# mahmoudnafifi/HistoGAN

Measured on AMD Instinct MI355X. Metric: train images/sec (G+D step, 256², h=64) at 1/2/4/8 MI355X; hist-kernel HBM GB/s, higher is better.
Workload: dtype f32; 1 GPU; HistoGAN G+D train step 256x256 capacity=16 batch=32/GPU h=64 insz=150 inverse-quadratic (GP every 4th, PL every 32nd step); batch_per_gpu=32, global_batch=32, image_size=256, network_capacity=16, h=64, parallelism=dp1, params_G=82968288, params_D=90896289

## Files before the change

### histogan_amd/_lib.py

```python
import ctypes
import os

import torch

_PKG = os.path.dirname(os.path.abspath(__file__))
_TAG = os.environ.get('HG_LIB_TAG', '')
LIB_PATH = os.path.join(_PKG, 'libhistogan_hip' + ('_' + _TAG if _TAG else '') + '.so')

HG_METHOD = {'thresholding': 0, 'RBF': 1, 'inverse-quadratic': 2}
HG_RESIZE_NONE, HG_RESIZE_BILINEAR, HG_RESIZE_SAMPLING = 0, 1, 2
HG_PROJ = {'rgbuv': 0, 'rgchroma': 1, 'direct': 2}


class HgHistParams(ctypes.Structure):
    _fields_ = [
        ('struct_size', ctypes.c_uint32),
        ('B', ctypes.c_int32), ('C', ctypes.c_int32), ('H', ctypes.c_int32), ('W', ctypes.c_int32),
        ('stride_b', ctypes.c_int64), ('stride_c', ctypes.c_int64),
        ('stride_h', ctypes.c_int64), ('stride_w', ctypes.c_int64),
        ('Hs', ctypes.c_int32), ('Ws', ctypes.c_int32),
        ('resize_mode', ctypes.c_int32),
        ('row_idx', ctypes.c_void_p), ('col_idx', ctypes.c_void_p),
        ('h', ctypes.c_int32),
        ('lo', ctypes.c_double), ('hi', ctypes.c_double),
        ('method', ctypes.c_int32),
        ('sigma', ctypes.c_double),
        ('intensity_scale', ctypes.c_int32),
        ('green_only', ctypes.c_int32),
        ('projection', ctypes.c_int32),
        ('pre_relu', ctypes.c_int32),
        ('proj_cache', ctypes.c_void_p),
        ('weight', ctypes.c_void_p),
        ('weight_stride_b', ctypes.c_int64), ('weight_stride_h', ctypes.c_int64), ('weight_stride_w', ctypes.c_int64),
    ]


class GlinLayer(ctypes.Structure):
    _fields_ = [('x', ctypes.c_void_p), ('w', ctypes.c_void_p), ('b', ctypes.c_void_p), ('y', ctypes.c_void_p),
                ('gw', ctypes.c_void_p), ('gb', ctypes.c_void_p), ('N', ctypes.c_int32), ('group', ctypes.c_int32)]


def _load():
    if not os.path.exists(LIB_PATH):
        raise ImportError(
            f'{LIB_PATH} not found: the gfx950 HIP library has not been built. '
            f'Run `python -m histogan_amd.build` (needs hipcc). There is no CPU/PyTorch fallback.')
    lib = ctypes.CDLL(LIB_PATH, mode=ctypes.RTLD_GLOBAL)
    vp, sz, i32, i64, f32 = ctypes.c_void_p, ctypes.c_size_t, ctypes.c_int32, ctypes.c_int64, ctypes.c_float
    PP = ctypes.POINTER(HgHistParams)
    lib.hg_version.restype = ctypes.c_int
    lib.hg_version.argtypes = []
    lib.hg_error_string.restype = ctypes.c_char_p
    lib.hg_error_string.argtypes = [ctypes.c_int]
    lib.hg_rgbuv_hist_workspace_bytes.restype = ctypes.c_int
    lib.hg_rgbuv_hist_workspace_bytes.argtypes = [PP, ctypes.POINTER(sz), ctypes.POINTER(sz)]
    lib.hg_rgbuv_hist_uses_proj_cache.restype = ctypes.c_int
    lib.hg_rgbuv_hist_uses_proj_cache.argtypes = [PP]
    lib.hg_rgbuv_hist_fwd.restype = ctypes.c_int
    lib.hg_rgbuv_hist_fwd.argtypes = [PP, vp, vp, vp, vp, sz, vp]
    lib.hg_rgbuv_hist_bwd.restype = ctypes.c_int
    lib.hg_rgbuv_hist_bwd.argtypes = [PP, vp, vp, vp, vp, vp, vp, sz, vp]
    lib.hg_hellinger_workspace_bytes.restype = sz
    lib.hg_hellinger_workspace_bytes.argtypes = [i64]
    lib.hg_hellinger_fwd_bwd.restype = ctypes.c_int
    lib.hg_hellinger_fwd_bwd.argtypes = [vp, vp, i64, i32, f32, vp, vp, vp, sz, vp]
    lib.hg_selftest_fastlog.restype = ctypes.c_int
    lib.hg_selftest_fastlog.argtypes = [vp, vp]
    lib.hg_modulate_fwd.restype = ctypes.c_int
    lib.hg_modulate_fwd.argtypes = [vp, vp, vp, i32, i32, i32, i32, i32, vp]
    lib.hg_modulate_bwd.restype = ctypes.c_int
    lib.hg_modulate_bwd.argtypes = [vp, vp, vp, vp, vp, i32, i32, i32, i32, i32, vp, sz, vp]
    lib.hg_nets_workspace_bytes.restype = sz
    lib.hg_nets_workspace_bytes.argtypes = [i32, i32, i32, i32]
    lib.hg_torgb_fwd.restype = ctypes.c_int
    lib.hg_torgb_fwd.argtypes = [vp, vp, vp, vp, vp, i32, i32, i32, i32, vp]
    lib.hg_torgb_bwd_workspace_bytes.restype = sz
    lib.hg_torgb_bwd_workspace_bytes.argtypes = [i32, i32, i32, i32]
    lib.hg_torgb_bwd.restype = ctypes.c_int
    lib.hg_torgb_bwd.argtypes = [vp, vp, vp, vp, vp, vp, vp, i32, i32, i32, i32, vp, sz, vp]
    lib.hg_gstage_bwd_workspace_bytes.restype = sz
    lib.hg_gstage_bwd_workspace_bytes.argtypes = [i32, i32, i32, i32]
    lib.hg_gstage_bwd.restype = ctypes.c_int
    lib.hg_gstage_bwd.argtypes = [vp, vp, vp, i32, vp, vp, vp, i32, vp, vp, vp, vp, i32, vp, vp, vp, vp, vp, vp, vp, i32, i32, i32,
                                  vp, sz, vp]
    lib.hg_channel_sum.restype = ctypes.c_int
    lib.hg_channel_sum.argtypes = [vp, vp, i32, i32, i32, vp, sz, vp]
    lib.hg_demod_noise_lrelu_fwd.restype = ctypes.c_int
    lib.hg_demod_noise_lrelu_fwd.argtypes = [vp, vp, vp, vp, vp, vp, i32, i32, i32, i32, vp]
    lib.hg_demod_noise_lrelu_bwd.restype = ctypes.c_int
    lib.hg_demod_noise_lrelu_bwd.argtypes = [vp, vp, vp, vp, vp, vp, vp, vp, vp, vp, vp, i32, i32, i32, i32, vp, sz, vp]
    lib.hg_lrelu_bwd_channel_sum.restype = ctypes.c_int
    lib.hg_lrelu_bwd_channel_sum.argtypes = [vp, vp, f32, vp, vp, i32, i32, i32, vp, sz, vp]
    lib.hg_demod_style_grad_workspace_bytes.restype = ctypes.c_size_t
    lib.hg_demod_style_grad_workspace_bytes.argtypes = [i32, i32, i32]
    lib.hg_demod_style_grad.restype = ctypes.c_int
    lib.hg_demod_style_grad.argtypes = [vp, vp, vp, vp, vp, i32, i32, i32, vp, sz, vp]
    lib.hg_demod_weight_term.restype = ctypes.c_int
    lib.hg_demod_weight_term.argtypes = [vp, vp, vp, vp, vp, i32, i32, i32, i32, i32, vp]
    lib.hg_diffgrad_step.restype = ctypes.c_int
    lib.hg_diffgrad_step.argtypes = [vp, vp, vp, vp, vp, i64, f32, f32, f32, f32, i32, vp]
    lib.hg_diffgrad_step_size.restype = f32
    lib.hg_diffgrad_step_size.argtypes = [f32, f32, f32, i32]
    lib.hg_diffgrad_step_dev.restype = ctypes.c_int
    lib.hg_diffgrad_step_dev.argtypes = [vp, vp, vp, vp, vp, i64, vp, f32, f32, f32, vp]
    lib.hg_ema_update.restype = ctypes.c_int
    lib.hg_ema_update.argtypes = [vp, vp, i64, f32, vp]
    lib.hg_conv_packed_elems.restype = sz
    lib.hg_conv_packed_elems.argtypes = [i32, i32, i32, i32]
    lib.hg_conv_pack_weights.restype = ctypes.c_int
    lib.hg_conv_pack_weights.argtypes = [vp, vp, i32, i32, i32, i32, vp]
    lib.hg_conv_pack_weights_both.restype = ctypes.c_int
    lib.hg_conv_pack_weights_both.argtypes = [vp, vp, vp, i32, i32, i32, vp]
    lib.hg_conv2d_fwd.restype = ctypes.c_int
    lib.hg_conv2d_fwd.argtypes = [vp, vp, vp, vp, vp, vp, i32, i32, i32, i32, i32, i32, i32, vp, sz, vp]
    lib.hg_conv2d_fwd_add.restype = ctypes.c_int
    lib.hg_conv2d_fwd_add.argtypes = [vp, vp, vp, vp, vp, i32, i32, i32, i32, i32, i32, i32, vp, sz, vp]
    lib.hg_modconv2d_fwd.restype = ctypes.c_int
    lib.hg_modconv2d_fwd.argtypes = [vp, vp, vp, vp, vp, vp, vp, vp, i32, f32, i32, i32, i32, i32, i32, i32, vp, sz, vp]
    lib.hg_conv2d_workspace_bytes.restype = sz
    lib.hg_conv2d_workspace_bytes.argtypes = [i32, i32, i32, i32, i32, i32, i32, i32]
    lib.hg_conv_pack_blocks.restype = ctypes.c_int32
    lib.hg_conv_pack_blocks.argtypes = [i32, i32]
    lib.hg_conv_pack_weights_multi.restype = ctypes.c_int
    lib.hg_conv_pack_weights_multi.argtypes = [vp, i32, i32, vp]
    lib.hg_conv2d_plan.restype = ctypes.c_int
    lib.hg_conv2d_plan.argtypes = [i32, i32, i32, i32, i32, i32, i32, i32, ctypes.POINTER(ctypes.c_int32)]
    lib.hg_conv2d_dgrad.restype = ctypes.c_int
    lib.hg_conv2d_dgrad.argtypes = [vp, vp, vp, vp, vp, i32, i32, i32, i32, i32, i32, i32, vp, sz, vp]
    lib.hg_conv2d_wgrad_workspace_bytes.restype = sz
    lib.hg_conv2d_wgrad_workspace_bytes.argtypes = [i32, i32, i32, i32, i32, i32, i32]
    lib.hg_conv2d_wgrad.restype = ctypes.c_int
    lib.hg_conv2d_wgrad.argtypes = [vp, vp, vp, vp, vp, i32, i32, i32, i32, i32, i32, i32, vp, sz, vp]
    lib.hg_instnorm_workspace_bytes.restype = sz
    lib.hg_instnorm_workspace_bytes.argtypes = [i64]
    lib.hg_instnorm_lrelu_fwd.restype = ctypes.c_int
    lib.hg_instnorm_lrelu_fwd.argtypes = [vp, vp, vp, i64, i32, f32, f32, vp, sz, vp]
    lib.hg_instnorm_lrelu_bwd.restype = ctypes.c_int
    lib.hg_instnorm_lrelu_bwd.argtypes = [vp, vp, vp, vp, i64, i32, f32, vp, sz, vp]
    lib.hg_stencil3.restype = ctypes.c_int
    lib.hg_stencil3.argtypes = [vp, vp, ctypes.POINTER(f32), i32, i32, i32, i32, i32, vp]
    lib.hg_depthwise_valid.restype = ctypes.c_int
    lib.hg_depthwise_valid.argtypes = [vp, vp, vp, i64, i32, i32, i32, i32, vp]
    GL = ctypes.POINTER(GlinLayer)
    lib.hg_grouped_linear_fwd.restype = ctypes.c_int
    lib.hg_grouped_linear_fwd.argtypes = [GL, i32, i32, i32, vp]
    lib.hg_grouped_linear_bwd_input_workspace_bytes.restype = sz
    lib.hg_grouped_linear_bwd_input_workspace_bytes.argtypes = [GL, i32, i32, i32]
    lib.hg_grouped_linear_bwd_input.restype = ctypes.c_int
    lib.hg_grouped_linear_bwd_input.argtypes = [GL, i32, ctypes.POINTER(vp), i32, i32, i32, vp, sz, vp]
    lib.hg_grouped_linear_bwd_params.restype = ctypes.c_int
    lib.hg_grouped_linear_bwd_params.argtypes = [GL, i32, i32, i32, vp]
    lib.hg_wino_supported.restype = ctypes.c_int
    lib.hg_wino_supported.argtypes = [i32, i32, i32, i32, i32]
    lib.hg_wino_packed_elems.restype = sz
    lib.hg_wino_packed_elems.argtypes = [i32, i32, i32]
    lib.hg_wino_pack_weights.restype = ctypes.c_int
    lib.hg_wino_pack_weights.argtypes = [vp, vp, i32, i32, i32, vp]
    lib.hg_wino_pack_blocks.restype = ctypes.c_int32
    lib.hg_wino_pack_blocks.argtypes = [i32, i32, i32, i32]
    lib.hg_wino_pack_weights_multi.restype = ctypes.c_int
    lib.hg_wino_pack_weights_multi.argtypes = [vp, i32, i32, vp]
    lib.hg_wino_workspace_bytes.restype = sz
    lib.hg_wino_workspace_bytes.argtypes = [i32, i32, i32, i32, i32]
    lib.hg_wino_conv2d.restype = ctypes.c_int
    lib.hg_wino_conv2d.argtypes = [vp, vp, vp, vp, vp, vp, vp, vp, i32, f32, vp, i32, i32, i32, i32, i32, vp, sz, vp]
    lib.hg_wino_wgrad_supported.restype = ctypes.c_int
    lib.hg_wino_wgrad_supported.argtypes = [i32, i32, i32, i32, i32]
    lib.hg_wino_wgrad_workspace_bytes.restype = sz
    lib.hg_wino_wgrad_workspace_bytes.argtypes = [i32, i32, i32, i32, i32]
    lib.hg_wino_wgrad.restype = ctypes.c_int
    lib.hg_wino_wgrad.argtypes = [vp, vp, vp, i32, i32, i32, i32, i32, vp, sz, vp]
    lib.hg_augment_spatial.restype = ctypes.c_int
    lib.hg_augment_spatial.argtypes = [vp, vp, vp, i32, i32, i32, i32, i32, vp]
    lib.hg_augment_workspace_bytes.restype = sz
    lib.hg_augment_workspace_bytes.argtypes = [i32]
    lib.hg_sample_mean.restype = ctypes.c_int
    lib.hg_sample_mean.argtypes = [vp, vp, i32, i64, vp, sz, vp]
    lib.hg_augment_color.restype = ctypes.c_int
    lib.hg_augment_color.argtypes = [vp, vp, vp, vp, i32, i32, i32, i32, vp]
    lib.hg_resize_axis.restype = ctypes.c_int
    lib.hg_resize_axis.argtypes = [vp, i32, i64, i64, i64, i32, vp, i32, i64, i64, i64, i32, i32, i32, i32, vp, vp, i32,
                                   i32, vp]
    lib.hg_pyr_down.restype = ctypes.c_int
    lib.hg_pyr_down.argtypes = [vp, vp, i32, i32, i32, vp]
    lib.hg_pyr_up_add.restype = ctypes.c_int
    lib.hg_pyr_up_add.argtypes = [vp, vp, vp, f32, vp, vp, f32, vp, i32, i32, i32, vp]
    lib.hg_color_moments_workspace_bytes.restype = sz
    lib.hg_color_moments_workspace_bytes.argtypes = [i64]
    lib.hg_color_moments.restype = ctypes.c_int
    lib.hg_color_moments.argtypes = [vp, i64, i64, i64, vp, vp, sz, vp]
    lib.hg_color_affine.restype = ctypes.c_int
    lib.hg_color_affine.argtypes = [vp, i64, i64, i64, ctypes.POINTER(f32), vp, i32, vp]
    lib.hg_u8_hwc_to_f32.restype = ctypes.c_int
    lib.hg_u8_hwc_to_f32.argtypes = [vp, vp, i32, i64, vp]
    lib.hg_f32_to_u8_hwc.restype = ctypes.c_int
    lib.hg_f32_to_u8_hwc.argtypes = [vp, vp, i32, i64, vp]
    return lib


lib = _load()

EXPORTS = ('hg_version', 'hg_error_string', 'hg_rgbuv_hist_workspace_bytes', 'hg_rgbuv_hist_uses_proj_cache', 'hg_rgbuv_hist_fwd',
           'hg_rgbuv_hist_bwd', 'hg_hellinger_workspace_bytes', 'hg_hellinger_fwd_bwd', 'hg_selftest_fastlog',
           'hg_modulate_fwd', 'hg_modulate_bwd', 'hg_demod_noise_lrelu_fwd', 'hg_demod_noise_lrelu_bwd',
           'hg_diffgrad_step', 'hg_diffgrad_step_size', 'hg_diffgrad_step_dev', 'hg_ema_update', 'hg_nets_workspace_bytes', 'hg_channel_sum', 'hg_lrelu_bwd_channel_sum', 'hg_demod_weight_term', 'hg_demod_style_grad', 'hg_demod_style_grad_workspace_bytes',
           'hg_conv_packed_elems', 'hg_conv_pack_weights', 'hg_conv_pack_weights_both', 'hg_conv_pack_blocks', 'hg_conv_pack_weights_multi', 'hg_conv2d_fwd', 'hg_conv2d_fwd_add', 'hg_modconv2d_fwd', 'hg_conv2d_workspace_bytes', 'hg_conv2d_plan', 'hg_conv2d_dgrad',
           'hg_conv2d_wgrad_workspace_bytes',
           'hg_conv2d_wgrad',
           'hg_instnorm_workspace_bytes', 'hg_instnorm_lrelu_fwd', 'hg_instnorm_lrelu_bwd', 'hg_stencil3',
           'hg_depthwise_valid', 'hg_augment_spatial', 'hg_augment_workspace_bytes', 'hg_sample_mean',
           'hg_augment_color', 'hg_grouped_linear_fwd', 'hg_grouped_linear_bwd_input_workspace_bytes',
           'hg_grouped_linear_bwd_input', 'hg_grouped_linear_bwd_params',
           'hg_wino_supported', 'hg_wino_packed_elems', 'hg_wino_pack_weights', 'hg_wino_pack_blocks', 'hg_wino_pack_weights_multi', 'hg_wino_workspace_bytes', 'hg_wino_conv2d',
           'hg_wino_wgrad_supported', 'hg_wino_wgrad_workspace_bytes', 'hg_wino_wgrad',
           'hg_torgb_fwd', 'hg_torgb_bwd_workspace_bytes', 'hg_torgb_bwd', 'hg_gstage_bwd_workspace_bytes', 'hg_gstage_bwd',
           'hg_resize_axis', 'hg_pyr_down', 'hg_pyr_up_add', 'hg_color_moments_workspace_bytes', 'hg_color_moments',
           'hg_color_affine', 'hg_u8_hwc_to_f32', 'hg_f32_to_u8_hwc')


class HgError(RuntimeError):
    pass


def check(rc, what):
    if rc != 0:
        msg = lib.hg_error_string(rc).decode()
        raise HgError(f'{what}: {msg} (code {rc})')


class NullCtx:
    def __enter__(self):
        return self

    def __exit__(self, *a):
        return False


_NULL = NullCtx()


def on_device(device):
    idx = device.index
    if idx is None or idx == torch.cuda.current_device():
        return _NULL
    return torch.cuda.device(device)


def raw_stream(device):
    idx = device.index if device.index is not None else torch.cuda.current_device()
    return ctypes.c_void_p(torch._C._cuda_getCurrentRawStream(idx))


def stream_of(t):
    return raw_stream(t.device)


def f32c(t):
    t = t.detach()
    t = t if t.dtype == torch.float32 else t.float()
    return t if t.is_contiguous() else t.contiguous()


def ptr(t):
    return None if t is None else t.data_ptr()


def need_gpu(t, what, found='tensor on {}'):
    if not torch.is_tensor(t) or not t.is_cuda:
        raise RuntimeError(f'{what}: {found.format(getattr(t, "device", None))}; the MI355X-native path has no CPU implementation')


def workspace(nbytes, device):
    return torch.empty(max(nbytes, 4), dtype=torch.uint8, device=device)
```

### histogan_amd/conv.py

```python
import contextlib
import ctypes
import os
import weakref

import torch

from ._lib import check, f32c, lib, on_device, ptr, raw_stream, stream_of, workspace
from .launch import channel_sum

PACK_FWD, PACK_DGRAD = 0, 1
_skip_wgrad = False

WINO = os.environ.get('HG_WINO', '1') != '0'
_wino_ok = {}
_wino_used = set()


def wino_supported(B, K, N, H, W):
    key = (B, K, N, H, W)
    r = _wino_ok.get(key)
    if r is None:
        r = _wino_ok[key] = bool(WINO and lib.hg_wino_supported(B, K, N, H, W))
    return r

# ... 305 lines not shown
    if st is None:
        st = _pack_streams[device.index] = torch.cuda.Stream(device=device)
    st.wait_event(torch.cuda.current_stream(device).record_event())
    with torch.cuda.stream(st):
        ok = _pack_owner(owner, device, record_on=st)
    return ok


def drain_pack_streams():
    for idx, st in _pack_streams.items():
        torch.cuda.current_stream(torch.device('cuda', idx)).wait_stream(st)
    _pack_events.clear()


def _await_pack(owner, device, key=None):
    if torch.cuda.is_current_stream_capturing():
        return
    ents = _pack_events.get(owner)
    if ents:
        cur = torch.cuda.current_stream(device)
        for ev, seen, keys in ents:
            if (key is None or key in keys) and cur.cuda_stream not in seen:
                cur.wait_event(ev)
                seen.add(cur.cuda_stream)


def _pack_both(w):
    Co, Ci, k, _ = w.shape
    with on_device(w.device):
        wf = torch.empty(lib.hg_conv_packed_elems(Co, Ci, k, PACK_FWD), dtype=torch.float32, device=w.device)
        wd = torch.empty(lib.hg_conv_packed_elems(Co, Ci, k, PACK_DGRAD), dtype=torch.float32, device=w.device)
        check(lib.hg_conv_pack_weights_both(w.data_ptr(), wf.data_ptr(), wd.data_ptr(), Co, Ci, k, stream_of(w)),
              'hg_conv_pack_weights_both')
    if k == 3:
        wf.wino_src = wd.wino_src = w
    return {PACK_FWD: wf, PACK_DGRAD: wd}


def _pack_weights(w, mode):
    Co, Ci, k, _ = w.shape
    n = lib.hg_conv_packed_elems(Co, Ci, k, mode)
    if n == 0:
        raise ValueError(f'conv weights {tuple(w.shape)}: only square 1x1 / 3x3 kernels are implemented')
    with on_device(w.device):
        wt = torch.empty(n, dtype=torch.float32, device=w.device)
        check(lib.hg_conv_pack_weights(w.data_ptr(), wt.data_ptr(), Co, Ci, k, mode, stream_of(w)), 'hg_conv_pack_weights')
    if k == 3:
        wt.wino_src = w
    return wt


def conv_fwd_packed(x, wt, N, ksize, stride=1, iscale=None, oscale=None, bias=None):
    B, K, H, W = x.shape
    if ksize == 3 and stride == 1:
        u = _wino_u(wt, PACK_FWD, B, K, N, H, W)
        if u is not None:
            return wino_conv(x, u, N, iscale, oscale, bias)
    with on_device(x.device):
        out = torch.empty((B, N, _out_size(H, stride), _out_size(W, stride)), dtype=torch.float32, device=x.device)
        nb = lib.hg_conv2d_workspace_bytes(B, K, N, H, W, ksize, stride, 0)
        ws = torch.empty(nb, dtype=torch.uint8, device=x.device) if nb else None
        check(lib.hg_conv2d_fwd(x.data_ptr(), _direct_operand(wt).data_ptr(), out.data_ptr(), ptr(iscale), ptr(oscale), ptr(bias),
                                B, K, N, H, W, ksize, stride, ptr(ws), nb, stream_of(x)), 'hg_conv2d_fwd')
    return out


def conv_fwd_add_packed(x, wt, N, ksize, addend, bias=None, stride=1):
    B, K, H, W = x.shape
    if ksize == 3 and stride == 1 and tuple(addend.shape) == (B, N, H, W):
        u = _wino_u(wt, PACK_FWD, B, K, N, H, W)
        if u is not None:
            return wino_conv(x, u, N, bias=bias, addend=addend)
    with on_device(x.device):
        out = torch.empty((B, N, _out_size(H, stride), _out_size(W, stride)), dtype=torch.float32, device=x.device)
        if addend.shape != out.shape:
            raise ValueError(f'conv2d_add: addend {tuple(addend.shape)} does not match the output {tuple(out.shape)}')
        nb = lib.hg_conv2d_workspace_bytes(B, K, N, H, W, ksize, stride, 0)
        ws = torch.empty(nb, dtype=torch.uint8, device=x.device) if nb else None
        check(lib.hg_conv2d_fwd_add(x.data_ptr(), _direct_operand(wt).data_ptr(), out.data_ptr(), addend.data_ptr(), ptr(bias),
                                    B, K, N, H, W, ksize, stride, ptr(ws), nb, stream_of(x)), 'hg_conv2d_fwd_add')
    return out


def lrelu_bwd_channel_sum(g, out, slope, want_sum=True):
    g, out = f32c(g), f32c(out)
    B, C, H, W = g.shape
    with on_device(g.device):
        gm = torch.empty_like(g)
        cs = torch.empty(C, dtype=torch.float32, device=g.device) if want_sum else None
        nb = lib.hg_nets_workspace_bytes(B, C, H, W)
        ws = workspace(nb, g.device)
        check(lib.hg_lrelu_bwd_channel_sum(g.data_ptr(), out.data_ptr(), float(slope), gm.data_ptr(), ptr(cs), B, C, H * W,
                                           ws.data_ptr(), ws.numel(), stream_of(g)), 'hg_lrelu_bwd_channel_sum')
    return gm, cs


def conv_dgrad_packed(g, wt, N, H, W, ksize, stride=1, iscale=None, oscale=None):
    B, K = g.shape[:2]
    if ksize == 3 and stride == 1:
        u = _wino_u(wt, PACK_DGRAD, B, K, N, H, W)
        if u is not None:
            return wino_conv(g, u, N, iscale, oscale)
    with on_device(g.device):
        gin = torch.empty((B, N, H, W), dtype=torch.float32, device=g.device)
        nb = lib.hg_conv2d_workspace_bytes(B, K, N, H, W, ksize, stride, 1)
        ws = torch.empty(nb, dtype=torch.uint8, device=g.device) if nb else None
        check(lib.hg_conv2d_dgrad(g.data_ptr(), _direct_operand(wt).data_ptr(), gin.data_ptr(), ptr(iscale), ptr(oscale),
                                  B, K, N, H, W, ksize, stride, ptr(ws), nb, stream_of(g)), 'hg_conv2d_dgrad')
    return gin


def conv_wgrad(x, gout, ksize, stride=1, iscale=None, gscale=None, out=None):
    B, K, H, W = x.shape
    N = gout.shape[1]
    if ksize == 3 and stride == 1 and iscale is None and gscale is None and wino_wgrad_supported(B, K, N, H, W):
        with on_device(x.device):
            nbytes = lib.hg_wino_wgrad_workspace_bytes(B, K, N, H, W)
            ws = torch.empty(nbytes, dtype=torch.uint8, device=x.device)
            gw = out if out is not None else torch.empty((N, K, 3, 3), dtype=torch.float32, device=x.device)
            check(lib.hg_wino_wgrad(x.data_ptr(), gout.data_ptr(), gw.data_ptr(), B, K, N, H, W, ws.data_ptr(), nbytes, stream_of(x)),
                  'hg_wino_wgrad')
        return gw
    with on_device(x.device):
        nbytes = lib.hg_conv2d_wgrad_workspace_bytes(B, K, N, H, W, ksize, stride)
        ws = workspace(nbytes, x.device)
        gw = out if out is not None else torch.empty((N, K, ksize, ksize), dtype=torch.float32, device=x.device)
        check(lib.hg_conv2d_wgrad(x.data_ptr(), gout.data_ptr(), gw.data_ptr(), ptr(iscale), ptr(gscale),
                                  B, K, N, H, W, ksize, stride, ws.data_ptr(), ws.numel(), stream_of(x)), 'hg_conv2d_wgrad')
    return gw



_slots = {}
_side_streams = {}


def register_grad_slots(flat):
    ref = weakref.ref(flat)
    off = 0
    for p in flat.params:
        n = p.numel()
        if p.dim() == 4 and flat.grad is not None:
            _slots[(p.data_ptr(), tuple(p.shape))] = (off, n, ref)
        off += n


def grad_slot(w):
    if torch.is_grad_enabled():
        return None
    ent = _slots.get((w.data_ptr(), tuple(w.shape)))
    if ent is None:
        return None
    off, n, ref = ent
    flat = ref()
    if flat is None or not getattr(flat, 'direct_ok', False):
        return None
    return flat.grad[off:off + n].view(w.shape), flat


def side_stream(device):
    st = _side_streams.get(device.index)
    if st is None:
        st = _side_streams[device.index] = torch.cuda.Stream(device=device)
    return st


def _assert_single_writer(device):
    cur = torch.cuda.current_stream(device)
    assert torch.cuda.is_current_stream_capturing() or cur.cuda_stream == side_stream(device).cuda_stream, \
        'direct gradient write outside the weight-gradient stream'


def _direct_wgrad(w, x, g, stride):
    if torch.is_grad_enabled():
        return False
    key = (w.data_ptr(), tuple(w.shape))
    ent = _slots.get(key)
    if ent is None:
        return False
    off, n, ref = ent
    flat = ref()
    if flat is None:
        del _slots[key]
        return False
    if not getattr(flat, 'direct_ok', False):
        return False
    slot = flat.grad[off:off + n].view(w.shape)
    xc, gc = f32c(x), f32c(g)
    if _batch_pieces(xc, w, stride) != 1:
        return False
    skey = slot.data_ptr()
    if torch.cuda.is_current_stream_capturing():
# ... 116 lines not shown
        ctx.save_for_backward(g, x)
        ctx.stride = stride
        return conv_wgrad(f32c(x), f32c(g), ksize, stride)

    @staticmethod
    def backward(ctx, ggw):
        g, x = ctx.saved_tensors
        gg = gx = None
        if ctx.needs_input_grad[0]:
            gg = _Conv.apply(x, ggw, None, ctx.stride)
        if ctx.needs_input_grad[1]:
            gx = _ConvDgrad.apply(g, ggw, x.shape[2], x.shape[3], ctx.stride)
        return gg, gx, None, None


class _ConvLrelu(torch.autograd.Function):

    @staticmethod
    def forward(ctx, x, w, bias, stride, slope):
        _check_args(x, w, stride)
        if x.shape[1] != w.shape[1]:
            raise ValueError(f'conv2d: x {tuple(x.shape)} does not match w {tuple(w.shape)}')
        xc, wc = f32c(x), f32c(w)
        B, K, H, W = xc.shape
        N, k = w.shape[0], w.shape[2]
        wt = pack_weights(wc, PACK_FWD)
        bc = None if bias is None else f32c(bias)
        if stride != 1:
            raise ValueError('conv2d_lrelu: stride 1 only')
        out = modconv_fwd_packed(xc, wt, N, k, bias=bc, slope=slope)
        ctx.save_for_backward(x, w, out)
        ctx.stride, ctx.has_bias, ctx.slope = stride, bias is not None, float(slope)
        return out

    @staticmethod
    def backward(ctx, g):
        x, w, out = ctx.saved_tensors
        gx = gw = gb = None
        want_gb = ctx.has_bias and ctx.needs_input_grad[2] and not _skip_wgrad
        if torch.is_grad_enabled():
            gm = torch.ops.aten.leaky_relu_backward(g, out, ctx.slope, True)
            if want_gb:
                gb = gm.sum(dim=(0, 2, 3))
        else:
            gm, gb = lrelu_bwd_channel_sum(g, out, ctx.slope, want_gb)
        if ctx.needs_input_grad[0]:
            gx = _ConvDgrad.apply(gm, w, x.shape[2], x.shape[3], ctx.stride)
        if not _skip_wgrad:
            if ctx.needs_input_grad[1] and not _direct_wgrad(w, x, gm, ctx.stride):
                gw = _ConvWgrad.apply(gm, x, w.shape[2], ctx.stride)
        return gx, gw, gb, None, None


class _ConvAdd(torch.autograd.Function):

    @staticmethod
    def forward(ctx, x, w, bias, addend, stride):
        _check_args(x, w, stride)
        if x.shape[1] != w.shape[1]:
            raise ValueError(f'conv2d: x {tuple(x.shape)} does not match w {tuple(w.shape)}')
        ctx.save_for_backward(x, w)
        ctx.stride, ctx.has_bias = stride, bias is not None
        xc, wc = f32c(x), f32c(w)
        bc = None if bias is None else f32c(bias)
        return conv_fwd_add_packed(xc, pack_weights(wc, PACK_FWD), w.shape[0], w.shape[2], f32c(addend), bc, stride)

    @staticmethod
    def backward(ctx, g):
        x, w = ctx.saved_tensors
        gx = gw = gb = None
        if ctx.needs_input_grad[0]:
            gx = _ConvDgrad.apply(g, w, x.shape[2], x.shape[3], ctx.stride)
        if not _skip_wgrad:
            if ctx.needs_input_grad[1] and not _direct_wgrad(w, x, g, ctx.stride):
                gw = _ConvWgrad.apply(g, x, w.shape[2], ctx.stride)
            if ctx.has_bias and ctx.needs_input_grad[2]:
                if torch.is_grad_enabled():
                    gb = g.sum(dim=(0, 2, 3))
                else:
                    gb = channel_sum(g)
        return gx, gw, gb, (g if ctx.needs_input_grad[3] else None), None


_I32 = 2 ** 31 - 1


def _batch_pieces(x, w, stride):
    B, K, H, W = x.shape
    per = max(K * H * W, w.shape[0] * _out_size(H, stride) * _out_size(W, stride))
    if B * per <= _I32:
        return 1
    if per > _I32:
        raise ValueError(f'conv2d: one sample of shape {tuple(x.shape[1:])} -> {w.shape[0]} channels exceeds 2^31 elements')
    return -(-B // (_I32 // per))


def _sliced(fn, x, w, stride):
    n = _batch_pieces(x, w, stride)
    if n == 1:
        return fn(x)
    return torch.cat([fn(xs) for xs in x.chunk(n, dim=0)], dim=0)


def conv2d_lrelu(x, w, bias=None, slope=0.2):
    return _sliced(lambda t: _ConvLrelu.apply(t, w, bias, 1, slope), x, w, 1)


def conv2d(x, w, bias=None, stride=1):
    return _sliced(lambda t: _Conv.apply(t, w, bias, stride), x, w, stride)


def conv2d_add(x, w, bias, addend, stride=1):
    if _batch_pieces(x, w, stride) != 1:
        return conv2d(x, w, bias, stride) + addend
    return _ConvAdd.apply(x, w, bias, addend, stride)


def conv2d_same(x, w, bias=None):
    return _sliced(lambda t: _Conv.apply(t, w, bias, 1), x, w, 1)
```

### histogan_amd/csrc/hg_conv.hip

```cpp
#include <atomic>
#include <cstdio>
#include <cstdlib>
#include "hg_common.h"
#include "../../include/hg_hist.h"
#include "../../include/hg_conv.h"

constexpr int kConvMinWaves = 2;
constexpr int kConvKC = 4;

namespace {

struct Geom {
  int lTW, lTH, lNI;
  int TWp, IMS, HALO, CHS;
  float inv_TWp, inv_IMS, inv_HALO;
  int tiles_x, tiles_y, groups;
  int lo_y, lo_x;
};

struct ConvArgs {
  const float *in, *wt;
  float *out;
  const float *iscale, *oscale, *bias;
  const float *addend;
  int B, K, N, Kp, Np;
  int Hi, Wi;
  int Ho, Wo;
  int Hc, Wc;
  int os, oy, ox;
  int toff[9];
  int ntx, wrow0, wrow_dy, wrow_dx;
  int ksplit;
  float *slab;
  const float *noise_w, *noise_img;
  int noise_S;
  float slope;
  Geom g;
};

__device__ __forceinline__ int fdiv(int e, float inv) {
  return (int)(((float)e + 0.5f) * inv);
}

constexpr unsigned kOOB = 0xFFFFFFFFu;
__device__ __forceinline__ __amdgpu_buffer_rsrc_t make_rsrc(const float *base, unsigned bytes = kOOB) {
  return __builtin_amdgcn_make_buffer_rsrc(const_cast<float *>(base), 0, (int)bytes, 0x00020000);
}
__device__ __forceinline__ const float *uniform_ptr(const float *p) {
  const unsigned long long v = (unsigned long long)p;
  const unsigned lo = __builtin_amdgcn_readfirstlane((unsigned)v), hi = __builtin_amdgcn_readfirstlane((unsigned)(v >> 32));
  return (const float *)(((unsigned long long)hi << 32) | lo);
}
constexpr unsigned kFar = 0x80000000u;
__device__ __forceinline__ float buf_load(__amdgpu_buffer_rsrc_t r, unsigned voff, int soff) {
  return __builtin_bit_cast(float, __builtin_amdgcn_raw_buffer_load_b32(r, (int)voff, soff, 0));
}
__device__ __forceinline__ f32x4 buf_load4(__amdgpu_buffer_rsrc_t r, unsigned voff, int soff) {
  return __builtin_bit_cast(f32x4, __builtin_amdgcn_raw_buffer_load_b128(r, (int)voff, soff, 0));
}

template <int MT>
struct MfmaTile {
  typedef f32x16 acc_t;
  static constexpr int NR = 16, KS = 2;
  static __device__ __forceinline__ acc_t mma(float a, float b, acc_t c) { return __builtin_amdgcn_mfma_f32_32x32x2f32(a, b, c, 0, 0, 0); }
  static __device__ __forceinline__ int row(int r, int lk) { return (r & 3) + 8 * (r >> 2) + 4 * lk; }
};
template <>
struct MfmaTile<16> {
  typedef f32x4 acc_t;
  static constexpr int NR = 4, KS = 4;
  static __device__ __forceinline__ acc_t mma(float a, float b, acc_t c) { return __builtin_amdgcn_mfma_f32_16x16x4f32(a, b, c, 0, 0, 0); }
  static __device__ __forceinline__ int row(int r, int lk) { return 4 * lk + r; }
};

template <int WC, int WP, int TC, int TP, int TAPS, int KC, int IS, bool SM, int MT, bool FE>
__device__ __forceinline__ void conv_body(const ConvArgs &a, const int bidx, const int bidy, const int bidz) {
  typedef MfmaTile<MT> M;
  constexpr int KS = M::KS;
  static_assert(KC % KS == 0, "chunk must hold whole MFMA k-steps");
  constexpr int NT = WC * WP * 64;
  constexpr int NB = WC * TC * MT;
  constexpr int MB = WP * TP * MT;
  constexpr int WPT = KC * NB / 4;
  constexpr int WTOT = TAPS * WPT;
  constexpr int NW = (WTOT + NT - 1) / NT;
  constexpr int R16 = IS == 2 ? (SM ? 100 : 83) : (TAPS == 1 ? 16 : (SM ? 64 : (MB == 256 ? 22 : (MB == 128 ? 26 : 36))));
  constexpr int HMAX = KC * MB * R16 / 16;
  constexpr int NH = (HMAX + NT - 1) / NT;

  extern __shared__ float smem[];
  float *Ws = smem;
  float *Xs = smem + TAPS * KC * NB;

  const Geom &g = a.g;
  const int tid = threadIdx.x, lane = tid & 63, wave = tid >> 6;
  const int lm = lane % MT, lk = lane / MT;
  const int wc = wave % WC, wp = wave / WC;
  const int Hi = a.Hi, Wi = a.Wi, K = a.K, N = a.N;

  int pt = bidx;
  const int tx = pt % g.tiles_x;
  pt /= g.tiles_x;
  const int ty = pt % g.tiles_y;
  const int grp = pt / g.tiles_y;
  const int x0 = tx << g.lTW, y0 = ty << g.lTH, b0 = grp << g.lNI;
  const int n0 = bidy * NB;
  const int TWm = (1 << g.lTW) - 1, THm = (1 << g.lTH) - 1;

  unsigned voff[NH];
  int xso[NH];
  const int htot = KC * g.HALO;
#pragma unroll
  for (int i = 0; i < NH; ++i) {
    const int e = tid + i * NT;
    voff[i] = kOOB;
    xso[i] = KC * g.CHS + lane;
    if (e < htot) {
      const int kc = fdiv(e, g.inv_HALO);
      const int r = e - kc * g.HALO;
      const int img = fdiv(r, g.inv_IMS);
      const int rr = r - img * g.IMS;
      const int hy = fdiv(rr, g.inv_TWp);
      const int hx = rr - hy * g.TWp;
      const int gy = y0 * IS + g.lo_y + hy, gx = x0 * IS + g.lo_x + hx, b = b0 + img;
      xso[i] = kc * g.CHS + r;
      if (b < a.B && (unsigned)gy < (unsigned)Hi && (unsigned)gx < (unsigned)Wi)
        voff[i] = (unsigned)(((img * K + kc) * Hi + gy) * Wi + gx) * 4u;
    }
  }
  unsigned wv[NW];
#pragma unroll
  for (int i = 0; i < NW; ++i) {
    const int id = tid + i * NT;
    const int t = id / WPT, e4 = id % WPT;
    const int kc = e4 / (NB / 4), c4 = e4 % (NB / 4);
    const int wrow = t < TAPS ? a.wrow0 + (t / a.ntx) * a.wrow_dy + (t % a.ntx) * a.wrow_dx : 0;
    wv[i] = (NW * NT == WTOT || id < WTOT) ? (unsigned)((wrow + kc) * a.Np + n0 + c4 * 4) * 4u : kOOB;
  }
  const int wdump = (TAPS * KC * NB + KC * g.CHS + 64) / 4 + 1 + lane;

  int pixoff[TP];
#pragma unroll
  for (int tp = 0; tp < TP; ++tp) {
    const int p = (wp * TP + tp) * MT + lm;
    const int px = p & TWm, py = (p >> g.lTW) & THm, pi = p >> (g.lTW + g.lTH);
    pixoff[tp] = pi * g.IMS + py * IS * g.TWp + px * IS + lk * g.CHS;
  }
  const int aoff = lk * NB + wc * TC * MT + lm;

  typename M::acc_t acc[TC][TP];
#pragma unroll
  for (int i = 0; i < TC; ++i)
#pragma unroll
    for (int j = 0; j < TP; ++j)
#pragma unroll
      for (int r = 0; r < M::NR; ++r) acc[i][j][r] = 0.f;

  float xr[NH];
// ... 15 lines not shown
  const int nchunks_all = (K + KC - 1) / KC;
  const int cps = (nchunks_all + a.ksplit - 1) / a.ksplit;
  const int c_begin = bidz * cps;
  const int nchunks = c_begin + cps < nchunks_all ? c_begin + cps : nchunks_all;
  const int HWi = Hi * Wi;
  const float *inblk = a.in + (size_t)b0 * K * HWi;
  const __amdgpu_buffer_rsrc_t rw = make_rsrc(a.wt), rs = make_rsrc(uniform_ptr(FE && a.iscale ? a.iscale : a.wt));

  auto prefetch = [&](int c) __attribute__((always_inline)) {
    const __amdgpu_buffer_rsrc_t rx = make_rsrc(inblk + (size_t)c * KC * HWi);
    if (K - c * KC < KC) {
      const int krem = K - c * KC;
#pragma unroll
      for (int i = 0; i < NH; ++i)
        if (fdiv(tid + i * NT, g.inv_HALO) >= krem) {
          voff[i] = kOOB;
          if constexpr (FE) soff[i] = kOOB;
        }
    }
#pragma unroll
    for (int i = 0; i < NH; ++i) xr[i] = buf_load(rx, voff[i], 0);
    if constexpr (FE) {
      if (a.iscale != nullptr) {
#pragma unroll
        for (int i = 0; i < NH; ++i) xs[i] = buf_load(rs, soff[i], c * KC * 4);
      }
    }
#pragma unroll
    for (int i = 0; i < NW; ++i) wr[i] = buf_load4(rw, wv[i], c * KC * a.Np * 4);
  };

  for (int c = c_begin - 1; c < nchunks; ++c) {
    if (c >= c_begin) {
      __syncthreads();
#pragma unroll
      for (int i = 0; i < NH; ++i) Xs[xso[i]] = (FE && a.iscale != nullptr) ? xr[i] * xs[FE ? i : 0] : xr[i];
#pragma unroll
      for (int i = 0; i < NW; ++i) {
        const int id = tid + i * NT;
        if (NW * NT == WTOT || i + 1 < NW) reinterpret_cast<f32x4 *>(Ws)[id] = wr[i];
        else reinterpret_cast<f32x4 *>(Ws)[id < WTOT ? id : wdump] = wr[i];
      }
      __syncthreads();
    }
    if (c + 1 < nchunks) prefetch(c + 1);
    if (c < c_begin) continue;

    constexpr int NS = TAPS * (KC / KS);
    float av[2][TC], bv[2][TP];
    auto ldop = [&](int s_, int slot) __attribute__((always_inline)) {
      const int t = s_ / (KC / KS), kk = s_ % (KC / KS);
#pragma unroll
      for (int i = 0; i < TC; ++i) av[slot][i] = Ws[(t * KC + kk * KS) * NB + aoff + i * MT];
      if constexpr (TAPS == 9) {
        const int roff = a.toff[(t / 3) * 3];
#pragma unroll
        for (int j = 0; j < TP; ++j) bv[slot][j] = (Xs + pixoff[j] + roff + kk * KS * g.CHS)[t % 3];
      } else {
        const int toff = a.toff[t];
#pragma unroll
        for (int j = 0; j < TP; ++j) bv[slot][j] = Xs[pixoff[j] + toff + kk * KS * g.CHS];
      }
    };
    ldop(0, 0);
    constexpr int DSN = (MT == 32 ? (TC + 1) / 2 : TC) + TP;
    __builtin_amdgcn_sched_group_barrier(0x100, DSN, 0);
#pragma unroll
    for (int s_ = 0; s_ < NS; ++s_) {
      if (s_ + 1 < NS) ldop(s_ + 1, (s_ + 1) & 1);
#pragma unroll
      for (int i = 0; i < TC; ++i)
#pragma unroll
        for (int j = 0; j < TP; ++j) acc[i][j] = M::mma(av[s_ & 1][i], bv[s_ & 1][j], acc[i][j]);
      if (s_ + 1 < NS) {
        __builtin_amdgcn_sched_group_barrier(0x002, 1, 0);
        __builtin_amdgcn_sched_group_barrier(0x100, DSN, 0);
      }
      __builtin_amdgcn_sched_group_barrier(0x008, TC * TP, 0);
    }
  }

  const int HWo = a.Ho * a.Wo;
  auto epilogue = [&](const bool fin) __attribute__((always_inline)) {
  if constexpr (!FE) {
#pragma unroll
    for (int j = 0; j < TP; ++j) {
      const int p = (wp * TP + j) * MT + lm;
      const int px = p & TWm, py = (p >> g.lTW) & THm, pi = p >> (g.lTW + g.lTH);
      const int cx = x0 + px, cy = y0 + py, b = b0 + pi;
      if (b >= a.B || cy >= a.Hc || cx >= a.Wc) continue;
      const size_t pofs = ((size_t)b * N) * HWo + (cy * a.os + a.oy) * a.Wo + cx * a.os + a.ox;
      float *ob = (fin ? a.out : a.slab + (size_t)bidz * a.B * N * HWo) + pofs;
#pragma unroll
      for (int i = 0; i < TC; ++i) {
#pragma unroll
        for (int r = 0; r < M::NR; ++r) {
          const int ch = n0 + (wc * TC + i) * MT + M::row(r, lk);
          if (ch < N) {
            float v = acc[i][j][r];
            if (fin && a.bias) v += a.bias[ch];
            if (fin && a.addend) v += a.addend[pofs + (size_t)ch * HWo];
            ob[(size_t)ch * HWo] = v;
          }
        }
      }
    }
  } else {
    const float *__restrict__ pbias_ = a.bias, *__restrict__ pnw_ = a.noise_w, *__restrict__ posc_ = a.oscale;
#pragma unroll
    for (int i = 0; i < TC; ++i) {
      float pbias[M::NR], pnw[M::NR];
#pragma unroll
      for (int r = 0; r < M::NR; ++r) {
        const int ch = n0 + (wc * TC + i) * MT + M::row(r, lk);
        const int cc = ch < N ? ch : N - 1;
        pbias[r] = (fin && pbias_) ? pbias_[cc] : 0.f;
        pnw[r] = (fin && a.noise_img) ? pnw_[cc] : 0.f;
      }
#pragma unroll
      for (int j = 0; j < TP; ++j) {
        const int p = (wp * TP + j) * MT + lm;
        const int px = p & TWm, py = (p >> g.lTW) & THm, pi = p >> (g.lTW + g.lTH);
        const int cx = x0 + px, cy = y0 + py, b = b0 + pi;
        if (b >= a.B || cy >= a.Hc || cx >= a.Wc) continue;
        const size_t pofs = ((size_t)b * N) * HWo + (cy * a.os + a.oy) * a.Wo + cx * a.os + a.ox;
        float *ob = (fin ? a.out : a.slab + (size_t)bidz * a.B * N * HWo) + pofs;
        const float nz = (a.noise_img != nullptr && fin)
                             ? a.noise_img[((size_t)b * a.noise_S + cy * a.os + a.oy) * a.noise_S + cx * a.os + a.ox] : 0.f;
        float posc[M::NR];
#pragma unroll
        for (int r = 0; r < M::NR; ++r) {
          const int ch = n0 + (wc * TC + i) * MT + M::row(r, lk);
          posc[r] = (fin && posc_) ? posc_[b * N + (ch < N ? ch : N - 1)] : 1.f;
        }
#pragma unroll
        for (int r = 0; r < M::NR; ++r) {
          const int ch = n0 + (wc * TC + i) * MT + M::row(r, lk);
          if (ch < N) {
            float v = fmaf(acc[i][j][r], posc[r], fmaf(pnw[r], nz, pbias[r]));
            if (fin && a.slope > 0.f) v = v > 0.f ? v : a.slope * v;
            ob[(size_t)ch * HWo] = v;
          }
        }
      }
    }
  }
  };
  epilogue(a.ksplit == 1);
}

template <int WC, int WP, int TC, int TP, int TAPS, int KC, int IS, bool SM, int MT, bool FE>
__global__ __launch_bounds__(WC *WP * 64, kConvMinWaves) void k_conv(const ConvArgs a) {
  conv_body<WC, WP, TC, TP, TAPS, KC, IS, SM, MT, FE>(a, blockIdx.x, blockIdx.y, blockIdx.z);
}

struct ConvArgs4 {
  ConvArgs c[4];
  int tiles[4];
  int xcd_map;
};
template <int WC, int WP, int TC, int TP, int KC, bool SM, int MT, bool FE>
__global__ __launch_bounds__(WC *WP * 64, kConvMinWaves) void k_conv_parity4(const ConvArgs4 a) {
  const int cls = a.xcd_map ? (blockIdx.x >> 3) & 3 : blockIdx.x & 3;
  const int t = a.xcd_map ? (blockIdx.x >> 5) * 8 + (blockIdx.x & 7) : blockIdx.x >> 2;
  if (t >= a.tiles[cls]) return;
  if (cls == 0) conv_body<WC, WP, TC, TP, 1, KC, 1, SM, MT, FE>(a.c[0], t, blockIdx.y, blockIdx.z);
  else if (cls == 1) conv_body<WC, WP, TC, TP, 2, KC, 1, SM, MT, FE>(a.c[1], t, blockIdx.y, blockIdx.z);
  else if (cls == 2) conv_body<WC, WP, TC, TP, 2, KC, 1, SM, MT, FE>(a.c[2], t, blockIdx.y, blockIdx.z);
  else conv_body<WC, WP, TC, TP, 4, KC, 1, SM, MT, FE>(a.c[3], t, blockIdx.y, blockIdx.z);
}

__global__ __launch_bounds__(256) void k_splitk_reduce(const float *__restrict__ slab, float *__restrict__ out,
                                                       const float *__restrict__ oscale, const float *__restrict__ bias,
                                                       const float *__restrict__ noise_w, const float *__restrict__ noise_img,
                                                       const float *__restrict__ addend, int noise_S, float slope,
                                                       long long total, int HWo, int Wo, int N, int ksplit) {
  for (long long i = (long long)blockIdx.x * 256 + threadIdx.x; i < total; i += (long long)gridDim.x * 256) {
    float v = 0.f;
    for (int z = 0; z < ksplit; ++z) v += slab[(size_t)z * total + i];
    const long long bn = i / HWo;
    const int n = (int)(bn % N);
    float add = bias ? bias[n] : 0.f;
    if (noise_img) {
      const int p = (int)(i - bn * HWo), y = p / Wo, x = p - y * Wo;
      add = fmaf(noise_w[n], noise_img[((size_t)(bn / N) * noise_S + y) * noise_S + x], add);
    }
    v = oscale ? fmaf(v, oscale[bn], add) : v + add;
    if (addend) v += addend[i];
    if (slope > 0.f) v = v > 0.f ? v : slope * v;
    out[i] = v;
  }
}

struct WgradArgs {
  const float *in, *gout;
  float *slab;
  const float *iscale, *gscale;
  int B, K, N, Hi, Wi, Ho, Wo, Kp32, Np32;
  int tiles_x, tiles_y, nchunks, splits, ktiles;
  float *gw;
};

constexpr int WG_TP = 32 * 9 + 4;

template <int PC, int LTW, int PAD, int IS>
struct CGeom {
  static constexpr int TW = 1 << LTW;
  static constexpr int TH = (PC / TW) < TW ? (PC / TW) : TW;
  static constexpr int NI = PC / (TW * TH);
  static constexpr int TWp = (TW - 1) * IS + 1 + 2 * PAD, THp = (TH - 1) * IS + 1 + 2 * PAD;
  static constexpr int IMS = TWp * THp, HALO = NI * IMS, CHS = HALO | 1;
};

template <int WN, int WK, int WS, int TAPS, int PC, int LTW, int IS, int MT, int TS = 1, bool SC = false>
__global__ __launch_bounds__(WN *WK *WS *TS * 64) void k_wgrad(const WgradArgs a) {
  typedef MfmaTile<MT> M;
  static_assert(TS == 1 || (TS == 3 && TAPS == 9), "tap split: rows of the 3x3 kernel");
  constexpr int TPW = TAPS / TS;
  constexpr int KS = M::KS;
  constexpr int NT = WN * WK * WS * TS * 64;
  constexpr int NBW = WN * MT;
  constexpr int KBW = WK * MT;
  constexpr int PAD = TAPS == 9 ? 1 : 0;
  using G = CGeom<PC, LTW, PAD, IS>;
  constexpr int GP = PC + 1;

  extern __shared__ float smem[];
  float *Gs = smem;
  float *Xs = smem + NBW * GP;

  const int tid = threadIdx.x, lane = tid & 63, wave = tid >> 6;
  const int lm = lane % MT, lk = lane / MT;
  static_assert((1 << LTW) >= KS, "the pixels of one MFMA k-step must lie in one tile row");
  const int wn = wave % WN, wk = (wave / WN) % WK, ws = (wave / (WN * WK)) % WS, wt = wave / (WN * WK * WS);
  const int t0 = wt * TPW;
  const int Hi = a.Hi, Wi = a.Wi, Ho = a.Ho, Wo = a.Wo, K = a.K, N = a.N;
  const int HWi = Hi * Wi, HWo = Ho * Wo;
  const int k0 = (blockIdx.x % a.ktiles) * KBW, n0 = (blockIdx.x / a.ktiles) * NBW;

  typename M::acc_t acc[TPW];
#pragma unroll
  for (int t = 0; t < TPW; ++t)
#pragma unroll
    for (int r = 0; r < M::NR; ++r) acc[t][r] = 0.f;

  const float *Ga = Gs + (wn * MT + lm) * GP + lk;
  const float *Xa = Xs + (wk * MT + lm) * G::CHS + lk * IS;

  constexpr int GCPI = NT / PC, NGI = (NBW + GCPI - 1) / GCPI;
  constexpr int HCPI = NT / G::HALO, NHI = (KBW + HCPI - 1) / HCPI;
  static_assert(HCPI >= 1, "halo tile wider than the block");
  const int gcs = tid / PC, gp = tid % PC;
  const int gpx = gp % G::TW, gpy = (gp / G::TW) % G::TH, gpi = gp / (G::TW * G::TH);
  const int hcs = tid / G::HALO, hrr = tid % G::HALO;
  const int himg = hrr / G::IMS, hy = (hrr % G::IMS) / G::TWp, hx = hrr % G::TWp;
  const bool hlane = hcs < HCPI;

  unsigned gstat = 0;
  unsigned long long hstat = 0;
  static_assert(NGI <= 32 && NHI <= 64, "validity masks");
#pragma unroll
  for (int i = 0; i < NGI; ++i)
    if (n0 + gcs + i * GCPI < N && (NGI * GCPI == NBW || gcs + i * GCPI < NBW)) gstat |= 1u << i;
#pragma unroll
  for (int i = 0; i < NHI; ++i)
    if (hlane && k0 + hcs + i * HCPI < K && (NHI * HCPI == KBW || hcs + i * HCPI < KBW)) hstat |= 1ull << i;

  float gr[NGI], hr[NHI];
  unsigned gmask = 0;
  unsigned long long hmask = 0;
  int pb0 = 0;
  auto prefetch = [&](int chunk) __attribute__((always_inline)) {
    int pt = chunk;
    const int tx = pt % a.tiles_x;
// ... 487 lines not shown
  const long long nblk = (long long)((Wc + tw - 1) / tw) * ((Hc + th - 1) / th) * ((B + ni - 1) / ni) * ((N + 63) / 64);
  const int kc = IS == 2 ? 8 : 2 * kConvKC, nchunks = (K + kc - 1) / kc;
  const int tgt64 = (big_split && IS == 1) ? 1024 : 512;
  if (have_ws && os == 1 && nblk < 384 && nchunks >= 8) {
    int ks = (int)((tgt64 + nblk - 1) / nblk);
    if (ks > nchunks / 4) ks = nchunks / 4;
    if (ks > 32) ks = 32;
    if (ks > 1) p.ksplit = ks;
  }
  return p;
}

inline int launch_splitk_reduce(const ConvArgs &a, int ksplit, hipStream_t st);

inline unsigned long long next_conv_tag() {
  static std::atomic<unsigned long long> ctr{0x9E3779B97F4A7C15ull ^ ((unsigned long long)(uintptr_t)&ctr << 17)};
  return ctr.fetch_add(2, std::memory_order_relaxed) | 1ull;
}

inline long long plan_blocks(const ConvPlan &p, int B, int N, int Hc, int Wc) {
  const long long px = (long long)B * Hc * Wc;
  const int nbt = p.tile == TILE_16x256 ? 16 : p.tile == TILE_32x256 ? 32 : (p.tile == TILE_64x256 || p.tile == TILE_64x64) ? 64 : 128;
  const int mbt = (p.tile == TILE_128x128 || p.tile == TILE_128x128_SM) ? 128 : p.tile == TILE_64x64 ? 64 : 256;
  return ((N + nbt - 1) / nbt) * ((px + mbt - 1) / mbt);
}
inline bool short_k_chunks(const ConvPlan &p, int B, int N, int Hc, int Wc) {
  if (p.tile == TILE_32x256) return true;
  if (p.tile == TILE_64x256 || (p.tile == TILE_128x128 && p.ksplit == 1)) {
    const long long nwg = plan_blocks(p, B, N, Hc, Wc), cus = num_cus();
    return nwg % (4 * cus) == 0 && nwg % (3 * cus) != 0 && nwg <= 32 * cus;
  }
  return false;
}

template <int WC, int WP, int TC, int TP, int TAPS, int KC, int IS, bool SM, int MT>
size_t prep_conv(ConvArgs &a, const Taps &tp, int ksplit) {
  constexpr int NB = WC * TC * MT, MB = WP * TP * MT;
  int lo_y = 0, hi_y = 0, lo_x = 0, hi_x = 0;
  for (int t = 0; t < TAPS; ++t) {
    lo_y = tp.dy[t] < lo_y ? tp.dy[t] : lo_y; hi_y = tp.dy[t] > hi_y ? tp.dy[t] : hi_y;
    lo_x = tp.dx[t] < lo_x ? tp.dx[t] : lo_x; hi_x = tp.dx[t] > hi_x ? tp.dx[t] : hi_x;
  }
  a.g = make_geom(MB, a.B, a.Hc, a.Wc, IS, lo_y, hi_y, lo_x, hi_x, false, SM ? 2 : 4);
  for (int t = 0; t < TAPS; ++t) a.toff[t] = (tp.dy[t] - lo_y) * a.g.TWp + (tp.dx[t] - lo_x);
  a.ntx = tp.ntx;
  a.wrow0 = tp.w[0] * a.Kp;
  a.wrow_dx = tp.ntx > 1 ? (tp.w[1] - tp.w[0]) * a.Kp : 0;
  a.wrow_dy = TAPS > tp.ntx ? (tp.w[tp.ntx] - tp.w[0]) * a.Kp : 0;
  a.ksplit = ksplit;
  if ((long long)(1 << a.g.lNI) * a.K * a.Hi * a.Wi >= (1LL << 30)) return 0;
  return ((size_t)TAPS * KC * NB + (size_t)KC * a.g.CHS + 64 + 8 + 256) * sizeof(float);
}

inline int fit_blocks_per_cu(const void *kern, int threads, long long nwg, size_t &lds, int state[2], const char *what) {
  if (!state[0]) {
    int n = 0;
    if (hipOccupancyMaxActiveBlocksPerMultiprocessor(&n, kern, threads, lds) != hipSuccess || n < 1) n = 1;
    state[0] = n;
  }
  const int by_lds = (int)(kLdsPerCu / lds), cm = by_lds < state[0] ? (by_lds > 1 ? by_lds : 1) : state[0];
  const int c = pick_blocks_per_cu(nwg, cm);
  if (c < cm) {
    const size_t need = (size_t)kLdsPerCu / (c + 1) + 512;
    if (lds < need) lds = need;
  }
  static const bool dbg = getenv("HG_CONV_DEBUG") != nullptr;
  if (dbg) fprintf(stderr, "%s: %lld blocks, max %d (registers %d) -> %d per CU, lds %zu\n", what, nwg, cm, state[0], c, lds);
  if (lds > 48 * 1024 && !state[1]) {
    hipError_t e = hipFuncSetAttribute(kern, hipFuncAttributeMaxDynamicSharedMemorySize, (int)kLdsPerCu);
    if (e != hipSuccess) return (int)e;
    state[1] = 1;
  }
  return 0;
}

template <int WC, int WP, int TC, int TP, int TAPS, int KC, int IS, bool SM = false, int MT = 32>
int launch_conv(ConvArgs a, const Taps &tp, int ksplit, bool reduce, hipStream_t st, size_t ws_bytes = 0) {
  constexpr int NB = WC * TC * MT, NT = WC * WP * 64;
  size_t lds = prep_conv<WC, WP, TC, TP, TAPS, KC, IS, SM, MT>(a, tp, ksplit);
  if (!lds) return HG_EUNSUPPORTED;
  bool inkernel_combine = false;
  (void)ws_bytes;
  const bool fe = a.iscale || a.oscale || a.noise_img || a.slope > 0.f;
  auto kern = fe ? k_conv<WC, WP, TC, TP, TAPS, KC, IS, SM, MT, true> : k_conv<WC, WP, TC, TP, TAPS, KC, IS, SM, MT, false>;
  static int state[2][2] = {{0, 0}, {0, 0}};
  const long long nwg = (long long)a.g.tiles_x * a.g.tiles_y * a.g.groups * ((a.N + NB - 1) / NB) * ksplit;
  char what[96];
  snprintf(what, sizeof what, "k_conv<%d,%d,%d,%d,taps %d,kc %d,is %d,mt %d,fe %d>", WC, WP, TC, TP, TAPS, KC, IS, MT, (int)fe);
  if (int rc = fit_blocks_per_cu((const void *)kern, NT, nwg, lds, state[fe], what)) return rc;
  unsigned gx = (unsigned)(a.g.tiles_x * a.g.tiles_y * a.g.groups);
  if (inkernel_combine) {
    const unsigned ny = (unsigned)((a.N + NB - 1) / NB);
    unsigned m = 8;
    for (unsigned d = 2; d <= 8; d *= 2) if (ny % d == 0) m = 8 / d;
    gx = (gx + m - 1) / m * m;
  }
  dim3 grid(gx, (unsigned)((a.N + NB - 1) / NB), (unsigned)ksplit);
  hipLaunchKernelGGL(kern, grid, dim3(NT), lds, st, a);
  HG_LAUNCH_CHECK();
  if (ksplit > 1 && reduce && !inkernel_combine) return launch_splitk_reduce(a, ksplit, st);
  return HG_OK;
}

template <int WC, int WP, int TC, int TP, int KC, bool SM = false, int MT = 32, bool WITH_FE = true>
int launch_conv_parity4(const ConvArgs (&base)[4], const Taps (&tp)[4], int ksplit, hipStream_t st) {
  constexpr int NB = WC * TC * MT, NT = WC * WP * 64;
  ConvArgs4 a4;
  size_t lds = 0;
  long long tiles_sum = 0;
  int tiles_max = 0;
  for (int c = 0; c < 4; ++c) {
    a4.c[c] = base[c];
    a4.tiles[c] = 0;
    if (base[c].Hc <= 0 || base[c].Wc <= 0) continue;
    size_t l = c == 0 ? prep_conv<WC, WP, TC, TP, 1, KC, 1, SM, MT>(a4.c[c], tp[c], ksplit)
               : c == 3 ? prep_conv<WC, WP, TC, TP, 4, KC, 1, SM, MT>(a4.c[c], tp[c], ksplit)
                        : prep_conv<WC, WP, TC, TP, 2, KC, 1, SM, MT>(a4.c[c], tp[c], ksplit);
    if (!l) return HG_EUNSUPPORTED;
    lds = l > lds ? l : lds;
    a4.tiles[c] = a4.c[c].g.tiles_x * a4.c[c].g.tiles_y * a4.c[c].g.groups;
    tiles_sum += a4.tiles[c];
    tiles_max = a4.tiles[c] > tiles_max ? a4.tiles[c] : tiles_max;
  }
  if (!tiles_max) return HG_OK;
  const ConvArgs &a = base[0];
  const bool fe = a.iscale || a.oscale || a.noise_img || a.slope > 0.f;
  if (fe && !WITH_FE) return HG_EUNSUPPORTED;
  auto kern = k_conv_parity4<WC, WP, TC, TP, KC, SM, MT, false>;
  if constexpr (WITH_FE) { if (fe) kern = k_conv_parity4<WC, WP, TC, TP, KC, SM, MT, true>; }
  static int state[2][2] = {{0, 0}, {0, 0}};
  const int ny = (a.N + NB - 1) / NB;
  if (int rc = fit_blocks_per_cu((const void *)kern, NT, tiles_sum * ny * ksplit, lds, state[fe], "k_conv_parity4")) return rc;
  const bool xcd_map = tiles_max >= 64;
  a4.xcd_map = xcd_map;
  const unsigned gx = xcd_map ? (unsigned)((tiles_max + 7) / 8 * 32) : (unsigned)(4 * tiles_max);
  hipLaunchKernelGGL(kern, dim3(gx, (unsigned)ny, (unsigned)ksplit), dim3(NT), lds, st, a4);
  HG_LAUNCH_CHECK();
  return HG_OK;
}

inline size_t conv_slab_bytes(const ConvPlan &p, int B, int N, int Ho, int Wo) {
  return p.ksplit > 1 ? (size_t)p.ksplit * B * N * Ho * Wo * sizeof(float) : 0;
}
inline size_t conv_ws_bytes(const ConvPlan &p, int B, int N, int Ho, int Wo) { return conv_slab_bytes(p, B, N, Ho, Wo); }


inline int launch_splitk_reduce(const ConvArgs &a, int ksplit, hipStream_t st) {
  const long long total = (long long)a.B * a.N * a.Ho * a.Wo;
  long long nb = (total + 255) / 256;
  if (nb > 4096) nb = 4096;
  hipLaunchKernelGGL(k_splitk_reduce, dim3((unsigned)nb), dim3(256), 0, st, a.slab, a.out, a.oscale, a.bias, a.noise_w,
                     a.noise_img, a.addend, a.noise_S, a.slope, total, a.Ho * a.Wo, a.Wo, a.N, ksplit);
  HG_LAUNCH_CHECK();
  return HG_OK;
}

template <int TAPS, int IS>
int dispatch_conv(ConvArgs a, const Taps &tp, void *ws, size_t ws_bytes, hipStream_t st, int force_ksplit = 0) {
  constexpr int KC = IS == 2 ? 4 : kConvKC;
  a.slab = (float *)ws;
  if (force_ksplit > 0) return launch_conv<2, 2, 1, 1, TAPS, 2 * KC, IS, true>(a, tp, force_ksplit, false, st);
  ConvPlan p = plan_conv(a.B, a.K, a.N, a.Hc, a.Wc, IS, a.os, ws != nullptr, true, TAPS);
  if (conv_slab_bytes(p, a.B, a.N, a.Ho, a.Wo) > ws_bytes) p.ksplit = 1;
  if constexpr (TAPS == 9 && IS == 1 && KC == 4) {
    const bool fe = a.iscale || a.oscale || a.noise_img || a.slope > 0.f;
    if (short_k_chunks(p, a.B, a.N, a.Hc, a.Wc) && (!fe || p.tile == TILE_32x256)) {
      if (p.tile == TILE_32x256) return launch_conv<1, 4, 1, 2, TAPS, 2, IS>(a, tp, 1, true, st);
      if (p.tile == TILE_64x256) return launch_conv<1, 4, 2, 2, TAPS, 2, IS>(a, tp, 1, true, st);
      return launch_conv<2, 2, 2, 2, TAPS, 2, IS>(a, tp, 1, true, st);
    }
  }
  switch (p.tile) {
    case TILE_16x256:
      return launch_conv<1, 4, 1, 4, TAPS, 4, IS, false, 16>(a, tp, 1, true, st);
    case TILE_32x256: return launch_conv<1, 4, 1, 2, TAPS, KC, IS>(a, tp, 1, true, st);
    case TILE_64x256: return launch_conv<1, 4, 2, 2, TAPS, KC, IS>(a, tp, 1, true, st);
    case TILE_128x128: return launch_conv<2, 2, 2, 2, TAPS, KC, IS>(a, tp, p.ksplit, true, st, ws_bytes);
    case TILE_128x128_SM:
      if constexpr (IS == 1) return launch_conv<2, 2, 2, 2, TAPS, KC, IS, true>(a, tp, p.ksplit, true, st, ws_bytes);
      else return HG_EUNSUPPORTED;
    default: return launch_conv<2, 2, 1, 1, TAPS, 2 * KC, IS, true>(a, tp, p.ksplit, true, st, ws_bytes);
  }
}

struct WgradPlan {
  int PC, lTW, tiles_x, tiles_y, groups;
  int MT;
  int WN, WK, WS;
  int nchunks, splits, ktiles, ntiles, Kp32, Np32;
  size_t slab_bytes;
};

inline int out_size(int in, int stride) { return (in - 1) / stride + 1; }

constexpr int wgrad_chunk_pixels(int stride, int MT, int lTW, int WS, int taps) {
  return stride == 2 ? 32 : ((MT == 16 && lTW >= 3) || (MT == 32 && WS > 1 && taps == 9 && lTW >= 4)) ? 128 : 64;
}

WgradPlan make_wgrad_plan(int B, int K, int N, int Hi, int Wi, int ksize, int stride) {
  WgradPlan p;
  const int Ho = out_size(Hi, stride), Wo = out_size(Wi, stride);
  p.MT = (N <= 16 && K <= 16) ? 16 : 32;
  int lTW = ceil_log2(Wo < 2 ? 2 : Wo);
  if (p.MT == 16 && lTW < 2) lTW = 2;
  if (lTW > 5) lTW = 5;
  p.lTW = lTW;
  if (p.MT == 16) {
    p.WN = p.WK = 1;
  } else if (stride == 2) {
    p.WN = p.WK = (N > 32 && K > 32) ? 2 : 1;
  } else {
    p.WN = N > 32 ? 2 : 1;
    p.WK = K > 32 ? 2 : 1;
  }
  p.WS = 4 / (p.WN * p.WK);
  p.PC = wgrad_chunk_pixels(stride, p.MT, lTW, p.WS, ksize * ksize);
  const int TW = 1 << lTW, TH = (p.PC / TW) < TW ? (p.PC / TW) : TW, NI = p.PC / (TW * TH);
  p.tiles_x = (Wo + TW - 1) / TW;
  p.tiles_y = (Ho + TH - 1) / TH;
  p.groups = (B + NI - 1) / NI;
  p.nchunks = p.tiles_x * p.tiles_y * p.groups;
  p.ktiles = (K + p.WK * p.MT - 1) / (p.WK * p.MT);
  p.ntiles = (N + p.WN * p.MT - 1) / (p.WN * p.MT);
  const int tiles = p.ktiles * p.ntiles;
  const int target = (ksize == 3 && p.MT == 32) ? 256 : 512;
  int s = (target + tiles - 1) / tiles;
  if (s > p.nchunks) s = p.nchunks;
  if (s < 1) s = 1;
  p.splits = s;
  p.Kp32 = p.ktiles * p.WK * p.MT;
  p.Np32 = p.ntiles * p.WN * p.MT;
  p.slab_bytes = (size_t)s * ksize * ksize * p.Kp32 * p.Np32 * sizeof(float);
  return p;
}

template <int WN, int WK, int WS, int TAPS, int LTW, int IS, int MT = 32, int TS = 1>
// ... 136 lines not shown
int hg_conv2d_plan(int32_t B, int32_t K, int32_t N, int32_t Hi, int32_t Wi, int32_t ksize, int32_t stride, int32_t dgrad,
                   int32_t out[5]) {
  if (!out || !conv_args_ok(B, K, N, Hi, Wi, ksize, stride)) return HG_EINVAL;
  if (dgrad && stride != 1) return HG_EUNSUPPORTED;
  const int Hc = dgrad ? Hi : out_size(Hi, stride), Wc = dgrad ? Wi : out_size(Wi, stride);
  const ConvPlan p = plan_conv(B, K, N, Hc, Wc, dgrad ? 1 : stride, 1, true, true, ksize * ksize);
  const bool k2 = ksize == 3 && stride == 1 && short_k_chunks(p, B, N, Hc, Wc);
  const int base_kc = (dgrad ? 1 : stride) == 2 ? 4 : kConvKC;
  out[0] = (int32_t)p.tile;
  out[1] = p.ksplit;
  out[2] = p.tile == TILE_16x256 ? 4 : (p.tile == TILE_64x64 ? 2 * base_kc : (k2 ? 2 : base_kc));
  const long long nb = plan_blocks(p, B, N, Hc, Wc) * p.ksplit;
  out[3] = nb > 0x7fffffffLL ? 0x7fffffff : (int32_t)nb;
  out[4] = num_cus();
  return HG_OK;
}

int hg_conv_pack_weights_both(const float *w, float *wt_fwd, float *wt_dgrad, int32_t Co, int32_t Ci, int32_t ksize,
                              void *stream) {
  if (!w || !wt_fwd || !wt_dgrad || Co <= 0 || Ci <= 0 || (ksize != 1 && ksize != 3)) return HG_EINVAL;
  const int Kpf = round_up(Ci, 16), Npf = round_up(Co, 128), Kpd = round_up(Co, 16), Npd = round_up(Ci, 128);
  const dim3 grid((unsigned)(round_up(Ci, 128) / 32), (unsigned)(round_up(Co, 128) / 32));
  hipStream_t st = (hipStream_t)stream;
  if (ksize == 3)
    hipLaunchKernelGGL(k_pack_both<9>, grid, dim3(256), 0, st, w, wt_fwd, wt_dgrad, Co, Ci, Kpf, Npf, Kpd, Npd);
  else
    hipLaunchKernelGGL(k_pack_both<1>, grid, dim3(256), 0, st, w, wt_fwd, wt_dgrad, Co, Ci, Kpf, Npf, Kpd, Npd);
  HG_LAUNCH_CHECK();
  return HG_OK;
}

static int conv2d_fwd_impl(const float *in, const float *wt, float *out, const float *iscale, const float *oscale,
                           const float *bias, const float *noise_w, const float *noise_img, int32_t noise_S,
                           float lrelu_slope, int32_t B, int32_t K, int32_t N, int32_t Hi, int32_t Wi, int32_t ksize,
                           int32_t stride, void *workspace, size_t workspace_bytes, void *stream,
                           const float *addend = nullptr) {
  if (!in || !wt || !out || !conv_args_ok(B, K, N, Hi, Wi, ksize, stride)) return HG_EINVAL;
  if (addend && (iscale || oscale || noise_img || lrelu_slope > 0.f)) return HG_EINVAL;
  if ((noise_img != nullptr) != (noise_w != nullptr) || lrelu_slope < 0.f) return HG_EINVAL;
  if (noise_img && (noise_S < out_size(Hi, stride) || noise_S < out_size(Wi, stride))) return HG_EINVAL;
  if (!fits_i32(B, K, N, Hi, Wi)) return HG_EUNSUPPORTED;
  ConvArgs a;
  a.in = in; a.wt = wt; a.out = out; a.iscale = iscale; a.oscale = oscale; a.bias = bias; a.addend = addend;
  a.noise_w = noise_w; a.noise_img = noise_img; a.noise_S = noise_S; a.slope = lrelu_slope;
  a.B = B; a.K = K; a.N = N; a.Hi = Hi; a.Wi = Wi;
  a.Ho = a.Hc = out_size(Hi, stride); a.Wo = a.Wc = out_size(Wi, stride);
  a.os = 1; a.oy = a.ox = 0;
  a.Kp = round_up(K, 16); a.Np = round_up(N, 128);
  Taps tp;
  hipStream_t st = (hipStream_t)stream;
  if (ksize == 1) {
    tp.n = 1; tp.ntx = 1; tp.dy[0] = tp.dx[0] = 0; tp.w[0] = 0;
    return dispatch_conv<1, 1>(a, tp, workspace, workspace_bytes, st);
  }
  tp.n = 9; tp.ntx = 3;
  for (int t = 0; t < 9; ++t) { tp.dy[t] = t / 3 - 1; tp.dx[t] = t % 3 - 1; tp.w[t] = t; }
  return stride == 1 ? dispatch_conv<9, 1>(a, tp, workspace, workspace_bytes, st)
                     : dispatch_conv<9, 2>(a, tp, workspace, workspace_bytes, st);
}

int hg_conv2d_fwd(const float *in, const float *wt, float *out, const float *iscale, const float *oscale,
                  const float *bias, int32_t B, int32_t K, int32_t N, int32_t Hi, int32_t Wi, int32_t ksize,
                  int32_t stride, void *workspace, size_t workspace_bytes, void *stream) {
  return conv2d_fwd_impl(in, wt, out, iscale, oscale, bias, nullptr, nullptr, 0, 0.f, B, K, N, Hi, Wi, ksize, stride,
                         workspace, workspace_bytes, stream);
}

int hg_conv2d_fwd_add(const float *in, const float *wt, float *out, const float *addend, const float *bias, int32_t B,
                      int32_t K, int32_t N, int32_t Hi, int32_t Wi, int32_t ksize, int32_t stride, void *workspace,
                      size_t workspace_bytes, void *stream) {
  if (!addend) return HG_EINVAL;
  return conv2d_fwd_impl(in, wt, out, nullptr, nullptr, bias, nullptr, nullptr, 0, 0.f, B, K, N, Hi, Wi, ksize, stride,
                         workspace, workspace_bytes, stream, addend);
}

int hg_modconv2d_fwd(const float *in, const float *wt, float *out, const float *iscale, const float *oscale,
                     const float *bias, const float *noise_w, const float *noise_img, int32_t noise_S,
                     float lrelu_slope, int32_t B, int32_t K, int32_t N, int32_t H, int32_t W, int32_t ksize,
                     void *workspace, size_t workspace_bytes, void *stream) {
  return conv2d_fwd_impl(in, wt, out, iscale, oscale, bias, noise_w, noise_img, noise_S, lrelu_slope, B, K, N, H, W, ksize,
                         1, workspace, workspace_bytes, stream);
}

int hg_conv2d_dgrad(const float *gout, const float *wt, float *gin, const float *iscale, const float *oscale,
                    int32_t B, int32_t K, int32_t N, int32_t Hi, int32_t Wi, int32_t ksize, int32_t stride,
                    void *workspace, size_t workspace_bytes, void *stream) {
  if (!gout || !wt || !gin || !conv_args_ok(B, K, N, Hi, Wi, ksize, stride)) return HG_EINVAL;
  if (!fits_i32(B, K, N, Hi, Wi)) return HG_EUNSUPPORTED;
  hipStream_t st = (hipStream_t)stream;
  ConvArgs a;
  a.in = gout; a.wt = wt; a.out = gin; a.iscale = iscale; a.oscale = oscale; a.bias = nullptr; a.addend = nullptr;
  a.noise_w = a.noise_img = nullptr; a.noise_S = 0; a.slope = 0.f;
  a.B = B; a.K = K; a.N = N;
  a.Hi = out_size(Hi, stride); a.Wi = out_size(Wi, stride);
  a.Ho = Hi; a.Wo = Wi;
  a.Kp = round_up(K, 16); a.Np = round_up(N, 128);
  Taps tp;
  if (stride == 1) {
    a.Hc = Hi; a.Wc = Wi; a.os = 1; a.oy = a.ox = 0;
    if (ksize == 1) {
      tp.n = 1; tp.ntx = 1; tp.dy[0] = tp.dx[0] = 0; tp.w[0] = 0;
      return dispatch_conv<1, 1>(a, tp, workspace, workspace_bytes, st);
    }
    tp.n = 9; tp.ntx = 3;
    for (int t = 0; t < 9; ++t) { tp.dy[t] = t / 3 - 1; tp.dx[t] = t % 3 - 1; tp.w[t] = t; }
    return dispatch_conv<9, 1>(a, tp, workspace, workspace_bytes, st);
  }
  a.os = 2;
  int ksplit = 0;
  bool plan64 = false;
  {
    ConvPlan p = plan_conv(B, K, N, (Hi + 1) / 2, (Wi + 1) / 2, 1, 1, workspace != nullptr, false);
    plan64 = p.tile == TILE_64x64 && Hi > 1 && Wi > 1;
    if (Hi > 1 && Wi > 1 && p.tile == TILE_64x64 && p.ksplit > 1 &&
        (size_t)p.ksplit * B * N * Hi * Wi * sizeof(float) <= workspace_bytes)
      ksplit = p.ksplit;
  }
  ConvArgs ca[4];
  Taps tps[4];
  for (int pY = 0; pY < 2; ++pY)
    for (int pX = 0; pX < 2; ++pX) {
      ConvArgs &c = ca[pY * 2 + pX];
      Taps &t = tps[pY * 2 + pX];
      c = a;
      c.Hc = (Hi - pY + 1) / 2; c.Wc = (Wi - pX + 1) / 2;
      c.oy = pY; c.ox = pX;
      t.n = 0; t.ntx = pX ? 2 : 1;
      for (int dy = 0; dy < 3; ++dy)
        for (int dx = 0; dx < 3; ++dx)
          if (((pY + 1 - dy) & 1) == 0 && ((pX + 1 - dx) & 1) == 0) {
            t.dy[t.n] = (pY + 1 - dy) / 2; t.dx[t.n] = (pX + 1 - dx) / 2; t.w[t.n] = 8 - (3 * dy + dx);
            ++t.n;
          }
    }
  if (!plan64 && Hi > 1 && Wi > 1) {
    const ConvPlan p = plan_conv(B, K, N, Hi / 2, Wi / 2, 1, 2, false, false, 4);
    int rc = HG_EUNSUPPORTED;
    switch (p.tile) {
      case TILE_16x256: rc = launch_conv_parity4<1, 4, 1, 4, 4, false, 16, false>(ca, tps, 1, st); break;
      case TILE_32x256: rc = launch_conv_parity4<1, 4, 1, 2, kConvKC, false, 32, false>(ca, tps, 1, st); break;
      case TILE_64x256: rc = launch_conv_parity4<1, 4, 2, 2, kConvKC, false, 32, false>(ca, tps, 1, st); break;
      case TILE_128x128: rc = launch_conv_parity4<2, 2, 2, 2, kConvKC, false, 32, false>(ca, tps, 1, st); break;
      default: break;
    }
    if (rc != HG_EUNSUPPORTED) return rc;
  }
  if (plan64) {
    if (ksplit > 1) ksplit = ksplit / 2 > 1 ? ksplit / 2 : 1;
    for (int c = 0; c < 4; ++c) ca[c].slab = (float *)workspace;
    const int rc = launch_conv_parity4<2, 2, 1, 1, 2 * kConvKC, true>(ca, tps, ksplit > 1 ? ksplit : 1, st);
    if (rc) return rc;
  } else {
    for (int c = 0; c < 4; ++c) {
      if (ca[c].Hc <= 0 || ca[c].Wc <= 0) continue;
      int rc;
      if (tps[c].n == 1) rc = dispatch_conv<1, 1>(ca[c], tps[c], workspace, workspace_bytes, st, ksplit);
      else if (tps[c].n == 2) rc = dispatch_conv<2, 1>(ca[c], tps[c], workspace, workspace_bytes, st, ksplit);
      else rc = dispatch_conv<4, 1>(ca[c], tps[c], workspace, workspace_bytes, st, ksplit);
      if (rc) return rc;
    }
  }
  if (ksplit > 1) {
    a.slab = (float *)workspace;
    return launch_splitk_reduce(a, ksplit, st);
  }
  return HG_OK;
}

size_t hg_conv2d_wgrad_workspace_bytes(int32_t B, int32_t K, int32_t N, int32_t Hi, int32_t Wi, int32_t ksize,
                                       int32_t stride) {
  if (!conv_args_ok(B, K, N, Hi, Wi, ksize, stride)) return 0;
  return make_wgrad_plan(B, K, N, Hi, Wi, ksize, stride).slab_bytes;
}

int hg_conv2d_wgrad(const float *in, const float *gout, float *gw, const float *iscale, const float *gscale, int32_t B,
// ... 17 lines not shown
```

### histogan_amd/csrc/hg_nets.hip

```cpp
#include "hg_common.h"
#include "../../include/hg_hist.h"
#include "../../include/hg_nets.h"

namespace {

template <int NT>
__device__ __forceinline__ float block_sum(float v, float *sm) {
  v = hg_wave_sum(v);
  if constexpr (NT == 64) return v;
  const int w = threadIdx.x >> 6;
  if ((threadIdx.x & 63) == 0) sm[w] = v;
  __syncthreads();
  float r = 0.f;
#pragma unroll
  for (int i = 0; i < NT / 64; ++i) r += sm[i];
  __syncthreads();
  return r;
}

__device__ __forceinline__ void up2_taps(int Y, int H, int &i0, int &i1, float &l) {
  const float src = fmaxf(0.5f * ((float)Y + 0.5f) - 0.5f, 0.f);
  i0 = min((int)src, H - 1);
  l = src - (float)i0;
  i1 = i0 + (i0 < H - 1 ? 1 : 0);
// ... 244 lines not shown
  a_b = block_sum<256>(a_b, sm);
  if (threadIdx.x == 0) {
    const size_t planes = gridDim.y, idx = (size_t)bo * gridDim.x + blockIdx.x;
    part[idx] = a_d;
    part[planes * gridDim.x + idx] = a_w;
    part[2 * planes * gridDim.x + idx] = a_b;
  }
}

__global__ __launch_bounds__(256) void k_dnl_bwd_finish(const float *__restrict__ part, float *__restrict__ gd,
                                                        float *__restrict__ gw, float *__restrict__ gb,
                                                        const float *__restrict__ ddiv, int planes, int chunks) {
  const int p = blockIdx.x * 256 + threadIdx.x;
  if (p >= planes) return;
  float v0 = 0.f, v1 = 0.f, v2 = 0.f;
  for (int c = 0; c < chunks; ++c) {
    v0 += part[(size_t)p * chunks + c];
    v1 += part[(size_t)planes * chunks + (size_t)p * chunks + c];
    v2 += part[2 * (size_t)planes * chunks + (size_t)p * chunks + c];
  }
  if (gd) gd[p] = ddiv ? v0 / ddiv[p] : v0;
  gw[p] = v1;
  gb[p] = v2;
}

__global__ __launch_bounds__(256) void k_channel_sum(const float *__restrict__ g, float *__restrict__ part, int B, int C,
                                                     int HW) {
  __shared__ float sm[4];
  const int c = blockIdx.y;
  float acc = 0.f;
  const long long per = (long long)B * HW;
  if ((HW & 3) == 0) {
    const int hw4 = HW / 4;
    for (long long e = (long long)blockIdx.x * 256 + threadIdx.x; e < per / 4; e += (long long)gridDim.x * 256) {
      const long long b = e / hw4, p4 = e - b * hw4;
      const float4 v = reinterpret_cast<const float4 *>(g + ((size_t)b * C + c) * HW)[p4];
      acc += (v.x + v.y) + (v.z + v.w);
    }
  } else {
    for (long long e = (long long)blockIdx.x * 256 + threadIdx.x; e < per; e += (long long)gridDim.x * 256) {
      const long long b = e / HW, p = e - b * HW;
      acc += g[((size_t)b * C + c) * HW + p];
    }
  }
  acc = block_sum<256>(acc, sm);
  if (threadIdx.x == 0) part[(size_t)c * gridDim.x + blockIdx.x] = acc;
}

__global__ __launch_bounds__(256) void k_lrelu_bwd_csum(const float *__restrict__ g, const float *__restrict__ out,
                                                        float *__restrict__ gm, float *__restrict__ part, float slope,
                                                        int B, int C, int HW) {
  __shared__ float sm[4];
  const int c = blockIdx.y;
  float acc = 0.f;
  const long long per = (long long)B * HW;
  if ((HW & 3) == 0) {
    const int hw4 = HW / 4;
    for (long long e = (long long)blockIdx.x * 256 + threadIdx.x; e < per / 4; e += (long long)gridDim.x * 256) {
      const long long b = e / hw4, p4 = e - b * hw4;
      const size_t off = ((size_t)b * C + c) * HW;
      const float4 v = reinterpret_cast<const float4 *>(g + off)[p4];
      const float4 o = reinterpret_cast<const float4 *>(out + off)[p4];
      float4 r;
      r.x = o.x > 0.f ? v.x : v.x * slope; r.y = o.y > 0.f ? v.y : v.y * slope;
      r.z = o.z > 0.f ? v.z : v.z * slope; r.w = o.w > 0.f ? v.w : v.w * slope;
      reinterpret_cast<float4 *>(gm + off)[p4] = r;
      acc += (r.x + r.y) + (r.z + r.w);
    }
  } else {
    for (long long e = (long long)blockIdx.x * 256 + threadIdx.x; e < per; e += (long long)gridDim.x * 256) {
      const long long b = e / HW, p = e - b * HW;
      const size_t off = ((size_t)b * C + c) * HW + p;
      const float v = g[off], r = out[off] > 0.f ? v : v * slope;
      gm[off] = r;
      acc += r;
    }
  }
  if (part) {
    acc = block_sum<256>(acc, sm);
    if (threadIdx.x == 0) part[(size_t)c * gridDim.x + blockIdx.x] = acc;
  }
}

__global__ __launch_bounds__(256) void k_diffgrad(float *__restrict__ p, const float *__restrict__ g,
                                                  float *__restrict__ m, float *__restrict__ v,
                                                  float *__restrict__ pg, long long n, float step_size, float b1,
                                                  float b2, float eps) {
  for (long long i = (long long)blockIdx.x * 256 + threadIdx.x; i < n; i += (long long)gridDim.x * 256) {
    const float gi = g[i];
    const float mi = b1 * m[i] + (1.f - b1) * gi;
    const float vi = b2 * v[i] + (1.f - b2) * gi * gi;
    const float dfc = 1.f / (1.f + expf(-fabsf(pg[i] - gi)));
    m[i] = mi; v[i] = vi; pg[i] = gi;
    p[i] -= step_size * (mi * dfc) / (sqrtf(vi) + eps);
  }
}

__global__ __launch_bounds__(256) void k_diffgrad_dev(float *__restrict__ p, const float *__restrict__ g,
                                                      float *__restrict__ m, float *__restrict__ v,
                                                      float *__restrict__ pg, long long n,
                                                      const float *__restrict__ step_size_dev, float b1, float b2,
                                                      float eps) {
  const float step_size = *step_size_dev;
  for (long long i = (long long)blockIdx.x * 256 + threadIdx.x; i < n; i += (long long)gridDim.x * 256) {
    const float gi = g[i];
    const float mi = b1 * m[i] + (1.f - b1) * gi;
    const float vi = b2 * v[i] + (1.f - b2) * gi * gi;
    const float dfc = 1.f / (1.f + expf(-fabsf(pg[i] - gi)));
    m[i] = mi; v[i] = vi; pg[i] = gi;
    p[i] -= step_size * (mi * dfc) / (sqrtf(vi) + eps);
  }
}

__global__ __launch_bounds__(256) void k_ema(float *__restrict__ ma, const float *__restrict__ p, long long n,
                                             float beta) {
  for (long long i = (long long)blockIdx.x * 256 + threadIdx.x; i < n; i += (long long)gridDim.x * 256)
    ma[i] = ma[i] * beta + (1.f - beta) * p[i];
}

inline unsigned grid_for(long long n_threads) {
  long long b = (n_threads + 255) / 256;
  if (b < 1) b = 1;
  if (b > 256 * 16) b = 256 * 16;
  return (unsigned)b;
}

__global__ __launch_bounds__(256) void k_demod_weight_term(const float *__restrict__ w, const float *__restrict__ gd,
                                                           const float *__restrict__ d, const float *__restrict__ s1,
                                                           float *__restrict__ gw, int B, int N, int K, int T,
                                                           int accumulate) {
  extern __shared__ float dsm[];
  float *Mrow = dsm, *gqc = dsm + K;
  const int o = blockIdx.x;
  for (int b = threadIdx.x; b < B; b += 256) {
    const float dd = d[(size_t)b * N + o];
    gqc[b] = gd[(size_t)b * N + o] * (-0.5f) * dd * dd * dd;
  }
  __syncthreads();
  for (int i = threadIdx.x; i < K; i += 256) {
    float m = 0.f;
    for (int b = 0; b < B; ++b) {
      const float sv = s1[(size_t)b * K + i];
      m = fmaf(gqc[b], sv * sv, m);
    }
    Mrow[i] = 2.f * m;
  }
  __syncthreads();
  const size_t base = (size_t)o * K * T;
  const int n = K * T;
  if ((n & 3) == 0) {
    const f32x4 *w4 = reinterpret_cast<const f32x4 *>(w + base);
    f32x4 *g4 = reinterpret_cast<f32x4 *>(gw + base);
    for (int e = threadIdx.x; e < n / 4; e += 256) {
      f32x4 v = w4[e];
#pragma unroll
      for (int c = 0; c < 4; ++c) v[c] *= Mrow[(4 * e + c) / T];
      if (accumulate) v += g4[e];
      g4[e] = v;
    }
  } else {
    for (int e = threadIdx.x; e < n; e += 256) {
      const float v = w[base + e] * Mrow[e / T];
      gw[base + e] = accumulate ? gw[base + e] + v : v;
    }
  }
}
// ... 136 lines not shown
  if (!conv && (!wn || !bn)) return HG_EINVAL;
  hipStream_t st = (hipStream_t)stream;
  const int planes = B * O;
  const int chunks = plane_chunks(planes, (long long)H * H / 4);
  if (!workspace || workspace_bytes < (size_t)3 * planes * chunks * sizeof(float)) return HG_EWORKSPACE;
  float *part = (float *)workspace;
  hipLaunchKernelGGL(k_dnl_bwd, dim3(chunks, planes), dim3(256), 0, st, gout, out, conv, d, nzt, wn, bn, gconv, part, O, H,
                     S);
  HG_LAUNCH_CHECK();
  hipLaunchKernelGGL(k_dnl_bwd_finish, dim3((planes + 255) / 256), dim3(256), 0, st, part, gd, gwn_part, gbn_part,
                     (!conv && d) ? d : nullptr, planes, chunks);
  HG_LAUNCH_CHECK();
  return HG_OK;
}

int hg_channel_sum(const float *g, float *out, int32_t B, int32_t C, int32_t HW, void *workspace, size_t workspace_bytes,
                   void *stream) {
  if (!g || !out || B <= 0 || C <= 0 || HW <= 0) return HG_EINVAL;
  hipStream_t st = (hipStream_t)stream;
  const int chunks = plane_chunks(C, (long long)B * HW / 4);
  if (!workspace || workspace_bytes < (size_t)C * chunks * sizeof(float)) return HG_EWORKSPACE;
  hipLaunchKernelGGL(k_channel_sum, dim3(chunks, C), dim3(256), 0, st, g, (float *)workspace, B, C, HW);
  HG_LAUNCH_CHECK();
  hipLaunchKernelGGL(k_plane_sum_finish, dim3((C + 255) / 256), dim3(256), 0, st, (const float *)workspace, out, C, chunks);
  HG_LAUNCH_CHECK();
  return HG_OK;
}

static int demod_style_splits(int N) {
  int ns = (N + 63) / 64;
  return ns > 64 ? 64 : (ns < 1 ? 1 : ns);
}

size_t hg_demod_style_grad_workspace_bytes(int32_t B, int32_t N, int32_t K) {
  if (B <= 0 || N <= 0 || K <= 0) return 0;
  return (size_t)demod_style_splits(N) * B * K * sizeof(float);
}

int hg_demod_style_grad(const float *gd, const float *d, const float *s1, const float *wsq, float *gy, int32_t B, int32_t N,
                        int32_t K, void *workspace, size_t workspace_bytes, void *stream) {
  if (!gd || !d || !s1 || !wsq || !gy || B <= 0 || N <= 0 || K <= 0) return HG_EINVAL;
  if (!workspace || workspace_bytes < hg_demod_style_grad_workspace_bytes(B, N, K)) return HG_EWORKSPACE;
  const int ns = demod_style_splits(N), rows_per = (N + ns - 1) / ns;
  const size_t lds = ((size_t)rows_per * DSG_LD + 4 * DSG_BT * 64) * sizeof(float);
  if (lds > 64 * 1024) return HG_EUNSUPPORTED;
  hipStream_t st = (hipStream_t)stream;
  hipLaunchKernelGGL(k_demod_style_grad, dim3((unsigned)((K + 63) / 64), (unsigned)ns), dim3(256), lds, st, gd, d, wsq,
                     (float *)workspace, B, N, K, rows_per);
  HG_LAUNCH_CHECK();
  const int BK = B * K;
  hipLaunchKernelGGL(k_demod_style_grad_finish, dim3((unsigned)((BK + 255) / 256)), dim3(256), 0, st,
                     (const float *)workspace, s1, gy, BK, ns);
  HG_LAUNCH_CHECK();
  return HG_OK;
}

int hg_demod_weight_term(const float *w, const float *gd, const float *d, const float *s1, float *gw, int32_t B,
                         int32_t N, int32_t K, int32_t taps, int32_t accumulate, void *stream) {
  if (!w || !gd || !d || !s1 || !gw || B <= 0 || N <= 0 || K <= 0 || taps <= 0) return HG_EINVAL;
  const size_t lds = (size_t)(K + B) * sizeof(float);
  if (lds > 64 * 1024) return HG_EUNSUPPORTED;
  hipLaunchKernelGGL(k_demod_weight_term, dim3((unsigned)N), dim3(256), lds, (hipStream_t)stream, w, gd, d, s1, gw, B, N,
                     K, taps, accumulate);
  HG_LAUNCH_CHECK();
  return HG_OK;
}

int hg_lrelu_bwd_channel_sum(const float *g, const float *out, float slope, float *gm, float *csum, int32_t B, int32_t C,
                             int32_t HW, void *workspace, size_t workspace_bytes, void *stream) {
  if (!g || !out || !gm || B <= 0 || C <= 0 || HW <= 0 || !(slope >= 0.f)) return HG_EINVAL;
  hipStream_t st = (hipStream_t)stream;
  const int chunks = plane_chunks(C, (long long)B * HW / 4);
  if (csum && (!workspace || workspace_bytes < (size_t)C * chunks * sizeof(float))) return HG_EWORKSPACE;
  hipLaunchKernelGGL(k_lrelu_bwd_csum, dim3(chunks, C), dim3(256), 0, st, g, out, gm, csum ? (float *)workspace : nullptr,
                     slope, B, C, HW);
  HG_LAUNCH_CHECK();
  if (csum) {
    hipLaunchKernelGGL(k_plane_sum_finish, dim3((C + 255) / 256), dim3(256), 0, st, (const float *)workspace, csum, C, chunks);
    HG_LAUNCH_CHECK();
  }
  return HG_OK;
}

int hg_diffgrad_step(float *p, const float *g, float *exp_avg, float *exp_avg_sq, float *prev_grad, int64_t n,
                     float lr, float beta1, float beta2, float eps, int32_t step, void *stream) {
  if (!p || !g || !exp_avg || !exp_avg_sq || !prev_grad || n <= 0 || step < 1) return HG_EINVAL;
  const double bc1 = 1.0 - pow((double)beta1, (double)step), bc2 = 1.0 - pow((double)beta2, (double)step);
  const float step_size = (float)((double)lr * sqrt(bc2) / bc1);
  hipLaunchKernelGGL(k_diffgrad, dim3(grid_for(n)), dim3(256), 0, (hipStream_t)stream, p, g, exp_avg, exp_avg_sq,
                     prev_grad, (long long)n, step_size, beta1, beta2, eps);
  HG_LAUNCH_CHECK();
  return HG_OK;
}

float hg_diffgrad_step_size(float lr, float beta1, float beta2, int32_t step) {
  const double bc1 = 1.0 - pow((double)beta1, (double)step), bc2 = 1.0 - pow((double)beta2, (double)step);
  return (float)((double)lr * sqrt(bc2) / bc1);
}

int hg_diffgrad_step_dev(float *p, const float *g, float *exp_avg, float *exp_avg_sq, float *prev_grad, int64_t n,
                         const float *step_size_dev, float beta1, float beta2, float eps, void *stream) {
  if (!p || !g || !exp_avg || !exp_avg_sq || !prev_grad || !step_size_dev || n <= 0) return HG_EINVAL;
  hipLaunchKernelGGL(k_diffgrad_dev, dim3(grid_for(n)), dim3(256), 0, (hipStream_t)stream, p, g, exp_avg, exp_avg_sq,
                     prev_grad, (long long)n, step_size_dev, beta1, beta2, eps);
  HG_LAUNCH_CHECK();
  return HG_OK;
}

int hg_ema_update(float *ma, const float *p, int64_t n, float beta, void *stream) {
  if (!ma || !p || n <= 0) return HG_EINVAL;
  hipLaunchKernelGGL(k_ema, dim3(grid_for(n)), dim3(256), 0, (hipStream_t)stream, ma, p, (long long)n, beta);
  HG_LAUNCH_CHECK();
  return HG_OK;
}

}
```

### histogan_amd/csrc/hg_wino.hip

```cpp
#include <cstdio>
#include <cstdlib>
#include <type_traits>
#include "hg_common.h"
#include "../../include/hg_hist.h"
#include "../../include/hg_conv.h"
#include "../../include/hg_wino.h"

namespace {

constexpr unsigned kOOB = 0xFFFFFFFFu;
__device__ __forceinline__ __amdgpu_buffer_rsrc_t make_rsrc(const float *base, unsigned bytes = kOOB) {
  return __builtin_amdgcn_make_buffer_rsrc(const_cast<float *>(base), 0, (int)bytes, 0x00020000);
}
__device__ __forceinline__ float buf_load(__amdgpu_buffer_rsrc_t r, unsigned voff, int soff) {
  return __builtin_bit_cast(float, __builtin_amdgcn_raw_buffer_load_b32(r, (int)voff, soff, 0));
}
__device__ __forceinline__ f32x2 buf_load2(__amdgpu_buffer_rsrc_t r, unsigned voff, int soff) {
  return __builtin_bit_cast(f32x2, __builtin_amdgcn_raw_buffer_load_b64(r, (int)voff, soff, 0));
}
__device__ __forceinline__ f32x4 buf_load4(__amdgpu_buffer_rsrc_t r, unsigned voff, int soff) {
  return __builtin_bit_cast(f32x4, __builtin_amdgcn_raw_buffer_load_b128(r, (int)voff, soff, 0));
}

struct WinoArgs {
  const float *in, *u;
  float *out;
  const float *iscale, *oscale, *bias, *addend, *noise_w, *noise_img;
  int noise_S;
  float slope;
  int B, K, N, H, W;
  int nblk, nch;
  int lTW, lTH, lNI;
  int tiles_w, tiles_h;
  int bt_x, bt_y;
  int ksplit;
  float *slab;
  int blocks, total_tiles;
  int xcd;
};

__device__ __forceinline__ int mrow(int r, int lk) { return (r & 3) + 8 * (r >> 2) + 4 * lk; }

template <int TC, int TP, int KC, bool FE>
__global__ __launch_bounds__(512) void k_wino(const WinoArgs a) {
  constexpr int NT = 512, NB = 32 * TC, TB = 32 * TP;
  static_assert(KC * TB == NT, "one (channel, tile) patch per thread and chunk");
  constexpr int NV = (KC / 2) * TC;
  static_assert(NV == 2 || NV % 4 == 0, "operand loads are 8 or 16 bytes");
  constexpr int VSZ = 16 * KC * TB;
  extern __shared__ float smem[];
  typedef std::integral_constant<int, 0> S0;
  typedef std::integral_constant<int, 1> S1;

  const int tid = threadIdx.x, lane = tid & 63, wave = tid >> 6;
  const int lm = lane & 31, lk = lane >> 5;
  const int H = a.H, W = a.W, K = a.K, N = a.N, HW = H * W;
  const int TWm = (1 << a.lTW) - 1, THm = (1 << a.lTH) - 1;
  const int t = tid % TB, kc = tid / TB;
  const size_t in_elems = (size_t)a.B * K * HW;
  const __amdgpu_buffer_rsrc_t ru = make_rsrc(a.u);
  const __amdgpu_buffer_rsrc_t rs = make_rsrc(FE && a.iscale ? a.iscale : a.u);
  const bool has_is = FE && a.iscale != nullptr;
  const int cps = (a.nch + a.ksplit - 1) / a.ksplit;

  int nb = 0, bx = 0, by = 0, b0 = 0, zs = 0, c_begin = 0, c_end = 0;
  const float *inblk = a.in;
  unsigned vo[4], so = kOOB, uo[2];
  bool c0bad = false, c3bad = false, sh1 = false;
  auto tile_setup = [&](int L) __attribute__((always_inline)) {
    int pt = L % a.blocks;
    zs = L / a.blocks;
    if (a.xcd) {
      const int q = pt & 7, r = pt >> 3;
      nb = r % a.nblk;
      pt = (r / a.nblk) * 8 + q;
    } else {
      nb = pt % a.nblk;
      pt /= a.nblk;
    }
    bx = pt % a.bt_x;
    pt /= a.bt_x;
    by = pt % a.bt_y;
    b0 = (pt / a.bt_y) << a.lNI;
    c_begin = zs * cps;
    c_end = c_begin + cps < a.nch ? c_begin + cps : a.nch;
    inblk = a.in + (size_t)b0 * K * HW;
    const int ttx = t & TWm, tty = (t >> a.lTW) & THm, timg = t >> (a.lTW + a.lTH);
    const int gtx = (bx << a.lTW) + ttx, gty = (by << a.lTH) + tty, b = b0 + timg;
    const bool ok = gtx < a.tiles_w && gty < a.tiles_h && b < a.B;
    const int x = 2 * gtx - 1, y0 = 2 * gty - 1;
    c0bad = x < 0;
    c3bad = x + 3 >= W;
    sh1 = ok && timg == 0 && kc == 0 && gty == 0 && gtx == 0;
#pragma unroll
    for (int r = 0; r < 4; ++r) {
      const int y = y0 + r;
      const bool rok = ok && (unsigned)y < (unsigned)H;
      const unsigned e = (unsigned)(((timg * K + kc) * H + y) * W + x);
      vo[r] = rok ? (r == 1 && sh1 ? 0u : e * 4u) : kOOB;
    }
    so = (FE && ok) ? (unsigned)(b * K + kc) * 4u : kOOB;
#pragma unroll
    for (int x2 = 0; x2 < 2; ++x2)
      uo[x2] = (unsigned)((((2 * wave + x2) * a.nblk + nb) * a.nch) * (NV * 64) + lane * (NV >= 4 ? 4 : 2)) * 4u;
  };

  f32x16 acc[2][TC][TP];
  float pd[2][16];
  float ps[2] = {1.f, 1.f};
  float ua[2][2][NV];

  auto load_patch = [&](int c, auto SET) __attribute__((always_inline)) {
    constexpr int S = decltype(SET)::value;
    const size_t rem = in_elems - ((size_t)b0 * K * HW + (size_t)c * KC * HW);
    const __amdgpu_buffer_rsrc_t rx = make_rsrc(inblk + (size_t)c * KC * HW, rem < (1ull << 30) ? (unsigned)rem * 4u : kOOB);
#pragma unroll
    for (int r = 0; r < 4; ++r) {
      const f32x4 m = buf_load4(rx, vo[r], 0);
#pragma unroll
      for (int e = 0; e < 4; ++e) pd[S][4 * r + e] = m[e];
    }
    if constexpr (FE) {
      if (has_is) ps[S] = buf_load(rs, so, c * KC * 4);
    }
  };
  auto load_u = [&](int c, auto SET) __attribute__((always_inline)) {
    constexpr int S = decltype(SET)::value;
// ... 57 lines not shown
      for (int j = 0; j < TP; ++j) bv[slot][j] = Vc[((2 * wave + x2) * KC + 2 * ks) * TB + 32 * j];
    };
    constexpr int DSN = (TP + 1) / 2;
    ldb(0, 0);
    __builtin_amdgcn_sched_group_barrier(0x100, DSN, 0);
#pragma unroll
    for (int st = 0; st < STEPS; ++st) {
      const int x2 = st / (KC / 2), ks = st % (KC / 2);
      if (st + 1 < STEPS) ldb(st + 1, (st + 1) & 1);
#pragma unroll
      for (int i = 0; i < TC; ++i)
#pragma unroll
        for (int j = 0; j < TP; ++j)
          acc[x2][i][j] = __builtin_amdgcn_mfma_f32_32x32x2f32(ua[S][x2][ks * TC + i], bv[st & 1][j], acc[x2][i][j], 0, 0, 0);
      if (st + 1 < STEPS) __builtin_amdgcn_sched_group_barrier(0x100, DSN, 0);
      __builtin_amdgcn_sched_group_barrier(0x008, TC * TP, 0);
    }
  };
  auto clampc = [&](int c) __attribute__((always_inline)) { return c < c_end ? c : c_end - 1; };
#define HG_WINO_BARRIER()               \
  __builtin_amdgcn_sched_barrier(0);    \
  __syncthreads();                      \
  __builtin_amdgcn_sched_barrier(0)

  int L = blockIdx.x;
  if (L < a.total_tiles) {
    tile_setup(L);
    if (c_begin < c_end) {
      load_patch(c_begin, S0{});
      load_u(c_begin, S0{});
    }
  }
  for (; L < a.total_tiles; L += gridDim.x) {
#pragma unroll
    for (int x2 = 0; x2 < 2; ++x2)
#pragma unroll
      for (int i = 0; i < TC; ++i)
#pragma unroll
        for (int j = 0; j < TP; ++j)
#pragma unroll
          for (int r = 0; r < 16; ++r) acc[x2][i][j][r] = 0.f;

    const int nc = c_end - c_begin;
    if (nc > 0) {
      load_patch(clampc(c_begin + 1), S1{});
      load_u(clampc(c_begin + 1), S1{});
      transform_store(0, S0{});
      HG_WINO_BARRIER();
      for (int c = c_begin; c + 1 < c_end; c += 2) {
        load_patch(clampc(c + 2), S0{});
        __builtin_amdgcn_sched_barrier(0);
        mfma_chunk(0, S0{});
        transform_store(1, S1{});
        load_u(clampc(c + 2), S0{});
        HG_WINO_BARRIER();
        load_patch(clampc(c + 3), S1{});
        __builtin_amdgcn_sched_barrier(0);
        mfma_chunk(1, S1{});
        transform_store(0, S0{});
        load_u(clampc(c + 3), S1{});
        HG_WINO_BARRIER();
      }
      if (nc & 1) mfma_chunk(0, S0{});
    }
    __builtin_amdgcn_sched_barrier(0);

    const int e_n0 = nb * NB, e_bx = bx, e_by = by, e_b0 = b0, e_zs = zs;
    if (L + (int)gridDim.x < a.total_tiles) {
      tile_setup(L + (int)gridDim.x);
      if (c_begin < c_end) {
        load_patch(c_begin, S0{});
        load_u(c_begin, S0{});
      }
    }
    __builtin_amdgcn_sched_barrier(0);

  const bool fin = a.ksplit == 1;
  float *ob = fin ? a.out : a.slab + (size_t)e_zs * a.B * N * HW;
  const int erow = tid >> 5, ecol = tid & 31;
  int etb[TP], ety[TP], etx[TP];
  bool eok[TP];
  float ebias[TC][2], enw[TC][2], eosc[TC][2][TP];
  f32x2 enz[TP][2];
#pragma unroll
  for (int j = 0; j < TP; ++j) {
    const int tl = 32 * j + ecol;
    const int ttx = tl & TWm, tty = (tl >> a.lTW) & THm, timg = tl >> (a.lTW + a.lTH);
    etx[j] = (e_bx << a.lTW) + ttx; ety[j] = (e_by << a.lTH) + tty; etb[j] = e_b0 + timg;
    eok[j] = etx[j] < a.tiles_w && ety[j] < a.tiles_h && etb[j] < a.B;
#pragma unroll
    for (int p2 = 0; p2 < 2; ++p2) {
      enz[j][p2] = f32x2{0.f, 0.f};
      if (fin && a.noise_img && eok[j])
        enz[j][p2] = *reinterpret_cast<const f32x2 *>(a.noise_img + ((size_t)etb[j] * a.noise_S + 2 * ety[j] + p2) * a.noise_S + 2 * etx[j]);
    }
  }
#pragma unroll
  for (int i = 0; i < TC; ++i)
#pragma unroll
    for (int h = 0; h < 2; ++h) {
      const int n = e_n0 + 32 * i + erow + 16 * h, nc_ = n < N ? n : N - 1;
      ebias[i][h] = (fin && a.bias) ? a.bias[nc_] : 0.f;
      enw[i][h] = (fin && a.noise_img) ? a.noise_w[nc_] : 0.f;
#pragma unroll
      for (int j = 0; j < TP; ++j) eosc[i][h][j] = (fin && a.oscale && eok[j]) ? a.oscale[etb[j] * N + nc_] : 1.f;
    }
#pragma unroll
  for (int i = 0; i < TC; ++i) {
#pragma unroll
    for (int j = 0; j < TP; ++j) {
      f32x2 ead[2][2];
#pragma unroll
      for (int h = 0; h < 2; ++h)
#pragma unroll
        for (int p2 = 0; p2 < 2; ++p2) {
          ead[h][p2] = f32x2{0.f, 0.f};
          const int n = e_n0 + 32 * i + erow + 16 * h;
          if (fin && a.addend && eok[j] && n < N)
            ead[h][p2] = *reinterpret_cast<const f32x2 *>(a.addend + (((size_t)etb[j] * N + n) * H + 2 * ety[j] + p2) * W + 2 * etx[j]);
        }
      __syncthreads();
#pragma unroll
      for (int x2 = 0; x2 < 2; ++x2)
#pragma unroll
        for (int r = 0; r < 16; ++r) smem[((2 * wave + x2) * 32 + mrow(r, lk)) * 32 + lm] = acc[x2][i][j][r];
      __syncthreads();
#pragma unroll
      for (int h = 0; h < 2; ++h) {
        const int row = erow + 16 * h;
        const int n = e_n0 + 32 * i + row;
        float m[16];
#pragma unroll
        for (int e = 0; e < 16; ++e) m[e] = smem[(e * 32 + row) * 32 + ecol];
        if (!eok[j] || n >= N) continue;
        float s0[4], s1[4];
#pragma unroll
        for (int c = 0; c < 4; ++c) {
          s0[c] = m[c] + m[4 + c] + m[8 + c];
          s1[c] = m[4 + c] - m[8 + c] - m[12 + c];
        }
        float y[2][2];
        y[0][0] = s0[0] + s0[1] + s0[2];
        y[0][1] = s0[1] - s0[2] - s0[3];
        y[1][0] = s1[0] + s1[1] + s1[2];
        y[1][1] = s1[1] - s1[2] - s1[3];
        const size_t o = (((size_t)etb[j] * N + n) * H + 2 * ety[j]) * W + 2 * etx[j];
        if (fin) {
#pragma unroll
          for (int p2 = 0; p2 < 2; ++p2)
#pragma unroll
            for (int q = 0; q < 2; ++q) {
              float v = fmaf(y[p2][q], eosc[i][h][j], fmaf(enw[i][h], enz[j][p2][q], ebias[i][h])) + ead[h][p2][q];
              if (a.slope > 0.f) v = v > 0.f ? v : a.slope * v;
              y[p2][q] = v;
            }
        }
        *reinterpret_cast<f32x2 *>(ob + o) = f32x2{y[0][0], y[0][1]};
        *reinterpret_cast<f32x2 *>(ob + o + W) = f32x2{y[1][0], y[1][1]};
      }
    }
  }
    __syncthreads();
  }
#undef HG_WINO_BARRIER
}

__global__ __launch_bounds__(256) void k_wino_reduce(const float *__restrict__ slab, float *__restrict__ out,
                                                     const float *__restrict__ oscale, const float *__restrict__ bias,
                                                     const float *__restrict__ noise_w, const float *__restrict__ noise_img,
                                                     const float *__restrict__ addend, int noise_S, float slope,
                                                     long long total4, int HW, int W, int N, int ksplit) {
  const size_t total = (size_t)total4 * 4;
  for (long long i4 = (long long)blockIdx.x * 256 + threadIdx.x; i4 < total4; i4 += (long long)gridDim.x * 256) {
    f32x4 v = {0.f, 0.f, 0.f, 0.f};
    for (int z = 0; z < ksplit; ++z) v += *reinterpret_cast<const f32x4 *>(slab + (size_t)z * total + (size_t)i4 * 4);
    const long long i = i4 * 4;
    const long long bn = i / HW;
    const int n = (int)(bn % N);
    const float bs = bias ? bias[n] : 0.f, osc = oscale ? oscale[bn] : 1.f, nw = noise_img ? noise_w[n] : 0.f;
    f32x4 nz = {0.f, 0.f, 0.f, 0.f};
    if (noise_img) {
      const int p = (int)(i - bn * HW), y = p / W, x = p - y * W;
#pragma unroll
      for (int e = 0; e < 4; ++e) {
        const int xe = x + e, ye = y + xe / W;
        nz[e] = noise_img[((size_t)(bn / N) * noise_S + ye) * noise_S + xe % W];
      }
    }
    f32x4 ad = {0.f, 0.f, 0.f, 0.f};
    if (addend) ad = *reinterpret_cast<const f32x4 *>(addend + i);
#pragma unroll
    for (int e = 0; e < 4; ++e) {
      float r = fmaf(v[e], osc, fmaf(nw, nz[e], bs)) + ad[e];
      if (slope > 0.f) r = r > 0.f ? r : slope * r;
      v[e] = r;
    }
    *reinterpret_cast<f32x4 *>(out + i) = v;
  }
}

template <int TC, int KC>
__device__ __forceinline__ void wino_pack_slot(const float *__restrict__ w, float *__restrict__ u, int Co, int Ci, int nblk,
                                               int nch, int mode, int ch, int nb, int tid ,
                                               float *__restrict__ wsq = nullptr) {
  constexpr int NV = (KC / 2) * TC, NB = 32 * TC;
  int e, lane;
  if constexpr (NV >= 4) {
    e = (tid >> 8) * 4 + (tid & 3);
    lane = (tid >> 2) & 63;
  } else {
    e = tid & 1;
    lane = tid >> 1;
  }
  const int ks = e / TC, i = e % TC, lm = lane & 31, lk = lane >> 5;
  const int k = ch * KC + 2 * ks + lk, n = nb * NB + 32 * i + lm;
  const int K = mode == HG_CONV_PACK_FWD ? Ci : Co, N = mode == HG_CONV_PACK_FWD ? Co : Ci;
  float g[9];
#pragma unroll
  for (int q = 0; q < 9; ++q) g[q] = 0.f;
  if (k < K && n < N) {
    const float *p = w + (mode == HG_CONV_PACK_FWD ? ((size_t)n * Ci + k) : ((size_t)k * Ci + n)) * 9;
#pragma unroll
    for (int q = 0; q < 9; ++q) g[q] = p[q];
    if (wsq != nullptr && mode == HG_CONV_PACK_FWD) {
      float q2 = 0.f;
#pragma unroll
      for (int q = 0; q < 9; ++q) q2 = fmaf(g[q], g[q], q2);
      wsq[(size_t)n * Ci + k] = q2;
    }
  }
  float gg[4][3];
#pragma unroll
  for (int c = 0; c < 3; ++c) {
    gg[0][c] = g[c];
    gg[1][c] = 0.5f * (g[c] + g[3 + c] + g[6 + c]);
    gg[2][c] = 0.5f * (g[c] - g[3 + c] + g[6 + c]);
    gg[3][c] = g[6 + c];
  }
  float uu[4][4];
#pragma unroll
  for (int r = 0; r < 4; ++r) {
    uu[r][0] = gg[r][0];
    uu[r][1] = 0.5f * (gg[r][0] + gg[r][1] + gg[r][2]);
    uu[r][2] = 0.5f * (gg[r][0] - gg[r][1] + gg[r][2]);
    uu[r][3] = gg[r][2];
  }
  const size_t xstride = (size_t)nblk * nch * (NV * 64);
  float *dst = u + ((size_t)nb * nch + ch) * (NV * 64) + tid;
#pragma unroll
  for (int r = 0; r < 4; ++r)
#pragma unroll
    for (int c = 0; c < 4; ++c) {
      const int rr = mode == HG_CONV_PACK_FWD ? r : (r == 0 ? 3 : (r == 3 ? 0 : r));
      const int cc = mode == HG_CONV_PACK_FWD ? c : (c == 0 ? 3 : (c == 3 ? 0 : c));
      dst[(size_t)(4 * r + c) * xstride] = uu[rr][cc];
    }
}

struct PackGeom {
  int variant, nblk, nch, blocks;
};
__host__ __device__ inline PackGeom pack_geom(int Co, int Ci, int mode, int force_variant) {
  const int K = mode == HG_CONV_PACK_FWD ? Ci : Co, N = mode == HG_CONV_PACK_FWD ? Co : Ci;
  PackGeom g;
  g.variant = force_variant >= 0 ? force_variant : (N <= 32 ? 1 : 0);
  const int NB = g.variant ? 32 : 64, KC = g.variant ? 4 : 8;
  g.nblk = (N + NB - 1) / NB;
  g.nch = K / KC;
  g.blocks = (K % KC) ? 0 : (g.variant ? ((g.nch + 3) / 4) * g.nblk : g.nch * g.nblk);
  return g;
}
__device__ __forceinline__ void wino_pack_block(const float *w, float *u, int Co, int Ci, int mode, const PackGeom &g, int local,
                                                float *wsq = nullptr) {
  if (g.variant == 0) {
    wino_pack_slot<2, 8>(w, u, Co, Ci, g.nblk, g.nch, mode, local % g.nch, local / g.nch, threadIdx.x, wsq);
  } else {
    const int cg = (g.nch + 3) / 4;
// ... 286 lines not shown
inline int force_variant() {
  static const int force = getenv("HG_WINO_VARIANT") ? atoi(getenv("HG_WINO_VARIANT")) : -1;
  return force;
}
inline int variant_of(int N) { return force_variant() >= 0 ? force_variant() : (N <= 32 ? 1 : 0); }
struct WinoPlan {
  int variant, NB, TB, KC, nblk, nch;
  int lTW, lTH, lNI, tiles_w, tiles_h, bt_x, bt_y, groups;
  int ksplit;
  long long blocks;
};
inline bool make_plan(int B, int K, int N, int H, int W, WinoPlan &p) {
  if (B <= 0 || K <= 0 || N <= 0 || H < 2 || W < 2 || (H & 1) || (W & 1)) return false;
  p.variant = variant_of(N);
  p.NB = p.variant ? 32 : 64;
  p.TB = p.variant ? 128 : 64;
  p.KC = p.variant ? 4 : 8;
  if (K % p.KC) return false;
  p.nblk = (N + p.NB - 1) / p.NB;
  p.nch = K / p.KC;
  p.tiles_w = W / 2;
  p.tiles_h = H / 2;
  const int lTB = ceil_log2(p.TB);
  p.lTW = ceil_log2(p.tiles_w);
  if (p.lTW > 4) p.lTW = 4;
  p.lTH = ceil_log2(p.tiles_h);
  if (p.lTH > lTB - p.lTW) p.lTH = lTB - p.lTW;
  p.lNI = lTB - p.lTW - p.lTH;
  p.bt_x = (p.tiles_w + (1 << p.lTW) - 1) >> p.lTW;
  p.bt_y = (p.tiles_h + (1 << p.lTH) - 1) >> p.lTH;
  p.groups = (B + (1 << p.lNI) - 1) >> p.lNI;
  p.blocks = (long long)p.nblk * p.bt_x * p.bt_y * p.groups;
  if ((long long)(1 << p.lNI) * K * H * W >= (1LL << 30)) return false;
  if (16LL * p.nblk * p.nch * ((p.KC / 2) * (p.NB / 32) * 64) >= (1LL << 30)) return false;
  if ((long long)B * N * H * W >= (1LL << 31) || (long long)B * K * H * W >= (1LL << 31)) return false;
  static const int force_ks = getenv("HG_WINO_KSPLIT") ? atoi(getenv("HG_WINO_KSPLIT")) : 0;
  const int cus = num_cus();
  int best = 1;
  double best_t = 1e300;
  for (int ks = 1; ks <= 16; ++ks) {
    if (ks > 1 && p.nch / ks < 8) break;
    const long long rounds = (p.blocks * ks + cus - 1) / cus;
    double t = (double)rounds * ((p.nch + ks - 1) / ks + 6);
    if (ks > 1) t += 4.0 + 0.02 * ks * rounds;
    if (t < best_t * 0.97) { best_t = t; best = ks; }
  }
  p.ksplit = force_ks > 0 ? (force_ks < p.nch ? force_ks : p.nch) : best;
  return true;
}

struct WgPlan {
  int lPW, lPH, lPI, lcg, lrg, nchunks, ktiles, ntiles, splits;
  size_t slab_bytes;
};
inline bool is_pow2(int v) { return v > 0 && (v & (v - 1)) == 0; }
inline bool make_wg_plan(int B, int K, int N, int H, int W, WgPlan &p) {
  if (B <= 0 || K <= 0 || N <= 0 || H < 2 || W < 2 || (H & 1) || (W & 1)) return false;
  const int tw = W / 2, th = H / 2;
  if (!is_pow2(tw) || !is_pow2(th)) return false;
  const int ltw = ceil_log2(tw), lth = ceil_log2(th);
  p.lPW = ltw < 3 ? ltw : 3;
  p.lPH = lth < 3 - p.lPW ? lth : 3 - p.lPW;
  p.lPI = 3 - p.lPW - p.lPH;
  p.lcg = ltw - p.lPW;
  p.lrg = lth - p.lPH;
  const int igroups = (B + (1 << p.lPI) - 1) >> p.lPI;
  const long long nch = (long long)igroups << (p.lcg + p.lrg);
  if (nch > (1 << 30)) return false;
  p.nchunks = (int)nch;
  p.ktiles = (K + 63) / 64;
  p.ntiles = (N + 63) / 64;
  if ((long long)((1 << p.lPI) * (K > N ? K : N) + 1) * H * W >= (1LL << 30)) return false;
  const int tiles = p.ktiles * p.ntiles, cus = num_cus();
  static const int force = getenv("HG_WINO_WG_SPLITS") ? atoi(getenv("HG_WINO_WG_SPLITS")) : 0;
  int s = tiles >= cus ? 1 : (cus + tiles - 1) / tiles;
  if (force > 0) s = force;
  if (s > p.nchunks) s = p.nchunks;
  if (s < 1) s = 1;
  p.splits = s;
  p.slab_bytes = (size_t)s * 16 * (p.ntiles * 64) * (p.ktiles * 64) * sizeof(float);
  return true;
}

template <int TC, int TP, int KC>
int launch_wino(const WinoArgs &a, const WinoPlan &p, bool fe, hipStream_t st) {
  auto kern = fe ? k_wino<TC, TP, KC, true> : k_wino<TC, TP, KC, false>;
  constexpr size_t lds = 2 * 16 * KC * 32 * TP * sizeof(float);
  static bool attr[kMaxDev][2] = {};
  const int dev = cur_dev();
  if (!attr[dev][fe]) {
    hipError_t e = hipFuncSetAttribute((const void *)kern, hipFuncAttributeMaxDynamicSharedMemorySize, (int)lds);
    if (e != hipSuccess) return (int)e;
    attr[dev][fe] = true;
  }
  const long long total = p.blocks * a.ksplit;
  static const int persist = getenv("HG_WINO_PERSIST") ? atoi(getenv("HG_WINO_PERSIST")) : 1;
  const long long grid = persist && total > num_cus() ? num_cus() : total;
  hipLaunchKernelGGL(kern, dim3((unsigned)grid), dim3(512), lds, st, a);
  HG_LAUNCH_CHECK();
  return HG_OK;
}

}

extern "C" {

int hg_wino_supported(int32_t B, int32_t K, int32_t N, int32_t H, int32_t W) {
  WinoPlan p;
  if (!make_plan(B, K, N, H, W, p)) return 0;
  constexpr int kMinK = 32;
  if (K < kMinK) return 0;
  return p.blocks * p.ksplit >= num_cus() / 2;
}

size_t hg_wino_packed_elems(int32_t Co, int32_t Ci, int32_t mode) {
  if (Co <= 0 || Ci <= 0 || (mode != HG_CONV_PACK_FWD && mode != HG_CONV_PACK_DGRAD)) return 0;
  const PackGeom g = pack_geom(Co, Ci, mode, force_variant());
  if (!g.blocks) return 0;
  return (size_t)16 * g.nblk * g.nch * (g.variant ? 128 : 512);
}

int hg_wino_pack_weights(const float *w, float *u, int32_t Co, int32_t Ci, int32_t mode, void *stream) {
  if (!w || !u || !hg_wino_packed_elems(Co, Ci, mode)) return HG_EINVAL;
  const PackGeom g = pack_geom(Co, Ci, mode, force_variant());
  hipLaunchKernelGGL(k_wino_pack, dim3((unsigned)g.blocks), dim3(512), 0, (hipStream_t)stream, w, u, Co, Ci, mode, force_variant());
  HG_LAUNCH_CHECK();
  return HG_OK;
}

int32_t hg_wino_pack_blocks(int32_t Co, int32_t Ci, int32_t want_fwd, int32_t want_dgrad) {
  if (Co <= 0 || Ci <= 0) return 0;
  return (want_fwd ? pack_geom(Co, Ci, HG_CONV_PACK_FWD, force_variant()).blocks : 0) +
         (want_dgrad ? pack_geom(Co, Ci, HG_CONV_PACK_DGRAD, force_variant()).blocks : 0);
}

int hg_wino_pack_weights_multi(const hg_wino_pack_item *items_dev, int32_t n_items, int32_t total_blocks, void *stream) {
  if (!items_dev || n_items <= 0 || total_blocks <= 0) return HG_EINVAL;
  hipLaunchKernelGGL(k_wino_pack_multi, dim3((unsigned)total_blocks), dim3(512), 0, (hipStream_t)stream, items_dev, n_items,
                     force_variant());
  HG_LAUNCH_CHECK();
  return HG_OK;
}

size_t hg_wino_workspace_bytes(int32_t B, int32_t K, int32_t N, int32_t H, int32_t W) {
  WinoPlan p;
  if (!make_plan(B, K, N, H, W, p) || p.ksplit == 1) return 0;
  return (size_t)p.ksplit * B * N * H * W * sizeof(float);
}

int hg_wino_conv2d(const float *in, const float *u, float *out, const float *iscale, const float *oscale,
                   const float *bias, const float *noise_w, const float *noise_img, int32_t noise_S, float lrelu_slope,
                   const float *addend, int32_t B, int32_t K, int32_t N, int32_t H, int32_t W, void *workspace,
                   size_t workspace_bytes, void *stream) {
  if (!in || !u || !out) return HG_EINVAL;
  if ((noise_img != nullptr) != (noise_w != nullptr) || lrelu_slope < 0.f) return HG_EINVAL;
  if (noise_img && (noise_S < H || noise_S < W || (noise_S & 1))) return HG_EINVAL;
  if (addend && (iscale || oscale || noise_img || lrelu_slope > 0.f)) return HG_EINVAL;
  WinoPlan p;
  if (!make_plan(B, K, N, H, W, p)) return HG_EUNSUPPORTED;
  if (p.ksplit > 1 && (!workspace || workspace_bytes < (size_t)p.ksplit * B * N * H * W * sizeof(float))) p.ksplit = 1;
  WinoArgs a;
  a.in = in; a.u = u; a.out = out; a.iscale = iscale; a.oscale = oscale; a.bias = bias; a.addend = addend;
  a.noise_w = noise_w; a.noise_img = noise_img; a.noise_S = noise_S; a.slope = lrelu_slope;
  a.B = B; a.K = K; a.N = N; a.H = H; a.W = W;
  a.nblk = p.nblk; a.nch = p.nch; a.lTW = p.lTW; a.lTH = p.lTH; a.lNI = p.lNI;
  a.tiles_w = p.tiles_w; a.tiles_h = p.tiles_h; a.bt_x = p.bt_x; a.bt_y = p.bt_y;
  a.ksplit = p.ksplit; a.slab = (float *)workspace;
  a.blocks = (int)p.blocks; a.total_tiles = (int)(p.blocks * p.ksplit);
  a.xcd = p.nblk > 1 && p.nblk < 8 && (p.blocks / p.nblk) % 8 == 0;
  hipStream_t st = (hipStream_t)stream;
  const bool fe = iscale != nullptr;
  int rc = p.variant == 0 ? launch_wino<2, 2, 8>(a, p, fe, st) : launch_wino<1, 4, 4>(a, p, fe, st);
  if (rc) return rc;
  if (p.ksplit > 1) {
    const long long total = (long long)B * N * H * W;
    long long nb = (total / 4 + 255) / 256;
    if (nb > 4096) nb = 4096;
    hipLaunchKernelGGL(k_wino_reduce, dim3((unsigned)nb), dim3(256), 0, st, a.slab, out, oscale, bias, noise_w, noise_img,
                       addend, noise_S, lrelu_slope, total / 4, H * W, W, N, p.ksplit);
    HG_LAUNCH_CHECK();
  }
  return HG_OK;
}

size_t hg_wino_wgrad_workspace_bytes(int32_t B, int32_t K, int32_t N, int32_t H, int32_t W) {
  WgPlan p;
  if (!make_wg_plan(B, K, N, H, W, p)) return 0;
  return p.slab_bytes;
}

int hg_wino_wgrad_supported(int32_t B, int32_t K, int32_t N, int32_t H, int32_t W) {
  WgPlan p;
  if (!make_wg_plan(B, K, N, H, W, p)) return 0;
  constexpr int kMinChannels = 64, kMinSide = 4;
  if (K < kMinChannels || N < kMinChannels || H < kMinSide || W < kMinSide) return 0;
  return p.nchunks / p.splits >= 4;
}

int hg_wino_wgrad(const float *in, const float *gout, float *gw, int32_t B, int32_t K, int32_t N, int32_t H, int32_t W,
                  void *workspace, size_t workspace_bytes, void *stream) {
  if (!in || !gout || !gw || !workspace) return HG_EINVAL;
  WgPlan p;
  if (!make_wg_plan(B, K, N, H, W, p)) return HG_EUNSUPPORTED;
  if (workspace_bytes < p.slab_bytes) return HG_EWORKSPACE;
  WinoWgArgs a;
  a.in = in; a.gout = gout; a.slab = (float *)workspace;
  a.B = B; a.K = K; a.N = N; a.H = H; a.W = W;
  a.ktiles = p.ktiles; a.splits = p.splits; a.nchunks = p.nchunks;
  a.lPW = p.lPW; a.lPH = p.lPH; a.lPI = p.lPI; a.lcg = p.lcg; a.lrg = p.lrg;
  a.Np = p.ntiles * 64; a.Kp = p.ktiles * 64;
  hipStream_t st = (hipStream_t)stream;
  constexpr size_t lds = 4 * (size_t)WG_OP * sizeof(float);
  static bool attr[kMaxDev] = {};
  const int dev = cur_dev();
  if (!attr[dev]) {
    hipError_t e = hipFuncSetAttribute((const void *)k_wino_wgrad, hipFuncAttributeMaxDynamicSharedMemorySize, (int)lds);
    if (e != hipSuccess) return (int)e;
    attr[dev] = true;
  }
  a.xtiles = p.ktiles * p.ntiles; a.total_blocks = a.xtiles * p.splits;
  a.xcd = p.splits % 8 == 0;
  static const int persist = getenv("HG_WINO_PERSIST") ? atoi(getenv("HG_WINO_PERSIST")) : 1;
  const int grid = persist && a.total_blocks > num_cus() ? num_cus() : a.total_blocks;
  hipLaunchKernelGGL(k_wino_wgrad, dim3((unsigned)grid), dim3(512), lds, st, a);
  HG_LAUNCH_CHECK();
  if (p.splits >= 16)
    hipLaunchKernelGGL(k_wino_wgrad_reduce<32>, dim3((unsigned)((a.Kp + 31) / 32), (unsigned)N), dim3(256), 0, st, a.slab, gw, N, K,
                       a.Np, a.Kp, p.splits);
  else if (p.splits >= 4)
    hipLaunchKernelGGL(k_wino_wgrad_reduce<8>, dim3((unsigned)((a.Kp + 127) / 128), (unsigned)N), dim3(256), 0, st, a.slab, gw, N, K,
                       a.Np, a.Kp, p.splits);
  else
    hipLaunchKernelGGL(k_wino_wgrad_reduce<1>, dim3((unsigned)((a.Kp + 1023) / 1024), (unsigned)N), dim3(256), 0, st, a.slab, gw, N,
                       K, a.Np, a.Kp, p.splits);
  HG_LAUNCH_CHECK();
  return HG_OK;
}

}
```

### histogan_amd/nets.py

```python
import os
from math import log2

import torch
import torch.nn.functional as F
from torch import nn

from . import ops
from .conv import conv2d, conv2d_add, conv2d_lrelu, conv2d_same

EPS = 1e-8


def leaky_relu(p=0.2):
    return nn.LeakyReLU(p, inplace=True)


class Flatten(nn.Module):
    def forward(self, x):
        return x.reshape(x.shape[0], -1)


def _noise_t(inoise):
    nzt = getattr(inoise, '_hg_nzt', None)
    if nzt is None:
        nzt = inoise[..., 0].transpose(1, 2).contiguous()
        try:
            inoise._hg_nzt = nzt
        except Exception:
            pass
    return nzt


PHASE_HOOK = None
_aux_streams = {}


def aux_stream(device):
    st = _aux_streams.get(device.index)
    if st is None:
        st = _aux_streams[device.index] = torch.cuda.Stream(device=device)
    return st


class Conv2DMod(nn.Module):
    def __init__(self, in_chan, out_chan, kernel, demod=True, stride=1, dilation=1, **kwargs):
        super().__init__()
        self.filters = out_chan
        self.demod = demod
        self.kernel = kernel
        self.stride = stride
        self.dilation = dilation
        self.weight = nn.Parameter(torch.randn((out_chan, in_chan, kernel, kernel)))
        nn.init.kaiming_normal_(self.weight, a=0, mode='fan_in', nonlinearity='leaky_relu')

    def _get_same_padding(self, size, kernel, dilation, stride):
        return ((size - 1) * (stride - 1) + dilation * (kernel - 1)) // 2

    def demod_coeff(self, y):
        return ops.demod_coeff(y, self.weight)

    def contract(self, x, y, upsample=False):
        if self.stride != 1:
            raise NotImplementedError('Conv2DMod: stride != 1 is not used by HistoGAN and not implemented')
        xm = ops.modulate(x, y, upsample)
        if self.dilation == 1 and self.kernel in (1, 3):
            return conv2d_same(xm, self.weight)
        raise NotImplementedError('Conv2DMod: only 1x1 / 3x3, dilation 1 (all HistoGAN uses) is implemented')

    def forward(self, x, y):
        c = self.contract(x, y)
        if self.demod:
            c = c * self.demod_coeff(y)[:, :, None, None]
        return c


class RGBBlock(nn.Module):
    def __init__(self, latent_dim, input_channel, upsample, rgba=False):
        super().__init__()
        self.input_channel = input_channel
        self.to_style = nn.Linear(latent_dim, input_channel)
        out_filters = 3 if not rgba else 4
        self.conv = Conv2DMod(input_channel, out_filters, 1, demod=False)
        self.upsample = nn.Upsample(scale_factor=2, mode='bilinear', align_corners=False) if upsample else None

    def forward(self, x, prev_rgb, istyle):
        return self.forward_(x, prev_rgb, self.to_style(istyle))

    def forward_(self, x, prev_rgb, style):
        if (not self.conv.demod and self.conv.kernel == 1 and self.conv.stride == 1 and self.conv.dilation == 1
# ... 110 lines not shown
                if gfused.supported(self, t, nzt):
                    return gfused.generator_train(self, t, nzt)
                if gfused.supported(self, t, nzt, train=False):
                    return gfused.generator_infer(self, t, nzt)
            for i, block in enumerate(self.blocks):
                x, rgb = block.forward_(x, rgb, t[3 * i], t[3 * i + 1], t[3 * i + 2], inoise=input_noise)
            return rgb
        if styles.is_cuda and not torch.is_grad_enabled() and not torch.cuda.is_current_stream_capturing():
            main, aux = torch.cuda.current_stream(styles.device), aux_stream(styles.device)
            aux.wait_event(main.record_event())
            ahead = []
            with torch.cuda.stream(aux):
                for style, block in zip(styles, self.blocks):
                    t = (block.to_style1(style), block.to_style2(style), block.to_rgb.to_style(style))
                    ahead.append((t, aux.record_event()))
            for (t, ev), block in zip(ahead, self.blocks):
                main.wait_event(ev)
                for u in t:
                    u.record_stream(main)
                x, rgb = block.forward_(x, rgb, t[0], t[1], t[2], inoise=input_noise)
            styles.record_stream(aux)
            return rgb
        for style, block in zip(styles, self.blocks):
            x, rgb = block(x, rgb, style, input_noise)
        return rgb


class HistVectorizer(nn.Module):
    def __init__(self, insize, emb, depth):
        super().__init__()
        self.flatten = Flatten()
        fc_layers = []
        for i in range(depth):
            if i == 0:
                fc_layers.extend([nn.Linear(insize * insize * 3, emb * 2), leaky_relu()])
            elif i == 1:
                fc_layers.extend([nn.Linear(emb * 2, emb), leaky_relu()])
            else:
                fc_layers.extend([nn.Linear(emb, emb), leaky_relu()])
        self.fcs = nn.Sequential(*fc_layers)

    def forward(self, x):
        x = self.flatten(x)
        if x.is_cuda and ops.SKINNY_SPLIT and len(self.fcs) >= 2 and x.shape[0] <= 64:
            fc = self.fcs[0]
            h = ops._skinny_mm(x.contiguous(), fc.weight, True)
            if fc.bias is not None:
                h = h + fc.bias
            return self.fcs[1:](h)
        return self.fcs(x)


class StyleVectorizer(nn.Module):
    def __init__(self, emb, depth):
        super().__init__()
        layers = []
        for i in range(depth):
            layers.extend([nn.Linear(emb, emb), leaky_relu()])
        self.net = nn.Sequential(*layers)

    def forward(self, x):
        return self.net(x)


class Conv2d(nn.Conv2d):

    def forward(self, x):
        k = self.kernel_size[0]
        if (self.kernel_size[0] != self.kernel_size[1] or self.padding != (k // 2, k // 2) or self.dilation != (1, 1)
                or self.groups != 1 or self.stride[0] != self.stride[1] or self.padding_mode != 'zeros'):
            raise NotImplementedError('Conv2d: only square 1x1/3x3, padding k//2, stride 1/2, dilation 1, groups 1')
        return conv2d(x, self.weight, self.bias, self.stride[0])


class DiscriminatorBlock(nn.Module):
    def __init__(self, input_channels, filters, downsample=True):
        super().__init__()
        self.conv_res = Conv2d(input_channels, filters, 1)
        self.net = nn.Sequential(Conv2d(input_channels, filters, 3, padding=1), leaky_relu(),
                                 Conv2d(filters, filters, 3, padding=1), leaky_relu())
        self.downsample = Conv2d(filters, filters, 3, padding=1, stride=2) if downsample else None

    def forward(self, x):
        h = conv2d_lrelu(x, self.net[0].weight, self.net[0].bias, 0.2)
        h = conv2d_lrelu(h, self.net[2].weight, self.net[2].bias, 0.2)
        x = conv2d_add(x, self.conv_res.weight, self.conv_res.bias, h)
        if self.downsample is not None:
            x = self.downsample(x)
        return x


class Residual(nn.Module):
    def __init__(self, fn):
        super().__init__()
        self.fn = fn

    def forward(self, x):
        return self.fn(x) + x


class Rezero(nn.Module):
    def __init__(self, fn):
        super().__init__()
        self.fn = fn
        self.g = nn.Parameter(torch.zeros(1))

    def forward(self, x):
        return self.fn(x) * self.g


class ImageLinearAttention(nn.Module):

    def __init__(self, chan, chan_out=None, kernel_size=1, padding=0, stride=1, key_dim=64, value_dim=64, heads=8,
                 norm_queries=True):
        super().__init__()
        if kernel_size != 1 or padding != 0 or stride != 1:
            raise NotImplementedError('ImageLinearAttention: only the 1x1 projections HistoGAN uses')
        self.chan = chan
        chan_out = chan if chan_out is None else chan_out
        self.key_dim, self.value_dim, self.heads, self.norm_queries = key_dim, value_dim, heads, norm_queries
        self.to_q = Conv2d(chan, key_dim * heads, 1)
        self.to_k = Conv2d(chan, key_dim * heads, 1)
        self.to_v = Conv2d(chan, value_dim * heads, 1)
        self.to_out = Conv2d(value_dim * heads, chan_out, 1)

    def forward(self, x, context=None):
        if context is not None:
            raise NotImplementedError('ImageLinearAttention: cross-attention context is not used by HistoGAN')
        b, c, h, w = x.shape
        heads = self.heads
        q, k, v = self.to_q(x), self.to_k(x), self.to_v(x)
        q, k, v = (t.reshape(b, heads, -1, h * w) for t in (q, k, v))
        q, k = (t * (self.key_dim ** -0.25) for t in (q, k))
        k = k.softmax(dim=-1)
        if self.norm_queries:
            q = q.softmax(dim=-2)
        context = torch.einsum('bhdn,bhen->bhde', k, v)
        out = torch.einsum('bhdn,bhde->bhen', q, context)
        return self.to_out(out.reshape(b, -1, h, w))


class PermuteToFrom(nn.Module):
    def __init__(self, fn):
        super().__init__()
        self.fn = fn

    def forward(self, x):
        out, loss = self.fn(x.permute(0, 2, 3, 1))
        return out.permute(0, 3, 1, 2), loss


class VectorQuantize(nn.Module):

    def __init__(self, dim, n_embed, decay=0.8, commitment=1., eps=1e-5):
        super().__init__()
        self.dim, self.n_embed, self.decay, self.commitment, self.eps = dim, n_embed, decay, commitment, eps
        embed = torch.randn(dim, n_embed)
        self.register_buffer('embed', embed)
        self.register_buffer('cluster_size', torch.zeros(n_embed))
        self.register_buffer('embed_avg', embed.clone())

    def forward(self, input):
        flatten = input.reshape(-1, self.dim)
        dist = flatten.pow(2).sum(1, keepdim=True) - 2 * flatten @ self.embed + self.embed.pow(2).sum(0, keepdim=True)
        embed_ind = (-dist).max(1)[1]
        quantize = F.embedding(embed_ind.view(*input.shape[:-1]), self.embed.transpose(0, 1))
        if self.training:
            with torch.no_grad():
                onehot = F.one_hot(embed_ind, self.n_embed).type(input.dtype)
# ... 53 lines not shown
```

### histogan_amd/trainer.py

```python
import json
import os
import sys
from math import floor, log2
from pathlib import Path
from random import random
from shutil import rmtree
from time import perf_counter

import numpy as np
import torch
import torch.nn.functional as F
from torch import nn
from torch.autograd import grad as torch_grad

from . import ddp
from .augment import AugWrapper
from .conv import drain_pack_streams, enable_pack_cache, input_grads_only, prepack_async, weights_changed
from .hist import hellinger_loss
from .nets import Discriminator, Generator, HistVectorizer, StyleVectorizer
from .optim import DiffGrad, FlatParams, conv_first, ema_update

EPS = 1e-8
EXTS = ['jpg', 'png']
G_OVERLAP_DDP = os.environ.get('HG_G_OVERLAP_DDP', 'auto')
GRAPH_MODE = os.environ.get('HG_GRAPH', 'auto')
GRAPH_AUTO_RATIO = float(os.environ.get('HG_GRAPH_AUTO_RATIO', '0.9'))
GRAPH_GP = os.environ.get('HG_GRAPH_GP', '1') != '0'
EARLY_GREDUCE = os.environ.get('HG_EARLY_GREDUCE', '1') != '0'
LAZY_STATS = os.environ.get('HG_LAZY_STATS', '1') != '0'


def _lazy_field(name):
    key = '_stat_' + name

    def get(self):
        if self.__dict__.get('_pending'):
            self._drain(0, in_train=False)
        try:
            return self.__dict__[key]
        except KeyError:
            raise AttributeError(name) from None

    def set_(self, v):
        self.__dict__[key] = v
    return property(get, set_)


def _cat_batches(a, b):
    if a.requires_grad or b.requires_grad or a.shape[1:] != b.shape[1:] or a.dtype != b.dtype:
        return torch.cat((a, b), dim=0)
    out = torch.empty((a.shape[0] + b.shape[0],) + tuple(a.shape[1:]), dtype=a.dtype, device=a.device)
    out[:a.shape[0]].copy_(a)
    out[a.shape[0]:].copy_(b)
    return out


class NanException(Exception):
    pass


class EMA():
    def __init__(self, beta):
        super().__init__()
        self.beta = beta

    def update_average(self, old, new):
        if old is None:
            return new
        return old * self.beta + (1 - self.beta) * new


def _freeze_gc_once(owner):
    if not getattr(owner, '_gc_frozen', False):
        import gc
        gc.collect()
        gc.freeze()
        owner._gc_frozen = True


def default(value, d):
    return d if value is None else value


def cast_list(el):
    return el if isinstance(el, list) else [el]


def is_empty(t):
    if isinstance(t, torch.Tensor):
        return t.nelement() == 0
    return t is None


def set_requires_grad(model, bool):
    for p in model.parameters():
        p.requires_grad = bool


def gradient_penalty(images, output, weight=10):
    batch_size = images.shape[0]
    with input_grads_only():
        gradients = torch_grad(outputs=output, inputs=images, grad_outputs=torch.ones_like(output),
                               create_graph=True, retain_graph=True, only_inputs=True)[0]
    gradients = gradients.reshape(batch_size, -1)
    return weight * ((gradients.norm(2, dim=1) - 1) ** 2).mean()


class _Rng:

    def __init__(self, device, mode='device'):
        self.device, self.mode = device, mode
# ... 389 lines not shown
        GAN._reduce_g.finish()
        weights_changed()

    def _device_step(self, alpha, apply_gradient_penalty, apply_path_penalty, gs=None):
        GAN = self.GAN
        dev = self.device
        zero = lambda: torch.zeros((), device=dev)
        mark = self._mark
        mark('start')
        total_disc_loss, total_gen_loss, total_hist_loss = zero(), zero(), zero()
        gp_val, q_val, pl_len = zero(), zero(), None

        batch_size = self.batch_size
        image_size = GAN.G.image_size
        latent_dim = GAN.G.latent_dim
        num_layers = GAN.G.num_layers
        Disc = GAN.D
        acc = self.gradient_accumulate_every
        has_vq = any(q is not None for q in Disc.quantize_blocks)
        aug = (lambda im, detach=False: GAN.D_aug.augment(im, prob=self.aug_prob, types=self.aug_types, detach=detach)
               ) if self.aug_prob > 0.0 else (lambda im, detach=False: im)

        def w_and_hw_static(tt_key, hist_batch):
            w_styles = self._latents_static(gs[tt_key], batch_size, num_layers - 2, latent_dim)
            h_w_space = torch.unsqueeze(GAN.H(hist_batch), dim=1)
            return w_styles, torch.cat((h_w_space, h_w_space), dim=1)

        def g_forward():
            if gs is None:
                style = get_latents_fn(batch_size, num_layers - 2, latent_dim)
                noise = self.rng.image_noise(batch_size, image_size)
                hist_batch = next(self.loader)['histograms'].to(dev)
                w_styles, h_w_space = self._w_and_hw(style, hist_batch)
            else:
                hist_batch = gs['hist_g']
                w_styles, h_w_space = w_and_hw_static('tt_g', hist_batch)
                noise = self.rng.image_noise(batch_size, image_size)
            return noise, hist_batch, w_styles, h_w_space, GAN.G(w_styles, h_w_space, noise)

        if not ddp.is_dist():
            ddp_ok = True
        elif G_OVERLAP_DDP in ('0', '1'):
            ddp_ok = G_OVERLAP_DDP == '1'
        else:
            ddp_ok = not ddp.ranks_share_a_device(dev)
        overlap_g = acc == 1 and ddp_ok
        self._extra_streams_ok = ddp_ok
        if overlap_g and not getattr(self, '_warn_off', False):
            fn = getattr(torch.autograd.graph, 'set_warn_on_accumulate_grad_stream_mismatch', None)
            if fn is not None:
                fn(False)
            self._warn_off = True
        early = None

        GAN.D_opt.zero_grad()
        for i in range(acc):
            if gs is None:
                get_latents_fn = self.rng.mixed_list if random() < self.mixed_prob else self.rng.noise_list
                style = get_latents_fn(batch_size, num_layers - 2, latent_dim)
                noise = self.rng.image_noise(batch_size, image_size)
                batch = next(self.loader)
                image_batch = batch['images'].to(dev).detach().requires_grad_(apply_gradient_penalty)
                hist_batch = batch['histograms'].to(dev)
            else:
                get_latents_fn = None
                image_batch, hist_batch = gs['images'], gs['hist_d']
                if apply_gradient_penalty:
                    image_batch = image_batch.detach().requires_grad_(True)
            with torch.no_grad():
                if gs is None:
                    w_styles, h_w_space = self._w_and_hw(style, hist_batch)
                else:
                    w_styles, h_w_space = w_and_hw_static('tt_d', hist_batch)
                    noise = self.rng.image_noise(batch_size, image_size)
                generated_images = GAN.G(w_styles, h_w_space, noise)
            mark('d_phase_g_forward')
            if overlap_g:
                main = torch.cuda.current_stream(dev)
                side2 = self._g_stream()
                side2.wait_event(main.record_event())
                with torch.cuda.stream(side2):
                    early = g_forward()
            if has_vq or apply_gradient_penalty:
                fake_output, fake_q_loss = Disc(aug(generated_images, True))
                real_output, real_q_loss = Disc(aug(image_batch))
            else:
                both_output, both_q_loss = Disc(_cat_batches(aug(generated_images, True), aug(image_batch)))
                fake_output, real_output = both_output[:batch_size], both_output[batch_size:]
                fake_q_loss = real_q_loss = both_q_loss * 0.5
            mark('d_forward')
            divergence = (F.relu(1 + real_output) + F.relu(1 - fake_output)).mean()
            quantize_loss = (fake_q_loss + real_q_loss).mean()
            q_val = quantize_loss.detach()
            disc_loss = divergence + quantize_loss
            if apply_gradient_penalty:
                gp = gradient_penalty(image_batch, real_output)
                gp_val = gp.detach()
                disc_loss = disc_loss + gp
            disc_loss = disc_loss / acc
            disc_loss.backward()
            mark('d_backward')
            total_disc_loss += divergence.detach() / acc
        GAN._reduce_d.start()

        GAN.G_opt.zero_grad()
        set_requires_grad(Disc, False)
        try:
            total_gen_loss, total_hist_loss, pl_len = self._g_phase(
                alpha, apply_path_penalty, gs, early, g_forward, aug, total_gen_loss, total_hist_loss)
        finally:
            set_requires_grad(Disc, True)
        if ddp.is_dist():
            GAN._reduce_g.start()
            GAN.G_opt.step_buckets(GAN._reduce_g)
        else:
            GAN._reduce_g()
            GAN.G_opt.step()
        prepack_async(GAN._flat_g.data)
        mark('g_optimizer')

        return torch.stack([total_disc_loss, total_gen_loss, total_hist_loss, gp_val.reshape(()),
                            q_val.reshape(()), pl_len if pl_len is not None else zero()]).double()

    def _g_phase(self, alpha, apply_path_penalty, gs, early, g_forward, aug, total_gen_loss, total_hist_loss):
        GAN, dev, Disc, acc = self.GAN, self.device, self.GAN.D, self.gradient_accumulate_every
        pl_len = None
        d_updated = False
        def update_d():
            if ddp.is_dist():
                GAN.D_opt.step_buckets(GAN._reduce_d)
            else:
                GAN._reduce_d.finish()
                GAN.D_opt.step()

        if early is not None:
            update_d()
            d_updated = True
        for i in range(acc):
            if early is not None:
                torch.cuda.current_stream(dev).wait_stream(self._g_stream())
                for t in early:
                    t.record_stream(torch.cuda.current_stream(dev))
                noise, hist_batch, w_styles, h_w_space, generated_images = early
                early = None
            else:
                noise, hist_batch, w_styles, h_w_space, generated_images = g_forward()
            if not d_updated:
                update_d()
                d_updated = True
            self._mark('g_forward_joined_d_updated')
            fake_output, _ = Disc(aug(generated_images))
            self._mark('g_phase_d_forward')
            if self.hist_alpha_weight:
                generated_histograms = self.histBlock(generated_images, pre_relu=True,
                                                      weight=_alpha_weight(generated_images))
            else:
                generated_histograms = self.histBlock(generated_images, pre_relu=True)
            histogram_loss = hellinger_loss(hist_batch, generated_histograms, alpha)
            loss = fake_output.mean()
            gen_loss = loss + histogram_loss
            if apply_path_penalty:
                std = 0.1 / (ddp.batch_std(w_styles) + EPS)
                w_styles_2 = w_styles + self.rng.randn_like(w_styles) / (std + EPS)
                pl_images = GAN.G(w_styles_2, h_w_space, noise)
                pl_lengths = ((pl_images - generated_images) ** 2).mean(dim=(1, 2, 3))
                pl_len = pl_lengths.detach().mean()
                if not is_empty(self.pl_mean):
                    pl_loss = ((pl_lengths - self.pl_mean) ** 2).mean()
                    if not bool(torch.isnan(pl_loss)):
                        gen_loss = gen_loss + pl_loss
            gen_loss = gen_loss / acc
            self._mark('g_phase_d_forward_hist_loss')
            early_reduce = (EARLY_GREDUCE and self.__dict__.get('_extra_streams_ok', True) and ddp.is_dist()
                            and acc == 1 and not apply_path_penalty
                            and not torch.cuda.is_current_stream_capturing())
            if early_reduce:
                from . import gfused
                gfused.AFTER_BLOCKS = self._early_g_reduce
            try:
                gen_loss.backward()
            finally:
                if early_reduce:
                    gfused.AFTER_BLOCKS = None
            self._mark('g_backward')
            total_gen_loss = total_gen_loss + loss.detach() / acc
            total_hist_loss = total_hist_loss + histogram_loss.detach() / acc
        return total_gen_loss, total_hist_loss, pl_len

    def train(self, alpha=2):
        assert self.loader is not None, ('You must first initialize the data source with '
                                         '`.set_data_src(<folder of images>)` or `.set_synthetic_data_src()`')
        torch.autograd.set_detect_anomaly(False)
        if self.GAN is None:
            self.init_GAN()
        if self._nan_checkpoint is not None:
            self._raise_nan(self._nan_checkpoint)
        GAN = self.GAN
        GAN.train()
        _freeze_gc_once(self)
        t_host0 = perf_counter()
        apply_gradient_penalty = self.steps % 4 == 0
        apply_path_penalty = self.steps % 32 == 0
        graphed = self._graph_eligible(apply_gradient_penalty, apply_path_penalty)
        try:
            if graphed:
                stats = self._graphed_step(alpha, apply_gradient_penalty)
            else:
                stats = self._device_step(alpha, apply_gradient_penalty, apply_path_penalty, None)
        except NanException:
            raise
        except Exception:
            if self.GAN is not None:
                self._reset_after_failed_step()
            raise

        self.host_enqueue_ms = (perf_counter() - t_host0) * 1e3
        self.last_step_graphed = bool(graphed) and self.graph_mode != '2' and not getattr(self, '_graph_failed', False)
        self._t_host0 = t_host0

        if ddp.is_dist():
            nan_flag = torch.isnan(stats[:4]).any().double().reshape(1)
            packed = torch.cat([stats, nan_flag * ddp.world_size()])
            torch.distributed.all_reduce(packed, op=torch.distributed.ReduceOp.SUM)
            packed /= ddp.world_size()
        else:
            packed = torch.cat([stats, torch.zeros(1, dtype=stats.dtype, device=stats.device)])
        host = self._host_buffer()
        host.copy_(packed, non_blocking=True)
        ev = torch.cuda.Event(enable_timing=True)
        ev.record()
        checkpoint_num = floor(self.steps / self.save_every)
        self._pending.append((ev, host, dict(step=self.steps, gp=apply_gradient_penalty, pl=apply_path_penalty,
                                             checkpoint=checkpoint_num, host_ms=self.host_enqueue_ms,
                                             prev_ev=self.__dict__.get('_last_step_ev'),
# ... 187 lines not shown
```

### include/hg_conv.h

```cpp
#ifndef HG_CONV_H
#define HG_CONV_H

#include <stddef.h>
#include <stdint.h>

#ifdef __cplusplus
extern "C" {
#endif

#define HG_CONV_PACK_FWD 0
#define HG_CONV_PACK_DGRAD 1

size_t hg_conv_packed_elems(int32_t Co, int32_t Ci, int32_t ksize, int32_t mode);
int hg_conv_pack_weights(const float *w, float *wt, int32_t Co, int32_t Ci, int32_t ksize, int32_t mode,
                         void *stream);

int hg_conv_pack_weights_both(const float *w, float *wt_fwd, float *wt_dgrad, int32_t Co, int32_t Ci, int32_t ksize,
                              void *stream);

int hg_conv2d_fwd(const float *in, const float *wt, float *out, const float *iscale, const float *oscale,
                  const float *bias, int32_t B, int32_t K, int32_t N, int32_t Hi, int32_t Wi, int32_t ksize,
                  int32_t stride, void *workspace, size_t workspace_bytes, void *stream);

int hg_conv2d_fwd_add(const float *in, const float *wt, float *out, const float *addend, const float *bias, int32_t B,
                      int32_t K, int32_t N, int32_t Hi, int32_t Wi, int32_t ksize, int32_t stride, void *workspace,
                      size_t workspace_bytes, void *stream);

int hg_modconv2d_fwd(const float *in, const float *wt, float *out, const float *iscale, const float *oscale,
                     const float *bias, const float *noise_w, const float *noise_img, int32_t noise_S,
                     float lrelu_slope, int32_t B, int32_t K, int32_t N, int32_t H, int32_t W, int32_t ksize,
                     void *workspace, size_t workspace_bytes, void *stream);

size_t hg_conv2d_workspace_bytes(int32_t B, int32_t K, int32_t N, int32_t Hi, int32_t Wi, int32_t ksize,
                                 int32_t stride, int32_t dgrad);

typedef struct hg_pack_item {
  const float *w;
  float *wt_fwd, *wt_dgrad;
  int32_t Co, Ci, ksize, block_begin;
  float *wsq;
} hg_pack_item;
int32_t hg_conv_pack_blocks(int32_t Co, int32_t Ci);
int hg_conv_pack_weights_multi(const hg_pack_item *items_dev, int32_t n_items, int32_t total_blocks, void *stream);

int hg_conv2d_plan(int32_t B, int32_t K, int32_t N, int32_t Hi, int32_t Wi, int32_t ksize, int32_t stride, int32_t dgrad,
                   int32_t out[5]);

int hg_conv2d_dgrad(const float *gout, const float *wt, float *gin, const float *iscale, const float *oscale,
                    int32_t B, int32_t K, int32_t N, int32_t Hi, int32_t Wi, int32_t ksize, int32_t stride,
                    void *workspace, size_t workspace_bytes, void *stream);

size_t hg_conv2d_wgrad_workspace_bytes(int32_t B, int32_t K, int32_t N, int32_t Hi, int32_t Wi, int32_t ksize,
                                       int32_t stride);
int hg_conv2d_wgrad(const float *in, const float *gout, float *gw, const float *iscale, const float *gscale,
                    int32_t B, int32_t K, int32_t N, int32_t Hi, int32_t Wi, int32_t ksize, int32_t stride,
                    void *workspace, size_t workspace_bytes, void *stream);

#ifdef __cplusplus
}
#endif
#endif
```

### include/hg_nets.h

```cpp
#ifndef HG_NETS_H
#define HG_NETS_H

#include <stddef.h>
#include <stdint.h>

#ifdef __cplusplus
extern "C" {
#endif

int hg_modulate_fwd(const float *x, const float *s, float *out, int32_t B, int32_t C, int32_t H, int32_t W,
                    int32_t upsample, void *stream);
int hg_modulate_bwd(const float *gout, const float *x, const float *s, float *gx, float *gs, int32_t B,
                    int32_t C, int32_t H, int32_t W, int32_t upsample, void *workspace, size_t workspace_bytes,
                    void *stream);

int hg_torgb_fwd(const float *x, const float *s, const float *w, const float *prev, float *out, int32_t B, int32_t O,
                 int32_t C, int32_t HW, void *stream);
size_t hg_torgb_bwd_workspace_bytes(int32_t B, int32_t O, int32_t C, int32_t HW);
int hg_torgb_bwd(const float *g, const float *x, const float *s, const float *w, float *gx, float *gs, float *gw, int32_t B,
                 int32_t O, int32_t C, int32_t HW, void *workspace, size_t workspace_bytes, void *stream);

size_t hg_gstage_bwd_workspace_bytes(int32_t B, int32_t C, int32_t H, int32_t up);
int hg_gstage_bwd(const float *out, const float *ga, const float *sa, int32_t up, const float *g_rgb, const float *w_rgb,
                  const float *s_rgb, int32_t Cr, const float *d, const float *nzt, const float *wn, const float *bn, int32_t S,
                  float *gconv, float *gs_a, float *gs_rgb, float *gw_rgb, float *gd, float *gwn, float *gbn, int32_t B,
                  int32_t C, int32_t H, void *workspace, size_t workspace_bytes, void *stream);

size_t hg_nets_workspace_bytes(int32_t B, int32_t C, int32_t H, int32_t W);

int hg_demod_noise_lrelu_fwd(const float *conv, const float *d, const float *nzt, const float *wn,
                             const float *bn, float *out, int32_t B, int32_t O, int32_t H, int32_t S,
                             void *stream);
int hg_demod_noise_lrelu_bwd(const float *gout, const float *out, const float *conv, const float *d,
                             const float *nzt, const float *wn, const float *bn, float *gconv, float *gd,
                             float *gwn_part, float *gbn_part, int32_t B, int32_t O, int32_t H, int32_t S,
                             void *workspace, size_t workspace_bytes, void *stream);

int hg_channel_sum(const float *g, float *out, int32_t B, int32_t C, int32_t HW, void *workspace,
                   size_t workspace_bytes, void *stream);

int hg_lrelu_bwd_channel_sum(const float *g, const float *out, float slope, float *gm, float *csum, int32_t B, int32_t C,
                             int32_t HW, void *workspace, size_t workspace_bytes, void *stream);

size_t hg_demod_style_grad_workspace_bytes(int32_t B, int32_t N, int32_t K);
int hg_demod_style_grad(const float *gd, const float *d, const float *s1, const float *wsq, float *gy, int32_t B, int32_t N,
                        int32_t K, void *workspace, size_t workspace_bytes, void *stream);

int hg_demod_weight_term(const float *w, const float *gd, const float *d, const float *s1, float *gw, int32_t B,
                         int32_t N, int32_t K, int32_t taps, int32_t accumulate, void *stream);

int hg_diffgrad_step(float *p, const float *g, float *exp_avg, float *exp_avg_sq, float *prev_grad,
                     int64_t n, float lr, float beta1, float beta2, float eps, int32_t step, void *stream);

float hg_diffgrad_step_size(float lr, float beta1, float beta2, int32_t step);
int hg_diffgrad_step_dev(float *p, const float *g, float *exp_avg, float *exp_avg_sq, float *prev_grad, int64_t n,
                         const float *step_size_dev, float beta1, float beta2, float eps, void *stream);

int hg_ema_update(float *ma, const float *p, int64_t n, float beta, void *stream);

#ifdef __cplusplus
}
#endif
#endif
```

### include/hg_wino.h

```cpp
#ifndef HG_WINO_H
#define HG_WINO_H

#include <stddef.h>
#include <stdint.h>

#ifdef __cplusplus
extern "C" {
#endif

int hg_wino_supported(int32_t B, int32_t K, int32_t N, int32_t H, int32_t W);

size_t hg_wino_packed_elems(int32_t Co, int32_t Ci, int32_t mode);
int hg_wino_pack_weights(const float *w, float *u, int32_t Co, int32_t Ci, int32_t mode, void *stream);

typedef struct hg_wino_pack_item {
  const float *w;
  float *u_fwd, *u_dgrad;
  float *wsq;
  int32_t Co, Ci, block_begin, reserved;
} hg_wino_pack_item;
int32_t hg_wino_pack_blocks(int32_t Co, int32_t Ci, int32_t want_fwd, int32_t want_dgrad);
int hg_wino_pack_weights_multi(const hg_wino_pack_item *items_dev, int32_t n_items, int32_t total_blocks, void *stream);

size_t hg_wino_workspace_bytes(int32_t B, int32_t K, int32_t N, int32_t H, int32_t W);

int hg_wino_conv2d(const float *in, const float *u, float *out, const float *iscale, const float *oscale,
                   const float *bias, const float *noise_w, const float *noise_img, int32_t noise_S, float lrelu_slope,
                   const float *addend, int32_t B, int32_t K, int32_t N, int32_t H, int32_t W, void *workspace,
                   size_t workspace_bytes, void *stream);

int hg_wino_wgrad_supported(int32_t B, int32_t K, int32_t N, int32_t H, int32_t W);
size_t hg_wino_wgrad_workspace_bytes(int32_t B, int32_t K, int32_t N, int32_t H, int32_t W);
int hg_wino_wgrad(const float *in, const float *gout, float *gw, int32_t B, int32_t K, int32_t N, int32_t H, int32_t W,
                  void *workspace, size_t workspace_bytes, void *stream);

#ifdef __cplusplus
}
#endif
#endif
```

Before: 879.0 images/s.

## Fuse discriminator residual block backward with masked dgrad epilogues

Adds a custom autograd function for the discriminator residual block. Its backward fuses the leaky-ReLU mask, the residual-gradient addend and the per-channel bias sums into the dgrad conv epilogues, for both the Winograd and the direct kernels. A new head kernel computes the masked gradient and both bias sums in one pass. This removes separate elementwise and reduction kernels and their extra HBM round trips, at the cost of new kernel template variants and a first-order-only restriction, so the gradient-penalty pass keeps the old path.

```diff
diff --git a/histogan_amd/_lib.py b/histogan_amd/_lib.py
--- a/histogan_amd/_lib.py
+++ b/histogan_amd/_lib.py
@@ -91,6 +91,8 @@
     lib.hg_demod_noise_lrelu_bwd.argtypes = [vp, vp, vp, vp, vp, vp, vp, vp, vp, vp, vp, i32, i32, i32, i32, vp, sz, vp]
     lib.hg_lrelu_bwd_channel_sum.restype = ctypes.c_int
     lib.hg_lrelu_bwd_channel_sum.argtypes = [vp, vp, f32, vp, vp, i32, i32, i32, vp, sz, vp]
+    lib.hg_dblock_head.restype = ctypes.c_int
+    lib.hg_dblock_head.argtypes = [vp, vp, f32, vp, vp, vp, i32, i32, i32, vp, sz, vp]
     lib.hg_demod_style_grad_workspace_bytes.restype = ctypes.c_size_t
     lib.hg_demod_style_grad_workspace_bytes.argtypes = [i32, i32, i32]
     lib.hg_demod_style_grad.restype = ctypes.c_int
@@ -127,6 +129,10 @@
     lib.hg_conv2d_plan.argtypes = [i32, i32, i32, i32, i32, i32, i32, i32, ctypes.POINTER(ctypes.c_int32)]
     lib.hg_conv2d_dgrad.restype = ctypes.c_int
     lib.hg_conv2d_dgrad.argtypes = [vp, vp, vp, vp, vp, i32, i32, i32, i32, i32, i32, i32, vp, sz, vp]
+    lib.hg_conv2d_dgrad_masked_workspace_bytes.restype = sz
+    lib.hg_conv2d_dgrad_masked_workspace_bytes.argtypes = [i32, i32, i32, i32, i32, i32, i32]
+    lib.hg_conv2d_dgrad_masked.restype = ctypes.c_int
+    lib.hg_conv2d_dgrad_masked.argtypes = [vp, vp, vp, vp, vp, f32, vp, i32, i32, i32, i32, i32, i32, vp, sz, vp]
     lib.hg_conv2d_wgrad_workspace_bytes.restype = sz
     lib.hg_conv2d_wgrad_workspace_bytes.argtypes = [i32, i32, i32, i32, i32, i32, i32]
     lib.hg_conv2d_wgrad.restype = ctypes.c_int
@@ -164,6 +170,10 @@
     lib.hg_wino_workspace_bytes.argtypes = [i32, i32, i32, i32, i32]
     lib.hg_wino_conv2d.restype = ctypes.c_int
     lib.hg_wino_conv2d.argtypes = [vp, vp, vp, vp, vp, vp, vp, vp, i32, f32, vp, i32, i32, i32, i32, i32, vp, sz, vp]
+    lib.hg_wino_masked_workspace_bytes.restype = sz
+    lib.hg_wino_masked_workspace_bytes.argtypes = [i32, i32, i32, i32, i32, i32]
+    lib.hg_wino_conv2d_masked.restype = ctypes.c_int
+    lib.hg_wino_conv2d_masked.argtypes = [vp, vp, vp, vp, vp, f32, vp, i32, i32, i32, i32, i32, vp, sz, vp]
     lib.hg_wino_wgrad_supported.restype = ctypes.c_int
     lib.hg_wino_wgrad_supported.argtypes = [i32, i32, i32, i32, i32]
     lib.hg_wino_wgrad_workspace_bytes.restype = sz
@@ -205,6 +215,7 @@
            'hg_modulate_fwd', 'hg_modulate_bwd', 'hg_demod_noise_lrelu_fwd', 'hg_demod_noise_lrelu_bwd',
            'hg_diffgrad_step', 'hg_diffgrad_step_size', 'hg_diffgrad_step_dev', 'hg_ema_update', 'hg_nets_workspace_bytes', 'hg_channel_sum', 'hg_lrelu_bwd_channel_sum', 'hg_demod_weight_term', 'hg_demod_style_grad', 'hg_demod_style_grad_workspace_bytes',
            'hg_conv_packed_elems', 'hg_conv_pack_weights', 'hg_conv_pack_weights_both', 'hg_conv_pack_blocks', 'hg_conv_pack_weights_multi', 'hg_conv2d_fwd', 'hg_conv2d_fwd_add', 'hg_modconv2d_fwd', 'hg_conv2d_workspace_bytes', 'hg_conv2d_plan', 'hg_conv2d_dgrad',
+           'hg_conv2d_dgrad_masked_workspace_bytes', 'hg_conv2d_dgrad_masked', 'hg_wino_masked_workspace_bytes', 'hg_wino_conv2d_masked', 'hg_dblock_head',
            'hg_conv2d_wgrad_workspace_bytes',
            'hg_conv2d_wgrad',
            'hg_instnorm_workspace_bytes', 'hg_instnorm_lrelu_fwd', 'hg_instnorm_lrelu_bwd', 'hg_stencil3',
diff --git a/histogan_amd/conv.py b/histogan_amd/conv.py
--- a/histogan_amd/conv.py
+++ b/histogan_amd/conv.py
@@ -411,14 +411,17 @@
     return out
 
 
+def _nets_workspace(B, C, H, W, device):
+    return workspace(lib.hg_nets_workspace_bytes(B, C, H, W), device)
+
+
 def lrelu_bwd_channel_sum(g, out, slope, want_sum=True):
     g, out = f32c(g), f32c(out)
     B, C, H, W = g.shape
     with on_device(g.device):
         gm = torch.empty_like(g)
         cs = torch.empty(C, dtype=torch.float32, device=g.device) if want_sum else None
-        nb = lib.hg_nets_workspace_bytes(B, C, H, W)
-        ws = workspace(nb, g.device)
+        ws = _nets_workspace(B, C, H, W, g.device)
         check(lib.hg_lrelu_bwd_channel_sum(g.data_ptr(), out.data_ptr(), float(slope), gm.data_ptr(), ptr(cs), B, C, H * W,
                                            ws.data_ptr(), ws.numel(), stream_of(g)), 'hg_lrelu_bwd_channel_sum')
     return gm, cs
@@ -437,6 +440,38 @@
         check(lib.hg_conv2d_dgrad(g.data_ptr(), _direct_operand(wt).data_ptr(), gin.data_ptr(), ptr(iscale), ptr(oscale),
                                   B, K, N, H, W, ksize, stride, ptr(ws), nb, stream_of(g)), 'hg_conv2d_dgrad')
     return gin
+
+
+def conv_dgrad_masked_packed(g, wt, N, H, W, ksize, addend=None, mask_ref=None, slope=0.0, want_sum=False):
+    B, K = g.shape[:2]
+    with on_device(g.device):
+        gin = torch.empty((B, N, H, W), dtype=torch.float32, device=g.device)
+        cs = torch.empty(N, dtype=torch.float32, device=g.device) if want_sum else None
+        u = _wino_u(wt, PACK_DGRAD, B, K, N, H, W) if ksize == 3 else None
+        if u is not None:
+            nb = lib.hg_wino_masked_workspace_bytes(B, K, N, H, W, int(want_sum))
+            ws = torch.empty(nb, dtype=torch.uint8, device=g.device) if nb else None
+            check(lib.hg_wino_conv2d_masked(g.data_ptr(), u.data_ptr(), gin.data_ptr(), ptr(addend), ptr(mask_ref), float(slope),
+                                            ptr(cs), B, K, N, H, W, ptr(ws), nb, stream_of(g)), 'hg_wino_conv2d_masked')
+        else:
+            nb = lib.hg_conv2d_dgrad_masked_workspace_bytes(B, K, N, H, W, ksize, int(want_sum))
+            ws = torch.empty(nb, dtype=torch.uint8, device=g.device) if nb else None
+            check(lib.hg_conv2d_dgrad_masked(g.data_ptr(), _direct_operand(wt).data_ptr(), gin.data_ptr(), ptr(addend),
+                                             ptr(mask_ref), float(slope), ptr(cs), B, K, N, H, W, ksize, ptr(ws), nb,
+                                             stream_of(g)), 'hg_conv2d_dgrad_masked')
+    return gin, cs
+
+
+def dblock_head(g, out, slope, want_sums=True):
+    B, C, H, W = g.shape
+    with on_device(g.device):
+        gm = torch.empty_like(g)
+        cg = torch.empty(C, dtype=torch.float32, device=g.device) if want_sums else None
+        cm = torch.empty(C, dtype=torch.float32, device=g.device) if want_sums else None
+        ws = _nets_workspace(B, C, H, W, g.device)
+        check(lib.hg_dblock_head(g.data_ptr(), out.data_ptr(), float(slope), gm.data_ptr(), ptr(cg), ptr(cm), B, C, H * W,
+                                 ws.data_ptr(), ws.numel(), stream_of(g)), 'hg_dblock_head')
+    return gm, cg, cm
 
 
 def conv_wgrad(x, gout, ksize, stride=1, iscale=None, gscale=None, out=None):
@@ -719,6 +754,81 @@
         return gx, gw, gb, (g if ctx.needs_input_grad[3] else None), None
 
 
+_fused_dblock = False
+
+
+@contextlib.contextmanager
+def fused_dblock_backward(on=True):
+    global _fused_dblock
+    old, _fused_dblock = _fused_dblock, bool(on)
+    try:
+        yield
+    finally:
+        _fused_dblock = old
+
+
+def fused_dblock_active(x, w1):
+    return _fused_dblock and x.is_cuda and _batch_pieces(x, w1, 1) == 1
+
+
+class _DBlock(torch.autograd.Function):
+
+    @staticmethod
+    def forward(ctx, x, w1, b1, w2, b2, wr, br, slope):
+        for w in (w1, w2, wr):
+            _check_args(x, w, 1)
+        F_ = w1.shape[0]
+        if (x.shape[1] != w1.shape[1] or x.shape[1] != wr.shape[1] or w2.shape[0] != F_ or w2.shape[1] != F_
+                or wr.shape[0] != F_ or w1.shape[2] != 3 or w2.shape[2] != 3 or wr.shape[2] != 1):
+            raise ValueError(f'dblock: x {tuple(x.shape)} does not match the weights '
+                             f'{tuple(w1.shape)}, {tuple(w2.shape)}, {tuple(wr.shape)}')
+        xc = f32c(x)
+        fb = lambda b: None if b is None else f32c(b)
+        out1 = modconv_fwd_packed(xc, pack_weights(f32c(w1), PACK_FWD), F_, 3, bias=fb(b1), slope=slope)
+        out2 = modconv_fwd_packed(out1, pack_weights(f32c(w2), PACK_FWD), F_, 3, bias=fb(b2), slope=slope)
+        y = conv_fwd_add_packed(xc, pack_weights(f32c(wr), PACK_FWD), F_, 1, out2, fb(br), 1)
+        ctx.save_for_backward(x, w1, w2, wr, out1, out2)
+        ctx.has_bias = (b1 is not None, b2 is not None, br is not None)
+        ctx.slope = float(slope)
+        return y
+
+    @staticmethod
+    def backward(ctx, g):
+        if torch.is_grad_enabled():
+            raise RuntimeError('the fused discriminator-block backward is first-order only (create_graph=True / double '
+                               'backward): run this pass outside conv.fused_dblock_backward()')
+        x, w1, w2, wr, out1, out2 = ctx.saved_tensors
+        need = ctx.needs_input_grad
+        wg = not _skip_wgrad
+        want_b1 = wg and ctx.has_bias[0] and need[2]
+        want_b2 = wg and ctx.has_bias[1] and need[4]
+        want_br = wg and ctx.has_bias[2] and need[6]
+        gx = gw1 = gb1 = gw2 = gb2 = gwr = gbr = None
+        g = f32c(g)
+        B, Cin, H, W = x.shape
+        F_ = w1.shape[0]
+        gm2, cg, cm = dblock_head(g, out2, ctx.slope, want_b2 or want_br)
+        gb2 = cm if want_b2 else None
+        gbr = cg if want_br else None
+        if wg and need[5] and not _direct_wgrad(wr, x, g, 1):
+            gwr = conv_wgrad(f32c(x), g, 1, 1)
+        if wg and need[3] and not _direct_wgrad(w2, out1, gm2, 1):
+            gw2 = conv_wgrad(out1, gm2, 3, 1)
+        if need[0] or want_b1 or (wg and need[1]):
+            gm1, gb1 = conv_dgrad_masked_packed(gm2, pack_weights(f32c(w2), PACK_DGRAD), F_, H, W, 3, mask_ref=out1,
+                                                slope=ctx.slope, want_sum=want_b1)
+            if need[0]:
+                gx_res = conv_dgrad_packed(g, pack_weights(f32c(wr), PACK_DGRAD), Cin, H, W, 1)
+                gx, _ = conv_dgrad_masked_packed(gm1, pack_weights(f32c(w1), PACK_DGRAD), Cin, H, W, 3, addend=gx_res)
+            if wg and need[1] and not _direct_wgrad(w1, x, gm1, 1):
+                gw1 = conv_wgrad(f32c(x), gm1, 3, 1)
+        return gx, gw1, gb1, gw2, gb2, gwr, gbr, None
+
+
+def dblock(x, w1, b1, w2, b2, wr, br, slope=0.2):
+    return _DBlock.apply(x, w1, b1, w2, b2, wr, br, slope)
+
+
 _I32 = 2 ** 31 - 1
 
 
diff --git a/histogan_amd/csrc/hg_conv.hip b/histogan_amd/csrc/hg_conv.hip
--- a/histogan_amd/csrc/hg_conv.hip
+++ b/histogan_amd/csrc/hg_conv.hip
@@ -4,6 +4,7 @@
 #include "hg_common.h"
 #include "../../include/hg_hist.h"
 #include "../../include/hg_conv.h"
+#include "../../include/hg_nets.h"
 
 constexpr int kConvMinWaves = 2;
 constexpr int kConvKC = 4;
@@ -36,6 +37,11 @@
   int noise_S;
   float slope;
   Geom g;
+  const float *mask_ref = nullptr;
+  float mask_slope = 0.f;
+  float *csum_part = nullptr;
+  float *csum = nullptr;
+  size_t csum_part_bytes = 0;
 };
 
 __device__ __forceinline__ int fdiv(int e, float inv) {
@@ -74,7 +80,7 @@
   static __device__ __forceinline__ int row(int r, int lk) { return 4 * lk + r; }
 };
 
-template <int WC, int WP, int TC, int TP, int TAPS, int KC, int IS, bool SM, int MT, bool FE>
+template <int WC, int WP, int TC, int TP, int TAPS, int KC, int IS, bool SM, int MT, bool FE, bool DM = false>
 __device__ __forceinline__ void conv_body(const ConvArgs &a, const int bidx, const int bidy, const int bidz) {
   typedef MfmaTile<MT> M;
   constexpr int KS = M::KS;
@@ -256,7 +262,64 @@
 
   const int HWo = a.Ho * a.Wo;
   auto epilogue = [&](const bool fin) __attribute__((always_inline)) {
-  if constexpr (!FE) {
+  if constexpr (DM) {
+    static_assert(!FE, "the masked epilogue extends the plain one");
+    float cs[TC][M::NR];
+#pragma unroll
+    for (int i = 0; i < TC; ++i)
+#pragma unroll
+      for (int r = 0; r < M::NR; ++r) cs[i][r] = 0.f;
+    const float *__restrict__ pad_ = a.addend, *__restrict__ pmk_ = a.mask_ref;
+#pragma unroll
+    for (int j = 0; j < TP; ++j) {
+      const int p = (wp * TP + j) * MT + lm;
+      const int px = p & TWm, py = (p >> g.lTW) & THm, pi = p >> (g.lTW + g.lTH);
+      const int cx = x0 + px, cy = y0 + py, b = b0 + pi;
+      const bool pok = b < a.B && cy < a.Hc && cx < a.Wc;
+      const size_t pofs = pok ? ((size_t)b * N) * HWo + (cy * a.os + a.oy) * a.Wo + cx * a.os + a.ox : 0;
+#pragma unroll
+      for (int i = 0; i < TC; ++i) {
+#pragma unroll
+        for (int r = 0; r < M::NR; ++r) {
+          const int ch = n0 + (wc * TC + i) * MT + M::row(r, lk);
+          if (pok && ch < N) {
+            const size_t o = pofs + (size_t)ch * HWo;
+            float v = acc[i][j][r];
+            if (pad_) v += pad_[o];
+            if (pmk_) v = pmk_[o] > 0.f ? v : v * a.mask_slope;
+            a.out[o] = v;
+            cs[i][r] += v;
+          }
+        }
+      }
+    }
+    if (a.csum_part != nullptr) {
+#pragma unroll
+      for (int i = 0; i < TC; ++i)
+#pragma unroll
+        for (int r = 0; r < M::NR; ++r) {
+          float v = cs[i][r];
+#pragma unroll
+          for (int o = MT / 2; o > 0; o >>= 1) v += __shfl_xor(v, o, 64);
+          cs[i][r] = v;
+        }
+      static_assert(WP * NB <= 256, "the exchange fits the staging dump rows");
+      __syncthreads();
+      if (lm == 0) {
+#pragma unroll
+        for (int i = 0; i < TC; ++i)
+#pragma unroll
+          for (int r = 0; r < M::NR; ++r) smem[wp * NB + (wc * TC + i) * MT + M::row(r, lk)] = cs[i][r];
+      }
+      __syncthreads();
+      if (tid < NB && n0 + tid < N) {
+        float v = 0.f;
+#pragma unroll
+        for (int w = 0; w < WP; ++w) v += smem[w * NB + tid];
+        a.csum_part[(size_t)(n0 + tid) * gridDim.x + bidx] = v;
+      }
+    }
+  } else if constexpr (!FE) {
 #pragma unroll
     for (int j = 0; j < TP; ++j) {
       const int p = (wp * TP + j) * MT + lm;
@@ -323,9 +386,9 @@
   epilogue(a.ksplit == 1);
 }
 
-template <int WC, int WP, int TC, int TP, int TAPS, int KC, int IS, bool SM, int MT, bool FE>
+template <int WC, int WP, int TC, int TP, int TAPS, int KC, int IS, bool SM, int MT, bool FE, bool DM = false>
 __global__ __launch_bounds__(WC *WP * 64, kConvMinWaves) void k_conv(const ConvArgs a) {
-  conv_body<WC, WP, TC, TP, TAPS, KC, IS, SM, MT, FE>(a, blockIdx.x, blockIdx.y, blockIdx.z);
+  conv_body<WC, WP, TC, TP, TAPS, KC, IS, SM, MT, FE, DM>(a, blockIdx.x, blockIdx.y, blockIdx.z);
 }
 
 struct ConvArgs4 {
@@ -344,11 +407,13 @@
   else conv_body<WC, WP, TC, TP, 4, KC, 1, SM, MT, FE>(a.c[3], t, blockIdx.y, blockIdx.z);
 }
 
+template <bool DM>
 __global__ __launch_bounds__(256) void k_splitk_reduce(const float *__restrict__ slab, float *__restrict__ out,
                                                        const float *__restrict__ oscale, const float *__restrict__ bias,
                                                        const float *__restrict__ noise_w, const float *__restrict__ noise_img,
                                                        const float *__restrict__ addend, int noise_S, float slope,
-                                                       long long total, int HWo, int Wo, int N, int ksplit) {
+                                                       long long total, int HWo, int Wo, int N, int ksplit,
+                                                       const float *__restrict__ mask_ref, float mask_slope) {
   for (long long i = (long long)blockIdx.x * 256 + threadIdx.x; i < total; i += (long long)gridDim.x * 256) {
     float v = 0.f;
     for (int z = 0; z < ksplit; ++z) v += slab[(size_t)z * total + i];
@@ -362,8 +427,19 @@
     v = oscale ? fmaf(v, oscale[bn], add) : v + add;
     if (addend) v += addend[i];
     if (slope > 0.f) v = v > 0.f ? v : slope * v;
+    if constexpr (DM) {
+      if (mask_ref) v = mask_ref[i] > 0.f ? v : v * mask_slope;
+    }
     out[i] = v;
   }
+}
+
+__global__ __launch_bounds__(256) void k_csum_finish(const float *__restrict__ part, float *__restrict__ out, int N, int tiles) {
+  const int ch = blockIdx.x * 256 + threadIdx.x;
+  if (ch >= N) return;
+  float v = 0.f;
+  for (int t = 0; t < tiles; ++t) v += part[(size_t)ch * tiles + t];
+  out[ch] = v;
 }
 
 struct WgradArgs {
@@ -1017,13 +1093,23 @@
   bool inkernel_combine = false;
   (void)ws_bytes;
   const bool fe = a.iscale || a.oscale || a.noise_img || a.slope > 0.f;
+  const bool dm = (a.mask_ref || a.csum) && ksplit == 1;
+  if (dm && (fe || a.bias || !(IS == 1 && (TAPS == 9 || TAPS == 1)))) return HG_EUNSUPPORTED;
   auto kern = fe ? k_conv<WC, WP, TC, TP, TAPS, KC, IS, SM, MT, true> : k_conv<WC, WP, TC, TP, TAPS, KC, IS, SM, MT, false>;
-  static int state[2][2] = {{0, 0}, {0, 0}};
+  if constexpr (IS == 1 && (TAPS == 9 || TAPS == 1)) {
+    if (dm) kern = k_conv<WC, WP, TC, TP, TAPS, KC, IS, SM, MT, false, true>;
+  }
+  static int state[3][2] = {{0, 0}, {0, 0}, {0, 0}};
   const long long nwg = (long long)a.g.tiles_x * a.g.tiles_y * a.g.groups * ((a.N + NB - 1) / NB) * ksplit;
   char what[96];
-  snprintf(what, sizeof what, "k_conv<%d,%d,%d,%d,taps %d,kc %d,is %d,mt %d,fe %d>", WC, WP, TC, TP, TAPS, KC, IS, MT, (int)fe);
-  if (int rc = fit_blocks_per_cu((const void *)kern, NT, nwg, lds, state[fe], what)) return rc;
+  snprintf(what, sizeof what, "k_conv<%d,%d,%d,%d,taps %d,kc %d,is %d,mt %d,fe %d,dm %d>", WC, WP, TC, TP, TAPS, KC, IS, MT, (int)fe, (int)dm);
+  if (int rc = fit_blocks_per_cu((const void *)kern, NT, nwg, lds, state[dm ? 2 : fe], what)) return rc;
   unsigned gx = (unsigned)(a.g.tiles_x * a.g.tiles_y * a.g.groups);
+  if (dm && a.csum) {
+    if (!a.csum_part || a.csum_part_bytes < (size_t)a.N * gx * sizeof(float)) return HG_EWORKSPACE;
+  } else if (dm) {
+    a.csum_part = nullptr;
+  }
   if (inkernel_combine) {
     const unsigned ny = (unsigned)((a.N + NB - 1) / NB);
     unsigned m = 8;
@@ -1033,6 +1119,10 @@
   dim3 grid(gx, (unsigned)((a.N + NB - 1) / NB), (unsigned)ksplit);
   hipLaunchKernelGGL(kern, grid, dim3(NT), lds, st, a);
   HG_LAUNCH_CHECK();
+  if (dm && a.csum) {
+    hipLaunchKernelGGL(k_csum_finish, dim3((unsigned)((a.N + 255) / 256)), dim3(256), 0, st, a.csum_part, a.csum, a.N, (int)gx);
+    HG_LAUNCH_CHECK();
+  }
   if (ksplit > 1 && reduce && !inkernel_combine) return launch_splitk_reduce(a, ksplit, st);
   return HG_OK;
 }
@@ -1084,9 +1174,18 @@
   const long long total = (long long)a.B * a.N * a.Ho * a.Wo;
   long long nb = (total + 255) / 256;
   if (nb > 4096) nb = 4096;
-  hipLaunchKernelGGL(k_splitk_reduce, dim3((unsigned)nb), dim3(256), 0, st, a.slab, a.out, a.oscale, a.bias, a.noise_w,
-                     a.noise_img, a.addend, a.noise_S, a.slope, total, a.Ho * a.Wo, a.Wo, a.N, ksplit);
+  if (a.mask_ref)
+    hipLaunchKernelGGL(k_splitk_reduce<true>, dim3((unsigned)nb), dim3(256), 0, st, a.slab, a.out, a.oscale, a.bias, a.noise_w,
+                       a.noise_img, a.addend, a.noise_S, a.slope, total, a.Ho * a.Wo, a.Wo, a.N, ksplit, a.mask_ref,
+                       a.mask_slope);
+  else
+    hipLaunchKernelGGL(k_splitk_reduce<false>, dim3((unsigned)nb), dim3(256), 0, st, a.slab, a.out, a.oscale, a.bias, a.noise_w,
+                       a.noise_img, a.addend, a.noise_S, a.slope, total, a.Ho * a.Wo, a.Wo, a.N, ksplit, nullptr, 0.f);
   HG_LAUNCH_CHECK();
+  if (a.csum) {
+    const int rc = hg_channel_sum(a.out, a.csum, a.B, a.N, a.Ho * a.Wo, a.csum_part, a.csum_part_bytes, st);
+    if (rc) return rc;
+  }
   return HG_OK;
 }
 
@@ -1389,15 +1488,68 @@
                          1, workspace, workspace_bytes, stream);
 }
 
+static size_t dgrad_csum_bytes(const ConvPlan &p, int B, int N, int Hi, int Wi) {
+  const int mb = (p.tile == TILE_128x128 || p.tile == TILE_128x128_SM) ? 128 : p.tile == TILE_64x64 ? 64 : 256;
+  long long t = pixel_tiles(mb, B, Hi, Wi, 2), t4 = pixel_tiles(mb, B, Hi, Wi, 4);
+  if (t4 > t) t = t4;
+  if (t < 64) t = 64;
+  return (size_t)N * t * sizeof(float);
+}
+static size_t align256(size_t v) { return (v + 255) / 256 * 256; }
+static ConvPlan dgrad_plan(int B, int K, int N, int Hi, int Wi, int ksize) {
+  ConvPlan p = plan_conv(B, K, N, Hi, Wi, 1, 1, true, true, ksize * ksize);
+  if (!conv_ws_bytes(p, B, N, Hi, Wi)) p = plan_conv(B, K, N, Hi, Wi, 1, 1, false, true, ksize * ksize);
+  return p;
+}
+
+size_t hg_conv2d_dgrad_masked_workspace_bytes(int32_t B, int32_t K, int32_t N, int32_t Hi, int32_t Wi, int32_t ksize,
+                                              int32_t want_csum) {
+  if (!conv_args_ok(B, K, N, Hi, Wi, ksize, 1)) return 0;
+  const ConvPlan p = dgrad_plan(B, K, N, Hi, Wi, ksize);
+  const size_t slab = conv_ws_bytes(p, B, N, Hi, Wi);
+  return want_csum ? align256(slab) + dgrad_csum_bytes(p, B, N, Hi, Wi) : slab;
+}
+
+static int conv2d_dgrad_impl(const float *gout, const float *wt, float *gin, const float *iscale, const float *oscale,
+                             int32_t B, int32_t K, int32_t N, int32_t Hi, int32_t Wi, int32_t ksize, int32_t stride,
+                             void *workspace, size_t workspace_bytes, void *stream, const float *addend = nullptr,
+                             const float *mask_ref = nullptr, float mask_slope = 0.f, float *csum = nullptr);
+
 int hg_conv2d_dgrad(const float *gout, const float *wt, float *gin, const float *iscale, const float *oscale,
                     int32_t B, int32_t K, int32_t N, int32_t Hi, int32_t Wi, int32_t ksize, int32_t stride,
                     void *workspace, size_t workspace_bytes, void *stream) {
+  return conv2d_dgrad_impl(gout, wt, gin, iscale, oscale, B, K, N, Hi, Wi, ksize, stride, workspace, workspace_bytes, stream);
+}
+
+int hg_conv2d_dgrad_masked(const float *gout, const float *wt, float *gin, const float *addend, const float *mask_ref,
+                           float mask_slope, float *csum, int32_t B, int32_t K, int32_t N, int32_t Hi, int32_t Wi,
+                           int32_t ksize, void *workspace, size_t workspace_bytes, void *stream) {
+  if (!(mask_slope >= 0.f)) return HG_EINVAL;
+  if (csum && (!workspace || workspace_bytes < hg_conv2d_dgrad_masked_workspace_bytes(B, K, N, Hi, Wi, ksize, 1)))
+    return HG_EWORKSPACE;
+  return conv2d_dgrad_impl(gout, wt, gin, nullptr, nullptr, B, K, N, Hi, Wi, ksize, 1, workspace, workspace_bytes, stream,
+                           addend, mask_ref, mask_slope, csum);
+}
+
+static int conv2d_dgrad_impl(const float *gout, const float *wt, float *gin, const float *iscale, const float *oscale,
+                             int32_t B, int32_t K, int32_t N, int32_t Hi, int32_t Wi, int32_t ksize, int32_t stride,
+                             void *workspace, size_t workspace_bytes, void *stream, const float *addend,
+                             const float *mask_ref, float mask_slope, float *csum) {
   if (!gout || !wt || !gin || !conv_args_ok(B, K, N, Hi, Wi, ksize, stride)) return HG_EINVAL;
   if (!fits_i32(B, K, N, Hi, Wi)) return HG_EUNSUPPORTED;
   hipStream_t st = (hipStream_t)stream;
   ConvArgs a;
-  a.in = gout; a.wt = wt; a.out = gin; a.iscale = iscale; a.oscale = oscale; a.bias = nullptr; a.addend = nullptr;
+  a.in = gout; a.wt = wt; a.out = gin; a.iscale = iscale; a.oscale = oscale; a.bias = nullptr; a.addend = addend;
   a.noise_w = a.noise_img = nullptr; a.noise_S = 0; a.slope = 0.f;
+  a.mask_ref = mask_ref; a.mask_slope = mask_slope; a.csum = csum;
+  if (csum) {
+    const ConvPlan p = dgrad_plan(B, K, N, Hi, Wi, ksize);
+    a.csum_part_bytes = dgrad_csum_bytes(p, B, N, Hi, Wi);
+    const size_t front = align256(conv_ws_bytes(p, B, N, Hi, Wi));
+    a.csum_part = (float *)((char *)workspace + front);
+    workspace_bytes = front;
+    if (!front) workspace = nullptr;
+  }
   a.B = B; a.K = K; a.N = N;
   a.Hi = out_size(Hi, stride); a.Wi = out_size(Wi, stride);
   a.Ho = Hi; a.Wo = Wi;
diff --git a/histogan_amd/csrc/hg_nets.hip b/histogan_amd/csrc/hg_nets.hip
--- a/histogan_amd/csrc/hg_nets.hip
+++ b/histogan_amd/csrc/hg_nets.hip
@@ -350,6 +350,47 @@
   }
 }
 
+__global__ __launch_bounds__(256) void k_dblock_head(const float *__restrict__ g, const float *__restrict__ out,
+                                                     float *__restrict__ gm, float *__restrict__ part, float slope, int B,
+                                                     int C, int HW) {
+  __shared__ float sm[4];
+  const int c = blockIdx.y;
+  float ag = 0.f, am = 0.f;
+  const long long per = (long long)B * HW;
+  if ((HW & 3) == 0) {
+    const int hw4 = HW / 4;
+    for (long long e = (long long)blockIdx.x * 256 + threadIdx.x; e < per / 4; e += (long long)gridDim.x * 256) {
+      const long long b = e / hw4, p4 = e - b * hw4;
+      const size_t off = ((size_t)b * C + c) * HW;
+      const float4 v = reinterpret_cast<const float4 *>(g + off)[p4];
+      const float4 o = reinterpret_cast<const float4 *>(out + off)[p4];
+      float4 r;
+      r.x = o.x > 0.f ? v.x : v.x * slope; r.y = o.y > 0.f ? v.y : v.y * slope;
+      r.z = o.z > 0.f ? v.z : v.z * slope; r.w = o.w > 0.f ? v.w : v.w * slope;
+      reinterpret_cast<float4 *>(gm + off)[p4] = r;
+      ag += (v.x + v.y) + (v.z + v.w);
+      am += (r.x + r.y) + (r.z + r.w);
+    }
+  } else {
+    for (long long e = (long long)blockIdx.x * 256 + threadIdx.x; e < per; e += (long long)gridDim.x * 256) {
+      const long long b = e / HW, p = e - b * HW;
+      const size_t off = ((size_t)b * C + c) * HW + p;
+      const float v = g[off], r = out[off] > 0.f ? v : v * slope;
+      gm[off] = r;
+      ag += v;
+      am += r;
+    }
+  }
+  if (part) {
+    ag = block_sum<256>(ag, sm);
+    am = block_sum<256>(am, sm);
+    if (threadIdx.x == 0) {
+      part[(size_t)c * gridDim.x + blockIdx.x] = ag;
+      part[((size_t)C + c) * gridDim.x + blockIdx.x] = am;
+    }
+  }
+}
+
 __global__ __launch_bounds__(256) void k_diffgrad(float *__restrict__ p, const float *__restrict__ g,
                                                   float *__restrict__ m, float *__restrict__ v,
                                                   float *__restrict__ pg, long long n, float step_size, float b1,
@@ -652,6 +693,26 @@
   return HG_OK;
 }
 
+int hg_dblock_head(const float *g, const float *out, float slope, float *gm, float *csum_g, float *csum_gm, int32_t B,
+                   int32_t C, int32_t HW, void *workspace, size_t workspace_bytes, void *stream) {
+  if (!g || !out || !gm || B <= 0 || C <= 0 || HW <= 0 || !(slope >= 0.f)) return HG_EINVAL;
+  if ((csum_g != nullptr) != (csum_gm != nullptr)) return HG_EINVAL;
+  hipStream_t st = (hipStream_t)stream;
+  const int chunks = plane_chunks(C, (long long)B * HW / 4);
+  if (csum_g && (!workspace || workspace_bytes < (size_t)2 * C * chunks * sizeof(float))) return HG_EWORKSPACE;
+  float *part = csum_g ? (float *)workspace : nullptr;
+  hipLaunchKernelGGL(k_dblock_head, dim3(chunks, C), dim3(256), 0, st, g, out, gm, part, slope, B, C, HW);
+  HG_LAUNCH_CHECK();
+  if (csum_g) {
+    hipLaunchKernelGGL(k_plane_sum_finish, dim3((C + 255) / 256), dim3(256), 0, st, (const float *)part, csum_g, C, chunks);
+    HG_LAUNCH_CHECK();
+    hipLaunchKernelGGL(k_plane_sum_finish, dim3((C + 255) / 256), dim3(256), 0, st, (const float *)part + (size_t)C * chunks,
+                       csum_gm, C, chunks);
+    HG_LAUNCH_CHECK();
+  }
+  return HG_OK;
+}
+
 int hg_diffgrad_step(float *p, const float *g, float *exp_avg, float *exp_avg_sq, float *prev_grad, int64_t n,
                      float lr, float beta1, float beta2, float eps, int32_t step, void *stream) {
   if (!p || !g || !exp_avg || !exp_avg_sq || !prev_grad || n <= 0 || step < 1) return HG_EINVAL;
diff --git a/histogan_amd/csrc/hg_wino.hip b/histogan_amd/csrc/hg_wino.hip
--- a/histogan_amd/csrc/hg_wino.hip
+++ b/histogan_amd/csrc/hg_wino.hip
@@ -5,6 +5,7 @@
 #include "../../include/hg_hist.h"
 #include "../../include/hg_conv.h"
 #include "../../include/hg_wino.h"
+#include "../../include/hg_nets.h"
 
 namespace {
 
@@ -37,12 +38,16 @@
   float *slab;
   int blocks, total_tiles;
   int xcd;
+  const float *mask_ref;
+  float mask_slope;
+  float *csum_part;
 };
 
 __device__ __forceinline__ int mrow(int r, int lk) { return (r & 3) + 8 * (r >> 2) + 4 * lk; }
 
-template <int TC, int TP, int KC, bool FE>
+template <int TC, int TP, int KC, bool FE, bool DM = false>
 __global__ __launch_bounds__(512) void k_wino(const WinoArgs a) {
+  static_assert(!(FE && DM), "the masked epilogue extends the plain one");
   constexpr int NT = 512, NB = 32 * TC, TB = 32 * TP;
   static_assert(KC * TB == NT, "one (channel, tile) patch per thread and chunk");
   constexpr int NV = (KC / 2) * TC;
@@ -266,6 +271,11 @@
   bool eok[TP];
   float ebias[TC][2], enw[TC][2], eosc[TC][2][TP];
   f32x2 enz[TP][2];
+  float ecs[DM ? TC : 1][2];
+  if constexpr (DM) {
+#pragma unroll
+    for (int i = 0; i < TC; ++i) ecs[i][0] = ecs[i][1] = 0.f;
+  }
 #pragma unroll
   for (int j = 0; j < TP; ++j) {
     const int tl = 32 * j + ecol;
@@ -275,7 +285,7 @@
 #pragma unroll
     for (int p2 = 0; p2 < 2; ++p2) {
       enz[j][p2] = f32x2{0.f, 0.f};
-      if (fin && a.noise_img && eok[j])
+      if (!DM && fin && a.noise_img && eok[j])
         enz[j][p2] = *reinterpret_cast<const f32x2 *>(a.noise_img + ((size_t)etb[j] * a.noise_S + 2 * ety[j] + p2) * a.noise_S + 2 * etx[j]);
     }
   }
@@ -284,16 +294,17 @@
 #pragma unroll
     for (int h = 0; h < 2; ++h) {
       const int n = e_n0 + 32 * i + erow + 16 * h, nc_ = n < N ? n : N - 1;
-      ebias[i][h] = (fin && a.bias) ? a.bias[nc_] : 0.f;
-      enw[i][h] = (fin && a.noise_img) ? a.noise_w[nc_] : 0.f;
-#pragma unroll
-      for (int j = 0; j < TP; ++j) eosc[i][h][j] = (fin && a.oscale && eok[j]) ? a.oscale[etb[j] * N + nc_] : 1.f;
+      ebias[i][h] = (!DM && fin && a.bias) ? a.bias[nc_] : 0.f;
+      enw[i][h] = (!DM && fin && a.noise_img) ? a.noise_w[nc_] : 0.f;
+#pragma unroll
+      for (int j = 0; j < TP; ++j) eosc[i][h][j] = (!DM && fin && a.oscale && eok[j]) ? a.oscale[etb[j] * N + nc_] : 1.f;
     }
 #pragma unroll
   for (int i = 0; i < TC; ++i) {
 #pragma unroll
     for (int j = 0; j < TP; ++j) {
       f32x2 ead[2][2];
+      f32x2 emk[DM ? 2 : 1][2];
 #pragma unroll
       for (int h = 0; h < 2; ++h)
 #pragma unroll
@@ -302,6 +313,11 @@
           const int n = e_n0 + 32 * i + erow + 16 * h;
           if (fin && a.addend && eok[j] && n < N)
             ead[h][p2] = *reinterpret_cast<const f32x2 *>(a.addend + (((size_t)etb[j] * N + n) * H + 2 * ety[j] + p2) * W + 2 * etx[j]);
+          if constexpr (DM) {
+            emk[h][p2] = f32x2{1.f, 1.f};
+            if (fin && a.mask_ref && eok[j] && n < N)
+              emk[h][p2] = *reinterpret_cast<const f32x2 *>(a.mask_ref + (((size_t)etb[j] * N + n) * H + 2 * ety[j] + p2) * W + 2 * etx[j]);
+          }
         }
       __syncthreads();
 #pragma unroll
@@ -334,26 +350,51 @@
           for (int p2 = 0; p2 < 2; ++p2)
 #pragma unroll
             for (int q = 0; q < 2; ++q) {
-              float v = fmaf(y[p2][q], eosc[i][h][j], fmaf(enw[i][h], enz[j][p2][q], ebias[i][h])) + ead[h][p2][q];
-              if (a.slope > 0.f) v = v > 0.f ? v : a.slope * v;
+              float v;
+              if constexpr (DM) {
+                v = y[p2][q] + ead[h][p2][q];
+                v = emk[h][p2][q] > 0.f ? v : v * a.mask_slope;
+              } else {
+                v = fmaf(y[p2][q], eosc[i][h][j], fmaf(enw[i][h], enz[j][p2][q], ebias[i][h])) + ead[h][p2][q];
+                if (a.slope > 0.f) v = v > 0.f ? v : a.slope * v;
+              }
               y[p2][q] = v;
             }
+          if constexpr (DM) ecs[i][h] += (y[0][0] + y[0][1]) + (y[1][0] + y[1][1]);
         }
         *reinterpret_cast<f32x2 *>(ob + o) = f32x2{y[0][0], y[0][1]};
         *reinterpret_cast<f32x2 *>(ob + o + W) = f32x2{y[1][0], y[1][1]};
       }
     }
   }
+  if constexpr (DM) {
+    if (fin && a.csum_part != nullptr) {
+      const int nslots = a.bt_x * a.bt_y * ((a.B + (1 << a.lNI) - 1) >> a.lNI);
+      const int slot = ((e_b0 >> a.lNI) * a.bt_y + e_by) * a.bt_x + e_bx;
+#pragma unroll
+      for (int i = 0; i < TC; ++i)
+#pragma unroll
+        for (int h = 0; h < 2; ++h) {
+          float v = ecs[i][h];
+#pragma unroll
+          for (int o = 16; o > 0; o >>= 1) v += __shfl_xor(v, o, 64);
+          const int n = e_n0 + 32 * i + erow + 16 * h;
+          if (ecol == 0 && n < N) a.csum_part[(size_t)n * nslots + slot] = v;
+        }
+    }
+  }
     __syncthreads();
   }
 #undef HG_WINO_BARRIER
 }
 
+template <bool DM>
 __global__ __launch_bounds__(256) void k_wino_reduce(const float *__restrict__ slab, float *__restrict__ out,
                                                      const float *__restrict__ oscale, const float *__restrict__ bias,
                                                      const float *__restrict__ noise_w, const float *__restrict__ noise_img,
                                                      const float *__restrict__ addend, int noise_S, float slope,
-                                                     long long total4, int HW, int W, int N, int ksplit) {
+                                                     long long total4, int HW, int W, int N, int ksplit,
+                                                     const float *__restrict__ mask_ref, float mask_slope) {
   const size_t total = (size_t)total4 * 4;
   for (long long i4 = (long long)blockIdx.x * 256 + threadIdx.x; i4 < total4; i4 += (long long)gridDim.x * 256) {
     f32x4 v = {0.f, 0.f, 0.f, 0.f};
@@ -371,12 +412,16 @@
         nz[e] = noise_img[((size_t)(bn / N) * noise_S + ye) * noise_S + xe % W];
       }
     }
-    f32x4 ad = {0.f, 0.f, 0.f, 0.f};
+    f32x4 ad = {0.f, 0.f, 0.f, 0.f}, mk = {1.f, 1.f, 1.f, 1.f};
     if (addend) ad = *reinterpret_cast<const f32x4 *>(addend + i);
+    if constexpr (DM) {
+      if (mask_ref) mk = *reinterpret_cast<const f32x4 *>(mask_ref + i);
+    }
 #pragma unroll
     for (int e = 0; e < 4; ++e) {
       float r = fmaf(v[e], osc, fmaf(nw, nz[e], bs)) + ad[e];
       if (slope > 0.f) r = r > 0.f ? r : slope * r;
+      if constexpr (DM) r = mk[e] > 0.f ? r : r * mask_slope;
       v[e] = r;
     }
     *reinterpret_cast<f32x4 *>(out + i) = v;
@@ -829,11 +874,19 @@
   return true;
 }
 
+__global__ __launch_bounds__(256) void k_wino_csum_finish(const float *__restrict__ part, float *__restrict__ out, int N, int tiles) {
+  const int n = blockIdx.x * 256 + threadIdx.x;
+  if (n >= N) return;
+  float v = 0.f;
+  for (int t = 0; t < tiles; ++t) v += part[(size_t)n * tiles + t];
+  out[n] = v;
+}
+
 template <int TC, int TP, int KC>
-int launch_wino(const WinoArgs &a, const WinoPlan &p, bool fe, hipStream_t st) {
-  auto kern = fe ? k_wino<TC, TP, KC, true> : k_wino<TC, TP, KC, false>;
+int launch_wino(const WinoArgs &a, const WinoPlan &p, int fe, hipStream_t st) {
+  auto kern = fe == 2 ? k_wino<TC, TP, KC, false, true> : fe ? k_wino<TC, TP, KC, true> : k_wino<TC, TP, KC, false>;
   constexpr size_t lds = 2 * 16 * KC * 32 * TP * sizeof(float);
-  static bool attr[kMaxDev][2] = {};
+  static bool attr[kMaxDev][3] = {};
   const int dev = cur_dev();
   if (!attr[dev][fe]) {
     hipError_t e = hipFuncSetAttribute((const void *)kern, hipFuncAttributeMaxDynamicSharedMemorySize, (int)lds);
@@ -895,16 +948,60 @@
   return (size_t)p.ksplit * B * N * H * W * sizeof(float);
 }
 
+static size_t align256(size_t v) { return (v + 255) / 256 * 256; }
+static size_t wino_csum_bytes(const WinoPlan &p, int N) {
+  long long t = (long long)p.bt_x * p.bt_y * p.groups;
+  if (t < 64) t = 64;
+  return (size_t)N * t * sizeof(float);
+}
+
+size_t hg_wino_masked_workspace_bytes(int32_t B, int32_t K, int32_t N, int32_t H, int32_t W, int32_t want_csum) {
+  WinoPlan p;
+  if (!make_plan(B, K, N, H, W, p)) return 0;
+  const size_t slab = p.ksplit == 1 ? 0 : (size_t)p.ksplit * B * N * H * W * sizeof(float);
+  return want_csum ? align256(slab) + wino_csum_bytes(p, N) : slab;
+}
+
+static int wino_conv2d_impl(const float *in, const float *u, float *out, const float *iscale, const float *oscale,
+                            const float *bias, const float *noise_w, const float *noise_img, int32_t noise_S, float lrelu_slope,
+                            const float *addend, int32_t B, int32_t K, int32_t N, int32_t H, int32_t W, void *workspace,
+                            size_t workspace_bytes, void *stream, const float *mask_ref, float mask_slope, float *csum);
+
 int hg_wino_conv2d(const float *in, const float *u, float *out, const float *iscale, const float *oscale,
                    const float *bias, const float *noise_w, const float *noise_img, int32_t noise_S, float lrelu_slope,
                    const float *addend, int32_t B, int32_t K, int32_t N, int32_t H, int32_t W, void *workspace,
                    size_t workspace_bytes, void *stream) {
+  return wino_conv2d_impl(in, u, out, iscale, oscale, bias, noise_w, noise_img, noise_S, lrelu_slope, addend, B, K, N, H, W,
+                          workspace, workspace_bytes, stream, nullptr, 0.f, nullptr);
+}
+
+int hg_wino_conv2d_masked(const float *in, const float *u, float *out, const float *addend, const float *mask_ref,
+                          float mask_slope, float *csum, int32_t B, int32_t K, int32_t N, int32_t H, int32_t W,
+                          void *workspace, size_t workspace_bytes, void *stream) {
+  if (!(mask_slope >= 0.f)) return HG_EINVAL;
+  if (csum && (!workspace || workspace_bytes < hg_wino_masked_workspace_bytes(B, K, N, H, W, 1))) return HG_EWORKSPACE;
+  return wino_conv2d_impl(in, u, out, nullptr, nullptr, nullptr, nullptr, nullptr, 0, 0.f, addend, B, K, N, H, W, workspace,
+                          workspace_bytes, stream, mask_ref, mask_slope, csum);
+}
+
+static int wino_conv2d_impl(const float *in, const float *u, float *out, const float *iscale, const float *oscale,
+                            const float *bias, const float *noise_w, const float *noise_img, int32_t noise_S, float lrelu_slope,
+                            const float *addend, int32_t B, int32_t K, int32_t N, int32_t H, int32_t W, void *workspace,
+                            size_t workspace_bytes, void *stream, const float *mask_ref, float mask_slope, float *csum) {
   if (!in || !u || !out) return HG_EINVAL;
   if ((noise_img != nullptr) != (noise_w != nullptr) || lrelu_slope < 0.f) return HG_EINVAL;
   if (noise_img && (noise_S < H || noise_S < W || (noise_S & 1))) return HG_EINVAL;
   if (addend && (iscale || oscale || noise_img || lrelu_slope > 0.f)) return HG_EINVAL;
   WinoPlan p;
   if (!make_plan(B, K, N, H, W, p)) return HG_EUNSUPPORTED;
+  float *csum_part = nullptr;
+  size_t csum_bytes = 0;
+  if (csum) {
+    const size_t front = align256(p.ksplit == 1 ? 0 : (size_t)p.ksplit * B * N * H * W * sizeof(float));
+    csum_part = (float *)((char *)workspace + front);
+    csum_bytes = wino_csum_bytes(p, N);
+    workspace_bytes = front;
+  }
   if (p.ksplit > 1 && (!workspace || workspace_bytes < (size_t)p.ksplit * B * N * H * W * sizeof(float))) p.ksplit = 1;
   WinoArgs a;
   a.in = in; a.u = u; a.out = out; a.iscale = iscale; a.oscale = oscale; a.bias = bias; a.addend = addend;
@@ -915,16 +1012,27 @@
   a.ksplit = p.ksplit; a.slab = (float *)workspace;
   a.blocks = (int)p.blocks; a.total_tiles = (int)(p.blocks * p.ksplit);
   a.xcd = p.nblk > 1 && p.nblk < 8 && (p.blocks / p.nblk) % 8 == 0;
+  const bool dm = (mask_ref || csum) && p.ksplit == 1;
+  a.mask_ref = mask_ref; a.mask_slope = mask_slope; a.csum_part = dm ? csum_part : nullptr;
   hipStream_t st = (hipStream_t)stream;
-  const bool fe = iscale != nullptr;
+  const int fe = dm ? 2 : (iscale != nullptr ? 1 : 0);
   int rc = p.variant == 0 ? launch_wino<2, 2, 8>(a, p, fe, st) : launch_wino<1, 4, 4>(a, p, fe, st);
   if (rc) return rc;
   if (p.ksplit > 1) {
     const long long total = (long long)B * N * H * W;
     long long nb = (total / 4 + 255) / 256;
     if (nb > 4096) nb = 4096;
-    hipLaunchKernelGGL(k_wino_reduce, dim3((unsigned)nb), dim3(256), 0, st, a.slab, out, oscale, bias, noise_w, noise_img,
-                       addend, noise_S, lrelu_slope, total / 4, H * W, W, N, p.ksplit);
+    if (mask_ref)
+      hipLaunchKernelGGL(k_wino_reduce<true>, dim3((unsigned)nb), dim3(256), 0, st, a.slab, out, oscale, bias, noise_w, noise_img,
+                         addend, noise_S, lrelu_slope, total / 4, H * W, W, N, p.ksplit, mask_ref, mask_slope);
+    else
+      hipLaunchKernelGGL(k_wino_reduce<false>, dim3((unsigned)nb), dim3(256), 0, st, a.slab, out, oscale, bias, noise_w,
+                         noise_img, addend, noise_S, lrelu_slope, total / 4, H * W, W, N, p.ksplit, nullptr, 0.f);
+    HG_LAUNCH_CHECK();
+    if (csum) return hg_channel_sum(out, csum, B, N, H * W, csum_part, csum_bytes, st);
+  } else if (csum) {
+    hipLaunchKernelGGL(k_wino_csum_finish, dim3((unsigned)((N + 255) / 256)), dim3(256), 0, st, csum_part, csum, N,
+                       p.bt_x * p.bt_y * p.groups);
     HG_LAUNCH_CHECK();
   }
   return HG_OK;
diff --git a/histogan_amd/nets.py b/histogan_amd/nets.py
--- a/histogan_amd/nets.py
+++ b/histogan_amd/nets.py
@@ -5,6 +5,7 @@
 import torch.nn.functional as F
 from torch import nn
 
+from . import conv as _conv
 from . import ops
 from .conv import conv2d, conv2d_add, conv2d_lrelu, conv2d_same
 
@@ -281,9 +282,13 @@
         self.downsample = Conv2d(filters, filters, 3, padding=1, stride=2) if downsample else None
 
     def forward(self, x):
-        h = conv2d_lrelu(x, self.net[0].weight, self.net[0].bias, 0.2)
-        h = conv2d_lrelu(h, self.net[2].weight, self.net[2].bias, 0.2)
-        x = conv2d_add(x, self.conv_res.weight, self.conv_res.bias, h)
+        if _conv.fused_dblock_active(x, self.net[0].weight):
+            x = _conv.dblock(x, self.net[0].weight, self.net[0].bias, self.net[2].weight, self.net[2].bias,
+                             self.conv_res.weight, self.conv_res.bias, 0.2)
+        else:
+            h = conv2d_lrelu(x, self.net[0].weight, self.net[0].bias, 0.2)
+            h = conv2d_lrelu(h, self.net[2].weight, self.net[2].bias, 0.2)
+            x = conv2d_add(x, self.conv_res.weight, self.conv_res.bias, h)
         if self.downsample is not None:
             x = self.downsample(x)
         return x
diff --git a/histogan_amd/trainer.py b/histogan_amd/trainer.py
--- a/histogan_amd/trainer.py
+++ b/histogan_amd/trainer.py
@@ -15,7 +15,8 @@
 
 from . import ddp
 from .augment import AugWrapper
-from .conv import drain_pack_streams, enable_pack_cache, input_grads_only, prepack_async, weights_changed
+from .conv import (drain_pack_streams, enable_pack_cache, fused_dblock_backward, input_grads_only, prepack_async,
+                   weights_changed)
 from .hist import hellinger_loss
 from .nets import Discriminator, Generator, HistVectorizer, StyleVectorizer
 from .optim import DiffGrad, FlatParams, conv_first, ema_update
@@ -27,6 +28,7 @@
 GRAPH_AUTO_RATIO = float(os.environ.get('HG_GRAPH_AUTO_RATIO', '0.9'))
 GRAPH_GP = os.environ.get('HG_GRAPH_GP', '1') != '0'
 EARLY_GREDUCE = os.environ.get('HG_EARLY_GREDUCE', '1') != '0'
+FUSED_DBLOCK = os.environ.get('HG_FUSED_DBLOCK', '1') != '0'
 LAZY_STATS = os.environ.get('HG_LAZY_STATS', '1') != '0'
 
 
@@ -582,10 +584,13 @@
                 with torch.cuda.stream(side2):
                     early = g_forward()
             if has_vq or apply_gradient_penalty:
-                fake_output, fake_q_loss = Disc(aug(generated_images, True))
-                real_output, real_q_loss = Disc(aug(image_batch))
+                with fused_dblock_backward(FUSED_DBLOCK):
+                    fake_output, fake_q_loss = Disc(aug(generated_images, True))
+                with fused_dblock_backward(FUSED_DBLOCK and not apply_gradient_penalty):
+                    real_output, real_q_loss = Disc(aug(image_batch))
             else:
-                both_output, both_q_loss = Disc(_cat_batches(aug(generated_images, True), aug(image_batch)))
+                with fused_dblock_backward(FUSED_DBLOCK):
+                    both_output, both_q_loss = Disc(_cat_batches(aug(generated_images, True), aug(image_batch)))
                 fake_output, real_output = both_output[:batch_size], both_output[batch_size:]
                 fake_q_loss = real_q_loss = both_q_loss * 0.5
             mark('d_forward')
@@ -649,7 +654,8 @@
                 update_d()
                 d_updated = True
             self._mark('g_forward_joined_d_updated')
-            fake_output, _ = Disc(aug(generated_images))
+            with fused_dblock_backward(FUSED_DBLOCK):
+                fake_output, _ = Disc(aug(generated_images))
             self._mark('g_phase_d_forward')
             if self.hist_alpha_weight:
                 generated_histograms = self.histBlock(generated_images, pre_relu=True,
diff --git a/include/hg_conv.h b/include/hg_conv.h
--- a/include/hg_conv.h
+++ b/include/hg_conv.h
@@ -50,6 +50,12 @@
                     int32_t B, int32_t K, int32_t N, int32_t Hi, int32_t Wi, int32_t ksize, int32_t stride,
                     void *workspace, size_t workspace_bytes, void *stream);
 
+size_t hg_conv2d_dgrad_masked_workspace_bytes(int32_t B, int32_t K, int32_t N, int32_t Hi, int32_t Wi, int32_t ksize,
+                                              int32_t want_csum);
+int hg_conv2d_dgrad_masked(const float *gout, const float *wt, float *gin, const float *addend, const float *mask_ref,
+                           float mask_slope, float *csum, int32_t B, int32_t K, int32_t N, int32_t Hi, int32_t Wi,
+                           int32_t ksize, void *workspace, size_t workspace_bytes, void *stream);
+
 size_t hg_conv2d_wgrad_workspace_bytes(int32_t B, int32_t K, int32_t N, int32_t Hi, int32_t Wi, int32_t ksize,
                                        int32_t stride);
 int hg_conv2d_wgrad(const float *in, const float *gout, float *gw, const float *iscale, const float *gscale,
diff --git a/include/hg_nets.h b/include/hg_nets.h
--- a/include/hg_nets.h
+++ b/include/hg_nets.h
@@ -42,6 +42,9 @@
 int hg_lrelu_bwd_channel_sum(const float *g, const float *out, float slope, float *gm, float *csum, int32_t B, int32_t C,
                              int32_t HW, void *workspace, size_t workspace_bytes, void *stream);
 
+int hg_dblock_head(const float *g, const float *out, float slope, float *gm, float *csum_g, float *csum_gm, int32_t B,
+                   int32_t C, int32_t HW, void *workspace, size_t workspace_bytes, void *stream);
+
 size_t hg_demod_style_grad_workspace_bytes(int32_t B, int32_t N, int32_t K);
 int hg_demod_style_grad(const float *gd, const float *d, const float *s1, const float *wsq, float *gy, int32_t B, int32_t N,
                         int32_t K, void *workspace, size_t workspace_bytes, void *stream);
diff --git a/include/hg_wino.h b/include/hg_wino.h
--- a/include/hg_wino.h
+++ b/include/hg_wino.h
@@ -29,6 +29,11 @@
                    const float *addend, int32_t B, int32_t K, int32_t N, int32_t H, int32_t W, void *workspace,
                    size_t workspace_bytes, void *stream);
 
+size_t hg_wino_masked_workspace_bytes(int32_t B, int32_t K, int32_t N, int32_t H, int32_t W, int32_t want_csum);
+int hg_wino_conv2d_masked(const float *in, const float *u, float *out, const float *addend, const float *mask_ref,
+                          float mask_slope, float *csum, int32_t B, int32_t K, int32_t N, int32_t H, int32_t W,
+                          void *workspace, size_t workspace_bytes, void *stream);
+
 int hg_wino_wgrad_supported(int32_t B, int32_t K, int32_t N, int32_t H, int32_t W);
 size_t hg_wino_wgrad_workspace_bytes(int32_t B, int32_t K, int32_t N, int32_t H, int32_t W);
 int hg_wino_wgrad(const float *in, const float *gout, float *gw, int32_t B, int32_t K, int32_t N, int32_t H, int32_t W,
```

Result: slower. 859.7 images/s (-2.2%).
